# LiJiangnanBit/path_optimizer

Measured on AMD Instinct MI355X. Metric: QP paths/sec at N=200 pts, batch=4096; ADMM iters to 1e-4, higher is better.
Workload: dtype f64

## Files before the change

path_optimizer_amd/binding.py:

```python
from __future__ import annotations

import ctypes as C
import os
import sys

import numpy as np

from .abi import (INFO_BYTES, INFO_DTYPE, PO_ABI_VERSION, PO_ERR_HIP, PO_ERR_UNSUPPORTED, PO_OK, PoBatchIn, PoBatchOut, PoParams)

_HERE = os.path.dirname(os.path.abspath(__file__))
LIB_PATH = os.environ.get("PO_LIB") or os.path.join(_HERE, "libpo_hip.so")
_LIB = None

EXPORTS = ["po_default_params", "po_problem_dims", "po_keep_control_steps", "po_create", "po_destroy", "po_set_stream", "po_debug_set", "po_device_count",
           "po_solve_batch", "po_solve_batch_device", "po_assemble_batch", "po_scaling_batch", "po_last_kernel_ms", "po_last_phase_ms", "po_debug_get", "po_strerror",
           "po_last_hip_error", "po_version", "po_set_map", "po_postcheck_batch", "po_postcheck_batch_device", "po_bounds_batch",
           "po_bounds_batch_device", "po_map_sample", "po_smooth_dims", "po_smooth_batch", "po_smooth_batch_device",
           "po_resample_batch", "po_resample_batch_device", "po_limits_batch", "po_limits_batch_device", "po_dp_search_batch",
           "po_dp_search_batch_device", "po_bspline_batch_device", "po_segment_raw_batch_device", "po_post_project_batch_device",
           "po_segment_init_batch_device", "po_plan_batch", "po_plan_batch_device", "po_densify_batch", "po_densify_batch_device",
           "po_distance_map_batch", "po_distance_map_batch_device", "po_set_map_occupancy", "po_set_map_occupancy_device", "po_get_map",
           "po_set_map_stack", "po_set_map_stack_occupancy", "po_set_map_stack_occupancy_device", "po_set_map_assignment", "po_set_map_assignment_device",
           "po_get_map_layer", "po_map_sample_layer",
           "po_rasterize_batch", "po_rasterize_batch_device", "po_set_map_stack_obstacles", "po_set_map_stack_obstacles_device",
           "po_set_world_occupancy", "po_set_world_occupancy_device", "po_rasterize_scene_batch", "po_rasterize_scene_batch_device",
           "po_set_map_stack_scene", "po_set_map_stack_scene_device",
           "po_default_select_params", "po_select_batch", "po_select_batch_device",
           "po_default_speed_params", "po_speed_batch", "po_speed_batch_device",
           "po_default_dynamic_params", "po_dynamic_batch", "po_dynamic_batch_device",
           "po_default_stplan_params", "po_stplan_batch", "po_stplan_batch_device",
           "po_default_nudge_params", "po_nudge_batch", "po_nudge_batch_device",
           "po_default_trajectory_params", "po_trajectory_batch", "po_trajectory_batch_device",
           "po_default_agentsets_params", "po_agentsets_batch", "po_agentsets_batch_device"]


class PoError(RuntimeError):
    pass


_ENV_DEBUG = {"PO_IDENTITY_ORDER": "identity_order", "PO_DEBUG_CYCLES": "debug_cycles", "PO_SMOOTH_SEQ": "smooth_seq",
              "PO_SMOOTH_WAVES": "smooth_waves", "PO_SMOOTH_NOPAD": "smooth_nopad", "PO_SMOOTH_DEBUG": "smooth_debug", "PO_DP_ONE_WAVE": "dp_one_wave", "PO_NEWTON_SLICE": "newton_slice",
              "PO_FIXED_LENGTH": "fixed_length"}


def lib():
    global _LIB
    if _LIB is None:
        if not os.path.exists(LIB_PATH):
            raise PoError(f"{LIB_PATH} not built: run `python -c 'import __graft_entry__ as g; g.build()'` "
                          "(hipcc --offload-arch=gfx950). There is no CPU fallback.")
        try:
            import torch
        except Exception:
            pass
        L = C.CDLL(LIB_PATH)
        L.po_strerror.restype = C.c_char_p
        L.po_last_hip_error.restype = C.c_char_p
        L.po_version.restype = C.c_char_p
        ver = L.po_version().decode()
        parts = ver.split()
        if len(parts) < 2 or not parts[1].isdigit() or int(parts[1]) != PO_ABI_VERSION:
            raise PoError(f"{LIB_PATH} reports '{ver}' but this binding is written against PO_ABI_VERSION {PO_ABI_VERSION} (include/po_hip.h): rebuild the library")
        L.po_create.argtypes = [C.c_int, C.POINTER(PoParams), C.POINTER(C.c_void_p)]
        L.po_destroy.argtypes = [C.c_void_p]
        L.po_set_stream.argtypes = [C.c_void_p, C.c_void_p]
        L.po_solve_batch.argtypes = [C.c_void_p, C.POINTER(PoBatchIn), C.POINTER(PoBatchOut)]
        L.po_solve_batch_device.argtypes = [C.c_void_p, C.POINTER(PoBatchIn), C.POINTER(PoBatchOut)]
        L.po_assemble_batch.argtypes = [C.c_void_p, C.POINTER(PoBatchIn), C.c_void_p, C.c_void_p, C.c_void_p]
        L.po_scaling_batch.argtypes = [C.c_void_p, C.POINTER(PoBatchIn), C.c_void_p]
        L.po_last_kernel_ms.argtypes = [C.c_void_p, C.POINTER(C.c_float)]
        L.po_last_phase_ms.argtypes = [C.c_void_p, C.POINTER(C.c_float)]
        L.po_debug_get.argtypes = [C.c_void_p, C.c_char_p, C.POINTER(C.c_longlong)]
        L.po_distance_map_batch.argtypes = [C.c_void_p, C.c_int, C.c_void_p, C.c_void_p]
        L.po_distance_map_batch_device.argtypes = [C.c_void_p, C.c_int, C.c_void_p, C.c_void_p]
        L.po_set_map_occupancy.argtypes = [C.c_void_p, C.c_void_p]
        L.po_set_map_occupancy_device.argtypes = [C.c_void_p, C.c_void_p]
        L.po_get_map.argtypes = [C.c_void_p, C.c_void_p, C.c_void_p]
        L.po_set_map_stack.argtypes = [C.c_void_p, C.c_int, C.c_void_p, C.c_void_p]
        L.po_set_map_stack_occupancy.argtypes = [C.c_void_p, C.c_int, C.c_void_p, C.c_void_p]
        L.po_set_map_stack_occupancy_device.argtypes = [C.c_void_p, C.c_int, C.c_void_p, C.c_void_p]
        L.po_set_map_assignment.argtypes = [C.c_void_p, C.c_int, C.c_void_p]
        L.po_set_map_assignment_device.argtypes = [C.c_void_p, C.c_int, C.c_void_p]
        L.po_get_map_layer.argtypes = [C.c_void_p, C.c_int, C.c_void_p, C.c_void_p]
        L.po_map_sample_layer.argtypes = [C.c_void_p, C.c_int, C.c_int, C.c_void_p, C.c_void_p, C.c_void_p]
        L.po_rasterize_batch.argtypes = [C.c_void_p, C.c_int, C.c_void_p, C.c_void_p, C.c_void_p]
        L.po_rasterize_batch_device.argtypes = [C.c_void_p, C.c_int, C.c_void_p, C.c_void_p, C.c_void_p]
        L.po_set_map_stack_obstacles.argtypes = [C.c_void_p, C.c_int, C.c_void_p, C.c_void_p]
        L.po_set_map_stack_obstacles_device.argtypes = [C.c_void_p, C.c_int, C.c_void_p, C.c_void_p]
        L.po_set_world_occupancy.argtypes = [C.c_void_p, C.c_void_p, C.c_int]
        L.po_set_world_occupancy_device.argtypes = [C.c_void_p, C.c_void_p, C.c_int]
        L.po_rasterize_scene_batch.argtypes = [C.c_void_p, C.c_int, C.c_void_p, C.c_void_p, C.c_void_p]
        L.po_rasterize_scene_batch_device.argtypes = [C.c_void_p, C.c_int, C.c_void_p, C.c_void_p, C.c_void_p]
        L.po_set_map_stack_scene.argtypes = [C.c_void_p, C.c_int, C.c_void_p, C.c_void_p]
        L.po_set_map_stack_scene_device.argtypes = [C.c_void_p, C.c_int, C.c_void_p, C.c_void_p]
        L.po_default_select_params.argtypes = [C.c_void_p]
        L.po_default_select_params.restype = None
        L.po_select_batch.argtypes = [C.c_void_p, C.c_void_p, C.c_void_p, C.c_void_p]
        L.po_select_batch_device.argtypes = [C.c_void_p, C.c_void_p, C.c_void_p, C.c_void_p]
        L.po_default_speed_params.argtypes = [C.c_void_p]
        L.po_default_speed_params.restype = None
        L.po_speed_batch.argtypes = [C.c_void_p, C.c_void_p, C.c_void_p, C.c_void_p]
        L.po_speed_batch_device.argtypes = [C.c_void_p, C.c_void_p, C.c_void_p, C.c_void_p]
        L.po_default_dynamic_params.argtypes = [C.c_void_p]
        L.po_default_dynamic_params.restype = None
        L.po_dynamic_batch.argtypes = [C.c_void_p, C.c_void_p, C.c_void_p, C.c_void_p]
        L.po_dynamic_batch_device.argtypes = [C.c_void_p, C.c_void_p, C.c_void_p, C.c_void_p]
        L.po_default_stplan_params.argtypes = [C.c_void_p]
        L.po_default_stplan_params.restype = None
        L.po_stplan_batch.argtypes = [C.c_void_p, C.c_void_p, C.c_void_p, C.c_void_p]
        L.po_stplan_batch_device.argtypes = [C.c_void_p, C.c_void_p, C.c_void_p, C.c_void_p]
        L.po_default_nudge_params.argtypes = [C.c_void_p]
        L.po_default_nudge_params.restype = None
        L.po_nudge_batch.argtypes = [C.c_void_p, C.c_void_p, C.c_void_p, C.c_void_p]
        L.po_nudge_batch_device.argtypes = [C.c_void_p, C.c_void_p, C.c_void_p, C.c_void_p]
        L.po_default_trajectory_params.argtypes = [C.c_void_p]
        L.po_default_trajectory_params.restype = None
        L.po_trajectory_batch.argtypes = [C.c_void_p, C.c_void_p, C.c_void_p, C.c_void_p]
        L.po_trajectory_batch_device.argtypes = [C.c_void_p, C.c_void_p, C.c_void_p, C.c_void_p]
        L.po_default_agentsets_params.argtypes = [C.c_void_p]
        L.po_default_agentsets_params.restype = None
        L.po_agentsets_batch.argtypes = [C.c_void_p, C.c_void_p, C.c_void_p, C.c_void_p]
        L.po_agentsets_batch_device.argtypes = [C.c_void_p, C.c_void_p, C.c_void_p, C.c_void_p]
        _LIB = L
    return _LIB


def _check(rc: int):
    if rc != PO_OK:
        L = lib()
        msg = L.po_strerror(rc).decode()
        if rc == PO_ERR_HIP:
            msg += ": " + L.po_last_hip_error().decode()
        raise PoError(f"libpo_hip: {msg} (rc={rc})")


def default_params() -> PoParams:
    p = PoParams()
    lib().po_default_params(C.byref(p))
    return p


def default_select_params():
    from .abi import PoSelectParams

    p = PoSelectParams()
    lib().po_default_select_params(C.byref(p))
    return p


def default_speed_params():
    from .abi import PoSpeedParams

    p = PoSpeedParams()
    lib().po_default_speed_params(C.byref(p))
    return p


def default_dynamic_params():
    from .abi import PoDynamicParams

    p = PoDynamicParams()
    lib().po_default_dynamic_params(C.byref(p))
    return p


def default_stplan_params():
    from .abi import PoStplanParams

    p = PoStplanParams()
    lib().po_default_stplan_params(C.byref(p))
    return p


def default_nudge_params():
    from .abi import PoNudgeParams

    p = PoNudgeParams()
    lib().po_default_nudge_params(C.byref(p))
    return p


def default_trajectory_params():
    from .abi import PoTrajectoryParams

    p = PoTrajectoryParams()
    lib().po_default_trajectory_params(C.byref(p))
    return p


def covering_discs(params):
    rad = np.sqrt(np.float64(params.car_length / 8) * np.float64(params.car_length / 8) + np.float64(params.car_width / 2) * np.float64(params.car_width / 2))
    return [float(params.d[j]) for j in range(4)], float(rad + np.float64(params.safety_margin))


def default_agentsets_params():
    from .abi import PoAgentsetsParams

    p = PoAgentsetsParams()
    lib().po_default_agentsets_params(C.byref(p))
    return p


def footprint_reach(params, margin):
    width, back, front = params.car_width, params.car_length / 2.0 - params.rear_axle_to_center, params.car_length / 2.0 + params.rear_axle_to_center
    length, bx, shift = front + back, (front - back) / 2.0, width / 4.0
    small_r = float(np.sqrt(2 * (shift * shift)))
    large_r = float(np.sqrt(width * width + ((length - width) / 2.0) * ((length - width) / 2.0))) / 2
    cx = [-back + shift, -back + shift, front - shift, front - shift, bx + (length - width) / 4, bx - (length - width) / 4]
    cy = [-width / 2.0 + shift, width / 2.0 - shift, -width / 2.0 + shift, width / 2.0 - shift, 0.0, 0.0]
    cr = [small_r] * 4 + [large_r] * 2
    return max(float(np.hypot(cx[q], cy[q])) + cr[q] for q in range(6)) + float(margin) + 1e-6


def problem_dims(form: int, N: int, keep: int):
    n, m, c = C.c_int(), C.c_int(), C.c_int()
    _check(lib().po_problem_dims(form, N, keep, C.byref(n), C.byref(m), C.byref(c)))
    return n.value, m.value, c.value


def smooth_dims(kind: int, P: int):
    n, m = C.c_int(), C.c_int()
    _check(lib().po_smooth_dims(kind, P, C.byref(n), C.byref(m)))
    return n.value, m.value


def keep_control_steps(form: int, ref_s) -> int:
    ref_s = np.ascontiguousarray(ref_s, dtype=np.float64)
    k = lib().po_keep_control_steps(form, ref_s.ctypes.data_as(C.c_void_p), len(ref_s))
    if k < 0:
        _check(k)
    return k


def _np(a):
    return None if a is None else a.ctypes.data_as(C.c_void_p)


OBSTACLE_DTYPE = np.dtype([("kind", np.int32), ("n_verts", np.int32), ("v", np.float64, (16,))])


def obstacle_disc(x, y, r):
    from .abi import PO_OBS_DISC

    o = np.zeros((), dtype=OBSTACLE_DTYPE)
    o["kind"] = PO_OBS_DISC
    o["v"][:3] = (x, y, r)
    return o


def obstacle_polygon(xy):
    from .abi import PO_OBS_MAX_VERTS, PO_OBS_POLY

    xy = np.asarray(xy, dtype=np.float64)
    if xy.ndim != 2 or xy.shape[1] != 2 or not 3 <= len(xy) <= PO_OBS_MAX_VERTS:
        raise ValueError("a polygon has 3 .. 8 vertices (x, y)")
    o = np.zeros((), dtype=OBSTACLE_DTYPE)
    o["kind"] = PO_OBS_POLY
    o["n_verts"] = len(xy)
    o["v"][:2 * len(xy)] = xy.reshape(-1)
    return o


def obstacle_box(cx, cy, half_length, half_width, yaw):
    c, s = np.cos(yaw), np.sin(yaw)
    corners = [(cx + sl * half_length * c - sw * half_width * s, cy + sl * half_length * s + sw * half_width * c) for sl, sw in ((1, 1), (-1, 1), (-1, -1), (1, -1))]
    return obstacle_polygon(corners)


def pack_obstacles(layers):
    if isinstance(layers, tuple) and len(layers) == 2:
        return np.ascontiguousarray(layers[0], dtype=OBSTACLE_DTYPE).reshape(-1), np.ascontiguousarray(layers[1], dtype=np.int32).reshape(-1)
    first = np.zeros(len(layers) + 1, dtype=np.int32)
    first[1:] = np.cumsum([len(l) for l in layers])
    obs = np.zeros(int(first[-1]), dtype=OBSTACLE_DTYPE)
    n = 0
    for l in layers:
        for o in l:
            obs[n] = o
            n += 1
    return obs, first


AGENT_DTYPE = np.dtype([("n_pts", np.int32), ("flags", np.int32), ("radius", np.float64), ("t", np.float64, (8,)), ("x", np.float64, (8,)),
                        ("y", np.float64, (8,))])


def pack_agents(sets):
    if isinstance(sets, tuple) and len(sets) == 2:
        return np.ascontiguousarray(sets[0], dtype=AGENT_DTYPE).reshape(-1), np.ascontiguousarray(sets[1], dtype=np.int32).reshape(-1)
    first = np.zeros(len(sets) + 1, dtype=np.int32)
    first[1:] = np.cumsum([len(s) for s in sets])
    agents = np.zeros(int(first[-1]), dtype=AGENT_DTYPE)
    i = 0
    for s in sets:
        for radius, flags, pts in s:
            if len(pts) > 8:
                raise ValueError("an agent has at most 8 points (t, x, y)")
            agents[i]["n_pts"], agents[i]["flags"], agents[i]["radius"] = len(pts), int(flags), radius
            for j, (t, x, y) in enumerate(pts):
                agents[i]["t"][j], agents[i]["x"][j], agents[i]["y"][j] = t, x, y
            i += 1
    return agents, first


def _agent_lists(agents):
    from .abi import PoAgentLists

    ag, first = pack_agents(agents)
    return PoAgentLists(_np(ag) if len(ag) else None, _np(first), len(ag), len(first) - 1), ag, first


def _agent_lists_device(t):
    from .abi import PoAgentLists

    ag = t.get("agents")
    n_agents = 0 if ag is None else ag.numel() * ag.element_size() // AGENT_DTYPE.itemsize
    return PoAgentLists(C.c_void_p(ag.data_ptr()) if n_agents else None, C.c_void_p(t["first"].data_ptr()), n_agents, t["first"].shape[0] - 1)


def pack_rings(shared, layers=None):
    rings = list(shared) + ([] if layers is None else [r for l in layers for r in l])
    xy = [np.asarray(r[0], dtype=np.float64).reshape(-1, 2) for r in rings]
    start = np.zeros(len(rings) + 1, dtype=np.int32)
    start[1:] = np.cumsum([len(v) for v in xy])
    verts = np.concatenate(xy) if xy else np.zeros((0, 2))
    flags = np.array([int(r[1]) for r in rings], dtype=np.int32)
    first = None
    if layers is not None:
        first = np.full(len(layers) + 1, len(shared), dtype=np.int32)
        first[1:] += np.cumsum([len(l) for l in layers]).astype(np.int32)
    return np.ascontiguousarray(verts, dtype=np.float64), start, flags, len(shared), first


def _i32(a):
    return None if a is None else np.ascontiguousarray(a, dtype=np.int32)


class Engine:

    def __init__(self, device: int = 0, params: PoParams | None = None):
        self.params = params or default_params()
        self._h = C.c_void_p()
        _check(lib().po_create(device, C.byref(self.params), C.byref(self._h)))
        try:
            for env, key in _ENV_DEBUG.items():
# ... 766 lines not shown
```

path_optimizer_amd/csrc/po_capi.cpp:

```cpp
#include <hip/hip_runtime.h>

#include <cmath>
#include <cstdint>
#include <cstdio>
#include <algorithm>
#include <cstdlib>
#include <cstring>
#include <limits>
#include <mutex>
#include <new>
#include <string>
#include <vector>

#include "../../include/po_hip.h"
#include "po_handle.hpp"
#include "po_launch.hpp"
#include "po_map.hpp"
#include "po_smooth.hpp"

static thread_local std::string g_hip_err;

bool hip_ok(hipError_t e, const char *what) {
    if (e == hipSuccess) return true;
    g_hip_err = std::string(what) + ": " + hipGetErrorString(e);
    return false;
}

extern "C" {

void po_default_params(po_params *p) {
    if (!p) return;
    const double car_length = 4.9, rear_axle_to_center = 1.45;
    std::memset(p, 0, sizeof(*p));
    p->d[0] = -3.0 / 8.0 * car_length + rear_axle_to_center;
    p->d[1] = -1.0 / 8.0 * car_length + rear_axle_to_center;
    p->d[2] = 1.0 / 8.0 * car_length + rear_axle_to_center;
    p->d[3] = 3.0 / 8.0 * car_length + rear_axle_to_center;
    p->w_curv = 10; p->w_curv_rate = 200; p->w_dev = 0; p->w_slack = 3;
    p->k_w_curv = 50; p->k_w_curv_rate = 200; p->k_w_dev = 0;
    p->w_k_slack = 500; p->w_kp_slack = 25000;
    p->margin = 1.3;
    p->max_steer = 30.0 * M_PI / 180.0;
    p->wheel_base = 2.85;
    p->enable_collision_check = 1;
    p->car_width = 2.0; p->car_length = 4.9; p->rear_axle_to_center = 1.45; p->safety_margin = 0.0;
    p->constraint_end_heading = 1;
    p->scaling = 10;
    p->eps_abs = 1e-4; p->eps_rel = 1e-4; p->eps_prim_inf = 1e-4; p->eps_dual_inf = 1e-4;
    p->rho0 = 0.1; p->sigma = 1e-6; p->alpha = 1.6; p->adapt_tol = 5.0;
    p->max_iter = 4000; p->check_every = 25; p->adapt_every = 100;
    p->t2_w_dev = 0.005; p->t2_w_curv = 1; p->t2_w_curv_rate = 10;
    p->cart_w_curv = 1; p->cart_w_curv_rate = 50; p->cart_w_dev = 0.0;
    p->mu = 0.4; p->max_curvature_rate = 0.1; p->search_lateral_range = 10.0; p->search_long_spacing = 1.5; p->search_lat_spacing = 0.6;
    p->enable_dynamic_segmentation = 1;
    p->enable_raw_output = 1; p->output_spacing = 0.3;
    p->polish = 0; p->polish_delta = 1e-6; p->polish_refine_iter = 3;
    p->refine = 0; p->refine_eps = 1e-7; p->refine_rounds = 1; p->refine_chain = 2; p->refine_extra_rounds = 0;
    p->refine_newton_rho = 100.0; p->refine_newton_rho_eq = 1e4; p->refine_newton_rho_max = 1e5; p->refine_ls_tol = 0.6; p->refine_ls_max = 30; p->refine_newton_max = 300; p->refine_newton_final = 3; p->refine_newton_escalate = 12; p->refine_newton_rho_eq_max = 1e6;
}

int po_problem_dims(int form, int N, int keep, int *n, int *m, int *C) {
    if (N < 2) return PO_ERR_INVALID;
    int c, nn, mm;
    if (form == PO_KP) {
        if (keep < 1) return PO_ERR_INVALID;
        c = (N + keep - 2) / keep; nn = 5 * N + c; mm = 11 * N + c + 2;
    } else if (form == PO_KPC) {
        if (keep != 4) return PO_ERR_INVALID;
        c = (N + keep - 2) / keep; nn = 6 * N + c; mm = 12 * N + 3 * c + 2;
    } else if (form == PO_K) {
        c = N - 1; nn = 4 * N - 1; mm = 11 * N - 1;
    } else {
        return PO_ERR_INVALID;
    }
    if (n) *n = nn;
    if (m) *m = mm;
    if (C) *C = c;
    return PO_OK;
}

int po_keep_control_steps(int form, const double *ref_s, int N) {
    if (!ref_s || N < 2) return PO_ERR_INVALID;
    if (form == PO_KPC) return 4;
    if (form == PO_K) return 1;
    if (form != PO_KP) return PO_ERR_INVALID;
    double interval = 0;
    for (int i = 1; i < N && i < 10; ++i) interval = std::fmax(interval, ref_s[i] - ref_s[i - 1]);
    const double q = 1.2 / interval;
    const int k = (q >= 2147483647.0 || q != q) ? 1 : static_cast<int>(q);
    return k > 1 ? k : 1;
}

static void runtime_prepare() {
    static std::once_flag once;
    std::call_once(once, [] { setenv("GPU_MAX_HW_QUEUES", "16", 0); });
}

int po_device_count(void) {
    runtime_prepare();
    int n = 0;
    return hipGetDeviceCount(&n) == hipSuccess ? n : 0;
}

int po_create(int device, const po_params *params, po_handle *out) {
    if (!params || !out) return PO_ERR_INVALID;
    if (params->scaling < 0 || params->scaling > 100) return PO_ERR_INVALID;
    if (params->refine != 0 && params->refine != 2) return PO_ERR_INVALID;
    if (params->refine == 2 && (params->refine_rounds > 1 ? params->refine_rounds : 1) + (params->refine_extra_rounds > 0 ? params->refine_extra_rounds : 0) >= 32) return PO_ERR_INVALID;
    runtime_prepare();
    int ndev = 0;
    HIP_TRY(hipGetDeviceCount(&ndev));
    if (device < 0 || device >= ndev) return PO_ERR_INVALID;
    HIP_TRY(hipSetDevice(device));
    po_handle_s *h = new (std::nothrow) po_handle_s;
    if (!h) return PO_ERR_NOMEM;
    h->device = device;
    { int cus = 0; if (hipDeviceGetAttribute(&cus, hipDeviceAttributeMultiprocessorCount, device) == hipSuccess && cus > 0) h->wave_slots = 4 * cus; }
    h->params = *params;
    if (!hip_ok(hipStreamCreateWithFlags(&h->own_stream.s, hipStreamNonBlocking), "hipStreamCreate") ||
        !hip_ok(hipEventCreate(&h->ev0.e), "hipEventCreate") || !hip_ok(hipEventCreate(&h->ev1.e), "hipEventCreate")) {
        delete h;
        return PO_ERR_HIP;
    }
    for (Event &e : h->evh) if (!hip_ok(hipEventCreate(&e.e), "hipEventCreate")) { delete h; return PO_ERR_HIP; }
    for (Event &e : h->evp) if (!hip_ok(hipEventCreate(&e.e), "hipEventCreate")) { delete h; return PO_ERR_HIP; }
    {
        Lock g(h->mu);
        h->stream = h->own_stream.s;
    }
    *out = h;
    return PO_OK;
}

int po_destroy(po_handle h) {
    if (!h) return PO_ERR_INVALID;
    (void)hipSetDevice(h->device);
    {
        Lock g(h->mu);
        (void)hipStreamSynchronize(h->stream);
    }
    delete h;
    return PO_OK;
}

int po_debug_set(po_handle h, const char *key, int value) {
    if (!h || !key) return PO_ERR_INVALID;
    Lock g(h->mu);
    const std::string k(key);
    if (k == "identity_order") h->env_identity = value != 0;
    else if (k == "host_threads") h->host_threads = value < 0 ? 0 : value;
    else if (k == "debug_cycles") h->env_cycles = value != 0;
    else if (k == "newton_slice") { h->nw_slice = value > 0 ? (int)value : 0; h->nw_slice_forced = value > 0; }
    else if (k == "fixed_length") h->fixed_length = value != 0;
    else if (k == "smooth_seq") h->env_smooth_seq = value != 0;
    else if (k == "smooth_waves") h->env_smooth_waves = value;
    else if (k == "smooth_nopad") h->env_smooth_nopad = value != 0;
    else if (k == "smooth_debug") h->env_smooth_debug = value != 0;
    else if (k == "dp_one_wave") h->env_dp_one_wave = value != 0;
    else return PO_ERR_INVALID;
    return PO_OK;
}

int po_debug_get(po_handle h, const char *key, long long *value) {
    if (!h || !key || !value) return PO_ERR_INVALID;
    const std::string k(key);
    Lock g(h->mu);
    if (k == "map_ptr") {
        *value = (long long)reinterpret_cast<uintptr_t>(h->maps.d);
        return PO_OK;
    }
    if (k == "map_layers") {
        *value = h->maps.d ? h->maps.M : 0;
        return PO_OK;
    }
    if (k == "world_cells") {
        *value = h->world.cells ? (long long)h->world.size_x * (long long)h->world.size_y : 0;
        return PO_OK;
    }
    if (k == "fixed_length_used") {
        *value = h->fixed_used;
        return PO_OK;
    }
    if (k == "dp_waves_used") {
        *value = h->dp_waves_used;
        return PO_OK;
    }
    if (k == "smooth_variant_used") {
        *value = h->smooth_variant_used;
        return PO_OK;
    }
    if (k == "fallback_paths") {
        *value = 0;
        if (!h->fb_buf.p) return PO_OK;
        HIP_TRY(hipSetDevice(h->device));
        HIP_TRY(hipStreamSynchronize(h->stream));
        int c = 0;
        HIP_TRY(hipMemcpy(&c, h->fb_buf.p, sizeof(int), hipMemcpyDeviceToHost));
        *value = c;
        return PO_OK;
    }
    if (k == "newton_parked") {
        *value = -1;
        if (!h->nw_idx_buf.p || h->nw_last_B <= 0) return PO_OK;
        HIP_TRY(hipSetDevice(h->device));
        HIP_TRY(hipStreamSynchronize(h->stream));
        int c = 0;
        HIP_TRY(hipMemcpy(&c, static_cast<int *>(h->nw_idx_buf.p) + h->nw_last_B, sizeof(int), hipMemcpyDeviceToHost));
        *value = c;
        return PO_OK;
    }
    if (k == "newton_list_ok") {
        *value = -1;
        if (!h->nw_idx_buf.p || h->nw_last_B <= 0) return PO_OK;
        HIP_TRY(hipSetDevice(h->device));
        HIP_TRY(hipStreamSynchronize(h->stream));
        const int B = h->nw_last_B;
        std::vector<int> kl(2 * (size_t)B + 1);
        HIP_TRY(hipMemcpy(kl.data(), h->nw_idx_buf.p, sizeof(int) * kl.size(), hipMemcpyDeviceToHost));
        const int *keys = kl.data(), *list = kl.data() + B;
        const int n = list[0];
        int parked = 0;
        for (int b = 0; b < B; ++b) parked += keys[b] >= 0;
        bool ok = n == parked;
        std::vector<char> seen((size_t)B, 0);
        for (int i = 0; ok && i < n; ++i) {
            const int b = list[1 + i];
            ok = b >= 0 && b < B && keys[b] >= 0 && !seen[(size_t)b];
            if (ok) seen[(size_t)b] = 1;
            if (ok && i > 0) { const int a = list[i]; ok = keys[a] > keys[b] || (keys[a] == keys[b] && a < b); }
        }
        *value = ok ? 1 : 0;
        return PO_OK;
    }
    return PO_ERR_INVALID;
}

int po_set_stream(po_handle h, void *hip_stream) {
    if (!h) return PO_ERR_INVALID;
    Lock g(h->mu);
    h->stream = hip_stream ? static_cast<hipStream_t>(hip_stream) : h->own_stream.s;
    return PO_OK;
}

static po::DevCar make_car(const po_params &p) {
    po::DevCar c{};
    const double width = p.car_width, back = p.car_length / 2.0 - p.rear_axle_to_center, front = p.car_length / 2.0 + p.rear_axle_to_center;
    const double length = front + back;
    c.bx = (front - back) / 2.0;
    c.br = std::sqrt((length / 2) * (length / 2) + (width / 2) * (width / 2));
    const double shift = width / 4.0, small_r = std::sqrt(2 * (shift * shift));
    const double large_r = std::sqrt(width * width + ((length - width) / 2.0) * ((length - width) / 2.0)) / 2;
    const double px[4] = {-back + shift, -back + shift, front - shift, front - shift};
    const double py[4] = {-width / 2.0 + shift, width / 2.0 - shift, -width / 2.0 + shift, width / 2.0 - shift};
    for (int i = 0; i < 4; ++i) { c.cx[i] = px[i]; c.cy[i] = py[i]; c.cr[i] = small_r; }
    c.cx[4] = c.bx + (length - width) / 4; c.cy[4] = 0; c.cr[4] = large_r;
    c.cx[5] = c.bx - (length - width) / 4; c.cy[5] = 0; c.cr[5] = large_r;
    c.enable = p.enable_collision_check;
    return c;
}

static void publish_stack(po_handle h, int M, int sx, int sy, double res, double px, double py, bool layer_pos) PO_REQUIRES(h->mu) {
    const bool keep = h->maps.M == M && h->maps.layer_of;
    po::DevMaps s{};
    s.d = static_cast<const float *>(h->map_buf.p); s.sx = sx; s.sy = sy; s.res = res; s.px = px; s.py = py;
    s.M = M; s.stride = (size_t)sx * (size_t)sy;
    s.pos = layer_pos ? static_cast<const double *>(h->map_pos_buf.p) : nullptr;
    s.layer_of = keep ? static_cast<const int *>(h->map_assign_buf.p) : nullptr;
    s.n_assign = keep ? h->maps.n_assign : 0;
    h->maps = s;
}
static int install_layers(po_handle h, int M, const po_map *map, const double *pos_xy) PO_REQUIRES(h->mu) {
    HIP_TRY(hipSetDevice(h->device));
    const size_t bytes = sizeof(float) * (size_t)M * (size_t)map->size_x * (size_t)map->size_y;
    if (bytes > h->map_buf.cap) h->maps.d = nullptr;
    if (int rc = grow_after_sync(h, h->map_buf, bytes)) return rc;
    if (pos_xy) {
        if (int rc = grow_after_sync(h, h->map_pos_buf, sizeof(double) * 2 * (size_t)M)) return rc;
        HIP_TRY(hipMemcpyAsync(h->map_pos_buf.p, pos_xy, sizeof(double) * 2 * (size_t)M, hipMemcpyHostToDevice, h->stream));
    }
    HIP_TRY(hipMemcpyAsync(h->map_buf.p, map->distance, bytes, hipMemcpyHostToDevice, h->stream));
    HIP_TRY(hipStreamSynchronize(h->stream));
    publish_stack(h, M, map->size_x, map->size_y, map->resolution, map->pos_x, map->pos_y, pos_xy != nullptr);
    return PO_OK;
}

int po_set_map(po_handle h, const po_map *map) {
    if (!h || !map || !map->distance || map->size_x < 1 || map->size_y < 1 || !(map->resolution > 0)) return PO_ERR_INVALID;
    Lock g(h->mu);
    return install_layers(h, 1, map, nullptr);
}

int po_set_map_stack(po_handle h, int M, const po_map *layers, const double *pos_xy) {
    if (!h || M < 1 || !layers || !layers->distance || layers->size_x < 1 || layers->size_y < 1 || !(layers->resolution > 0)) return PO_ERR_INVALID;
    if (layers->size_x > po_edt_max_side() || layers->size_y > po_edt_max_side() || M > po_edt_max_images()) return PO_ERR_UNSUPPORTED;
    Lock call(h->call_mu);
    Lock g(h->mu);
    return install_layers(h, M, layers, pos_xy);
}

int po_set_map_assignment_device(po_handle h, int n, const int *layer_of) {
    if (!h || n < 0) return PO_ERR_INVALID;
    Lock g(h->mu);
    if (n == 0 || !layer_of) {
        h->maps.layer_of = nullptr; h->maps.n_assign = 0;
        return PO_OK;
    }
    if (!h->maps.d) return PO_ERR_INVALID;
    HIP_TRY(hipSetDevice(h->device));
    if (int rc = grow_after_sync(h, h->map_assign_buf, sizeof(int) * (size_t)n)) return rc;
    HIP_TRY(hipMemcpyAsync(h->map_assign_buf.p, layer_of, sizeof(int) * (size_t)n, hipMemcpyDeviceToDevice, h->stream));
    h->maps.layer_of = static_cast<const int *>(h->map_assign_buf.p); h->maps.n_assign = n;
    return PO_OK;
}

int po_set_map_assignment(po_handle h, int n, const int *layer_of) {
    if (!h || n < 0) return PO_ERR_INVALID;
    Lock call(h->call_mu);
    Lock g(h->mu);
    if (n == 0 || !layer_of) {
        h->maps.layer_of = nullptr; h->maps.n_assign = 0;
        return PO_OK;
    }
    if (!h->maps.d) return PO_ERR_INVALID;
    for (int b = 0; b < n; ++b)
        if (layer_of[b] < 0 || layer_of[b] >= h->maps.M) return PO_ERR_INVALID;
    HIP_TRY(hipSetDevice(h->device));
    if (int rc = grow_after_sync(h, h->map_assign_buf, sizeof(int) * (size_t)n)) {
        h->maps.layer_of = nullptr; h->maps.n_assign = 0;
        return rc;
    }
    HIP_TRY(hipMemcpyAsync(h->map_assign_buf.p, layer_of, sizeof(int) * (size_t)n, hipMemcpyHostToDevice, h->stream));
    HIP_TRY(hipStreamSynchronize(h->stream));
    h->maps.layer_of = static_cast<const int *>(h->map_assign_buf.p); h->maps.n_assign = n;
    return PO_OK;
}

static int check_occupancy(po_handle h, int M, const po_occupancy *occ) {
    if (!h || M < 1 || !occ || !occ->cells || occ->size_x < 1 || occ->size_y < 1 || !(occ->resolution > 0)) return PO_ERR_INVALID;
    if (occ->size_x > po_edt_max_side() || occ->size_y > po_edt_max_side() || M > po_edt_max_images()) return PO_ERR_UNSUPPORTED;
    return PO_OK;
}

int po_distance_map_batch_device(po_handle h, int M, const po_occupancy *occ, float *distance) {
    if (int rc = check_occupancy(h, M, occ)) return rc;
    if (!distance) return PO_ERR_INVALID;
    Lock g(h->mu);
    HIP_TRY(hipSetDevice(h->device));
    if (int rc = grow_after_sync(h, h->edt_buf, po_edt_scratch_bytes(M, occ->size_x, occ->size_y))) return rc;
    HIP_TRY(po_launch_edt(occ->cells, M, occ->size_x, occ->size_y, (float)occ->resolution, h->edt_buf.p, distance, h->stream));
    return PO_OK;
}

int po_distance_map_batch(po_handle h, int M, const po_occupancy *occ, float *distance) {
    if (int rc = check_occupancy(h, M, occ)) return rc;
    if (!distance) return PO_ERR_INVALID;
    const size_t cells = (size_t)M * (size_t)occ->size_x * (size_t)occ->size_y;
    Stage S;
    const Slot<float> d_dist = S.out(distance, cells);
    const Slot<unsigned char> d_cells = S.in(occ->cells, cells);
    return staged_call(h, S, &po_handle_s::edt_io, true, [&] {
        po_occupancy dev = *occ;
        dev.cells = d_cells;
        return po_distance_map_batch_device(h, M, &dev, d_dist);
    });
}

static int stack_from_images(po_handle h, int M, const unsigned char *cells, int sx, int sy, double res, double px, double py, const double *pos_xy)
    PO_REQUIRES(h->mu) {
    const size_t stack_bytes = sizeof(float) * (size_t)M * (size_t)sx * (size_t)sy;
    if (stack_bytes > h->map_buf.cap) h->maps.d = nullptr;
    if (int rc = grow_after_sync(h, h->map_buf, stack_bytes)) return rc;
    if (int rc = grow_after_sync(h, h->edt_buf, po_edt_scratch_bytes(M, sx, sy))) return rc;
    if (pos_xy) {
        if (int rc = grow_after_sync(h, h->map_pos_buf, sizeof(double) * 2 * (size_t)M)) return rc;
        HIP_TRY(hipMemcpyAsync(h->map_pos_buf.p, pos_xy, sizeof(double) * 2 * (size_t)M, hipMemcpyDeviceToDevice, h->stream));
    }
    HIP_TRY(po_launch_edt(cells, M, sx, sy, (float)res, h->edt_buf.p, static_cast<float *>(h->map_buf.p), h->stream));
    publish_stack(h, M, sx, sy, res, px, py, pos_xy != nullptr);
    return PO_OK;
}

int po_set_map_stack_occupancy_device(po_handle h, int M, const po_occupancy *occ, const double *pos_xy) {
    if (int rc = check_occupancy(h, M, occ)) return rc;
    Lock g(h->mu);
    HIP_TRY(hipSetDevice(h->device));
    return stack_from_images(h, M, occ->cells, occ->size_x, occ->size_y, occ->resolution, occ->pos_x, occ->pos_y, pos_xy);
}

int po_set_map_occupancy_device(po_handle h, const po_occupancy *occ) { return po_set_map_stack_occupancy_device(h, 1, occ, nullptr); }

int po_set_map_stack_occupancy(po_handle h, int M, const po_occupancy *occ, const double *pos_xy) {
    if (int rc = check_occupancy(h, M, occ)) return rc;
    Stage S;
    const Slot<unsigned char> d_cells = S.in(occ->cells, (size_t)M * (size_t)occ->size_x * (size_t)occ->size_y);
    const Slot<double> d_pos = S.in(pos_xy, 2 * (size_t)M);
    return staged_call(h, S, &po_handle_s::edt_io, true, [&] {
        po_occupancy dev = *occ;
        dev.cells = d_cells;
        return po_set_map_stack_occupancy_device(h, M, &dev, d_pos);
    });
}

int po_set_map_occupancy(po_handle h, const po_occupancy *occ) { return po_set_map_stack_occupancy(h, 1, occ, nullptr); }

static int check_lists(po_handle h, int M, const po_obstacle_lists *L) {
    if (!h || M < 1 || !L || !L->first || L->n_obs < 0 || (L->n_obs > 0 && !L->obs) || L->size_x < 1 || L->size_y < 1 || !(L->resolution > 0) ||
        !std::isfinite(L->resolution))
        return PO_ERR_INVALID;
    if (L->base_count != 0 && L->base_count != 1 && L->base_count != M) return PO_ERR_INVALID;
    if (L->base_count != 0 && !L->base) return PO_ERR_INVALID;
    if (L->size_x > po_edt_max_side() || L->size_y > po_edt_max_side() || M > po_edt_max_images()) return PO_ERR_UNSUPPORTED;
    return PO_OK;
}
static int check_list_contents(int M, const po_obstacle_lists *L) {
    if (L->first[0] != 0) return PO_ERR_INVALID;
    for (int k = 0; k < M; ++k)
        if (L->first[k + 1] < L->first[k]) return PO_ERR_INVALID;
    if (L->first[M] > L->n_obs) return PO_ERR_INVALID;
    for (int i = 0; i < L->n_obs; ++i) {
        const po_obstacle &o = L->obs[i];
        if (o.kind == PO_OBS_DISC) {
            if (!std::isfinite(o.v[0]) || !std::isfinite(o.v[1]) || !std::isfinite(o.v[2]) || o.v[2] < 0) return PO_ERR_INVALID;
        } else if (o.kind == PO_OBS_POLY) {
            if (o.n_verts < 3 || o.n_verts > PO_OBS_MAX_VERTS) return PO_ERR_INVALID;
            for (int e = 0; e < 2 * o.n_verts; ++e)
                if (!std::isfinite(o.v[e])) return PO_ERR_INVALID;
        } else {
            return PO_ERR_INVALID;
        }
    }
    return PO_OK;
}
struct StagedLists {
    Slot<po_obstacle> obs;
    Slot<int> first;
    Slot<unsigned char> base;
    Slot<double> pos;
    void declare(Stage &S, int M, const po_obstacle_lists *L, const double *pos_xy) {
        obs = S.in(L->n_obs > 0 ? L->obs : nullptr, (size_t)L->n_obs);
        first = S.in(L->first, (size_t)M + 1);
        base = S.in(L->base_count > 0 ? L->base : nullptr, (size_t)L->base_count * (size_t)L->size_x * (size_t)L->size_y);
        pos = S.in(pos_xy, 2 * (size_t)M);
    }
    po_obstacle_lists device(const po_obstacle_lists *L) const {
        po_obstacle_lists d = *L;
        d.obs = obs; d.first = first; d.base = base;
        return d;
    }
};

int po_rasterize_batch_device(po_handle h, int M, const po_obstacle_lists *lists, const double *pos_xy, unsigned char *cells_out) {
    if (int rc = check_lists(h, M, lists)) return rc;
    if (!cells_out) return PO_ERR_INVALID;
    Lock g(h->mu);
    HIP_TRY(hipSetDevice(h->device));
    HIP_TRY(po_launch_raster(lists, M, pos_xy, cells_out, h->stream));
    return PO_OK;
}

int po_rasterize_batch(po_handle h, int M, const po_obstacle_lists *lists, const double *pos_xy, unsigned char *cells_out) {
    if (int rc = check_lists(h, M, lists)) return rc;
    if (!cells_out) return PO_ERR_INVALID;
    if (int rc = check_list_contents(M, lists)) return rc;
    Stage S;
    StagedLists d;
    d.declare(S, M, lists, pos_xy);
    const Slot<unsigned char> d_cells = S.out(cells_out, (size_t)M * (size_t)lists->size_x * (size_t)lists->size_y);
    return staged_call(h, S, &po_handle_s::edt_io, true, [&] {
        const po_obstacle_lists dev = d.device(lists);
        return po_rasterize_batch_device(h, M, &dev, d.pos, d_cells);
    });
}

int po_set_map_stack_obstacles_device(po_handle h, int M, const po_obstacle_lists *lists, const double *pos_xy) {
    if (int rc = check_lists(h, M, lists)) return rc;
    Lock g(h->mu);
    HIP_TRY(hipSetDevice(h->device));
    if (int rc = grow_after_sync(h, h->raster_buf, (size_t)M * (size_t)lists->size_x * (size_t)lists->size_y)) return rc;
    unsigned char *cells = static_cast<unsigned char *>(h->raster_buf.p);
    HIP_TRY(po_launch_raster(lists, M, pos_xy, cells, h->stream));
    return stack_from_images(h, M, cells, lists->size_x, lists->size_y, lists->resolution, lists->pos_x, lists->pos_y, pos_xy);
}

int po_set_map_stack_obstacles(po_handle h, int M, const po_obstacle_lists *lists, const double *pos_xy) {
    if (int rc = check_lists(h, M, lists)) return rc;
    if (int rc = check_list_contents(M, lists)) return rc;
    Stage S;
    StagedLists d;
    d.declare(S, M, lists, pos_xy);
    return staged_call(h, S, &po_handle_s::edt_io, true, [&] {
        const po_obstacle_lists dev = d.device(lists);
        return po_set_map_stack_obstacles_device(h, M, &dev, d.pos);
    });
}

static int check_world(po_handle h, const po_occupancy *w, int outside_occupied) {
    if (!h || (outside_occupied != 0 && outside_occupied != 1)) return PO_ERR_INVALID;
    if (!w) return PO_OK;
    if (!w->cells || w->size_x < 1 || w->size_y < 1 || !(w->resolution > 0) || !std::isfinite(w->resolution) || !std::isfinite(w->pos_x) || !std::isfinite(w->pos_y))
        return PO_ERR_INVALID;
    if (w->size_x > PO_WORLD_MAX_SIDE || w->size_y > PO_WORLD_MAX_SIDE) return PO_ERR_UNSUPPORTED;
    return PO_OK;
}
static int install_world(po_handle h, const po_occupancy *w, int outside_occupied, hipMemcpyKind kind) PO_REQUIRES(h->mu) {
    if (!w) {
        h->world = po_occupancy{};
        return PO_OK;
    }
    HIP_TRY(hipSetDevice(h->device));
    const size_t bytes = (size_t)w->size_x * (size_t)w->size_y;
    if (bytes > h->world_buf.cap) h->world.cells = nullptr;
    if (int rc = grow_after_sync(h, h->world_buf, bytes)) return rc;
    HIP_TRY(hipMemcpyAsync(h->world_buf.p, w->cells, bytes, kind, h->stream));
    h->world = *w;
    h->world.cells = static_cast<const unsigned char *>(h->world_buf.p);
    h->world_outside = outside_occupied;
    return PO_OK;
}

int po_set_world_occupancy_device(po_handle h, const po_occupancy *world, int outside_occupied) {
    if (int rc = check_world(h, world, outside_occupied)) return rc;
    Lock g(h->mu);
    return install_world(h, world, outside_occupied, hipMemcpyDeviceToDevice);
}

int po_set_world_occupancy(po_handle h, const po_occupancy *world, int outside_occupied) {
    if (int rc = check_world(h, world, outside_occupied)) return rc;
    Lock call(h->call_mu);
    Lock g(h->mu);
    PO_TRY(install_world(h, world, outside_occupied, hipMemcpyHostToDevice));
    if (world) HIP_TRY(hipStreamSynchronize(h->stream));
    return PO_OK;
}
// ... 903 lines not shown
```

path_optimizer_amd/csrc/po_device.hpp:

```cpp
#pragma once
#include <hip/hip_runtime.h>

#include "../../include/po_hip.h"

namespace po {

constexpr double kInf = 1e30;
constexpr double kInfThresh = 1e26;
constexpr int kStatusDeferred = -100;
constexpr double kRhoMin = 1e-6, kRhoMax = 1e6, kRhoEqOverIneq = 1e3, kRhoTol = 1e-4;
constexpr double kPi = 3.14159265358979323846;
constexpr double kPi2 = 1.57079632679489661923;
constexpr int kNwKeys = 32;

enum { F_KP = 0, F_KPC = 1, F_K = 2 };
enum { M_EY = 1, M_EPHI = 2, M_C = 4, M_S1 = 8, M_S2 = 16 };

struct DevParams {
    double d1, d2, d3, d4;
    double w_dev, w_c, w_cr, w_s1, w_s2, w_u, w_su;
    double margin, kmax, max_steer, wheel_base;
    double sigma, alpha, rho0, eps_abs, eps_rel, eps_pinf, adapt_tol;
    int max_iter, check_every, adapt_every, end_heading;
    double pol_delta;
    int polish, pol_refine;
    int refine, ref_rounds, ref_extra;
    double ref_eps;
    double ref_nw_rho, ref_nw_rho_eq, ref_nw_rho_max, ref_nw_rho_eq_max, ref_ls_tol;
    int ref_ls_max, ref_nw_max, ref_nw_final, ref_nw_esc;
    int ref_nw_slice;
};

struct DevBatch {
    int B, N, keep, C;
    const double *ref_x, *ref_y, *ref_z, *ref_k, *ref_s;
    const double *bounds, *x0, *goal_z, *max_k, *max_kp;
    double *out_states;
    po_info *out_info;
    double *out_x;
    const int *n_points;
    const int *order;
    const double *scale;
    long long *dbg_cycles;
    int perm_bits;
    int only_deferred;
    int n, m;
    int round;
    double *pol_state;
    int pol_stride;
    int *fb_list;
    int nw_phase;
    double *nw_state;
    int nw_stride;
    int *nw_keys;
    int *nw_list;
    int nw_follows;
    int fixed_len;
};

template <int F> struct FormTraits;
template <> struct FormTraits<F_KP> {
    static constexpr int NLOC = 8, NEND = 2, NDYN = 3, NS = 1, HAS_U = 1, NCTL = 1, HAS_SU = 0;
};
template <> struct FormTraits<F_KPC> {
    static constexpr int NLOC = 9, NEND = 2, NDYN = 3, NS = 2, HAS_U = 1, NCTL = 3, HAS_SU = 1;
};
template <> struct FormTraits<F_K> {
    static constexpr int NLOC = 9, NEND = 0, NDYN = 2, NS = 1, HAS_U = 0, NCTL = 0, HAS_SU = 0;
};

__host__ __device__ __forceinline__ double clipd(double v, double l, double u) { return fmin(fmax(v, l), u); }
struct NegInfT { __host__ __device__ constexpr operator double() const { return -kInf; } };
struct PosInfT { __host__ __device__ constexpr operator double() const { return kInf; } };
__host__ __device__ __forceinline__ double clipd(double v, NegInfT, double u) { return fmin(v, u); }
__host__ __device__ __forceinline__ double clipd(double v, double l, PosInfT) { return fmax(v, l); }
__host__ __device__ __forceinline__ double clipd(double v, NegInfT, PosInfT) { return v; }

__device__ __forceinline__ double rho_of(double l, double u, double rho, double rho_eq) {
    if (l < -kInfThresh && u > kInfThresh) return kRhoMin;
    return (u - l < kRhoTol) ? rho_eq : rho;
}

__device__ __forceinline__ double wrap_angle(double a) {
    for (int it = 0; it < 64; ++it) {
        if (a > kPi) a -= 2 * kPi;
        else if (a < -kPi) a += 2 * kPi;
        else break;
    }
    return a;
}

struct StageIn {
    double lb[4], ub[4];
    double maxk;
    double elo, ehi;
    int j, N, last;
};

template <int F, class Fn> __device__ __forceinline__ void local_rows(const StageIn &s, const DevParams &P, Fn &fn) {
    if constexpr (F == F_KP) {
        fn.template row<M_C>(0, 0., 0., 1., 0., 0., -P.kmax, P.kmax);
        fn.template row<M_S1>(1, 0., 0., 0., 1., 0., 0.0, P.margin);
        fn.template row<M_EY | M_EPHI>(2, 1., P.d1, 0., 0., 0., s.lb[0], s.ub[0]);
        fn.template row<M_EY | M_EPHI>(3, 1., P.d3, 0., 0., 0., s.lb[2], s.ub[2]);
        fn.template row<M_EY | M_EPHI | M_S1>(4, 1., P.d4, 0., -1., 0., NegInfT{}, s.ub[3] - P.margin);
        fn.template row<M_EY | M_EPHI | M_S1>(5, 1., P.d4, 0., 1., 0., s.lb[3] + P.margin, PosInfT{});
        fn.template row<M_EY | M_EPHI | M_S1>(6, 1., P.d2, 0., -1., 0., NegInfT{}, s.ub[1] - P.margin);
        fn.template row<M_EY | M_EPHI | M_S1>(7, 1., P.d2, 0., 1., 0., s.lb[1] + P.margin, PosInfT{});
    } else if constexpr (F == F_KPC) {
        fn.template row<M_C | M_S2>(0, 0., 0., 1., 0., 1., -s.maxk, PosInfT{});
        fn.template row<M_C | M_S2>(1, 0., 0., 1., 0., -1., NegInfT{}, s.maxk);
        fn.template row<M_S1>(2, 0., 0., 0., 1., 0., 0.0, P.margin);
        fn.template row<M_S2>(3, 0., 0., 0., 0., 1., 0.0, fmax(P.kmax - s.maxk, 0.0));
        fn.template row<M_EY | M_EPHI>(4, 1., P.d1, 0., 0., 0., s.lb[0], s.ub[0]);
        fn.template row<M_EY | M_EPHI>(5, 1., P.d2, 0., 0., 0., s.lb[1], s.ub[1]);
        fn.template row<M_EY | M_EPHI>(6, 1., P.d4, 0., 0., 0., s.lb[3], s.ub[3]);
        fn.template row<M_EY | M_EPHI | M_S1>(7, 1., P.d3, 0., -1., 0., NegInfT{}, s.ub[2] - P.margin);
        fn.template row<M_EY | M_EPHI | M_S1>(8, 1., P.d3, 0., 1., 0., s.lb[2] + P.margin, PosInfT{});
    } else {
        const bool win = s.last && (s.elo > -kInf);
        fn.template row<M_EPHI>(0, 0., 1., 0., 0., 0., win ? s.elo : -kInf, win ? s.ehi : kInf);
        fn.template row<M_EY>(1, 1., 0., 0., 0., 0., NegInfT{}, PosInfT{});
        if (!s.last) fn.template row<M_C>(2, 0., 0., 1., 0., 0., -P.max_steer, P.max_steer);
        fn.template row<M_S1>(3, 0., 0., 0., 1., 0., 0.0, P.margin);
        fn.template row<M_EY | M_EPHI>(4, 1., P.d1, 0., 0., 0., s.lb[0], s.ub[0]);
        fn.template row<M_EY | M_EPHI>(5, 1., P.d3, 0., 0., 0., s.lb[2], s.ub[2]);
        fn.template row<M_EY | M_EPHI>(6, 1., P.d4, 0., 0., 0., s.lb[3], s.ub[3]);
        fn.template row<M_EY | M_EPHI | M_S1>(7, 1., P.d2, 0., -1., 0., NegInfT{}, s.ub[1] - P.margin);
        fn.template row<M_EY | M_EPHI | M_S1>(8, 1., P.d2, 0., 1., 0., s.lb[1] + P.margin, PosInfT{});
    }
}

template <int F, class Fn> __device__ __forceinline__ void end_rows(const StageIn &s, const DevParams &, Fn &fn) {
    if constexpr (F == F_KP) {
        fn.template row<M_EY>(0, 1., 0., 0., 0., 0., -1.0, 1.0);
        fn.template row<M_EPHI>(1, 0., 1., 0., 0., 0., s.elo, s.ehi);
    } else if constexpr (F == F_KPC) {
        fn.template row<M_EY>(0, 1., 0., 0., 0., 0., NegInfT{}, PosInfT{});
        fn.template row<M_EPHI>(1, 0., 1., 0., 0., 0., s.elo, s.ehi);
    }
}

template <int F> __device__ __forceinline__ int ref_row_local(int r, int j, int N, int C) {
    if constexpr (F == F_KP) {
        const int cb = 5 * N + C;
        switch (r) {
            case 0: return 3 * N + j;
            case 1: return 4 * N + C + j;
            case 2: return cb + 2 * j;
            case 3: return cb + 2 * j + 1;
            default: return cb + (r - 2) * N + j;
        }
    } else if constexpr (F == F_KPC) {
        const int sb = 5 * N + 2 * C, cb = 7 * N + 3 * C;
        switch (r) {
            case 0: return 3 * N + j;
            case 1: return 4 * N + j;
            case 2: return sb + j;
            case 3: return sb + N + j;
            case 4: case 5: case 6: return cb + 3 * j + (r - 4);
            case 7: return cb + 3 * N + j;
            default: return cb + 4 * N + j;
        }
    } else {
        switch (r) {
            case 0: return 2 * N + 2 * j;
            case 1: return 2 * N + 2 * j + 1;
            case 2: return 4 * N + j;
            case 3: return 5 * N - 1 + j;
            case 4: case 5: case 6: return 6 * N - 1 + 3 * j + (r - 4);
            case 7: return 9 * N - 1 + j;
            default: return 10 * N - 1 + j;
        }
    }
}
template <int F> __device__ __forceinline__ int ref_row_end(int r, int N, int C) {
    if constexpr (F == F_KP) return 11 * N + C + r;
    else if constexpr (F == F_KPC) return 12 * N + 3 * C + r;
    else return 0;
}
template <int F> __device__ __forceinline__ int ref_row_ctl(int r, int c, int N, int C) {
    if constexpr (F == F_KP) return 4 * N + c;
    else if constexpr (F == F_KPC) return r == 0 ? 5 * N + c : (r == 1 ? 5 * N + C + c : 5 * N + 2 * C + 2 * N + c);
    else return 0;
}

template <int F> struct Dyn {
    double f[FormTraits<F>::NDYN][3];
    double beta[FormTraits<F>::NDYN];
    double b[FormTraits<F>::NDYN];
};
template <int F> __device__ __forceinline__ constexpr int dyn_tau(int r) {
    if constexpr (F == F_K) return r == 0 ? 1 : 0;
    else return r;
}
template <int F> __device__ __forceinline__ Dyn<F> make_dyn(double k, double ds, const DevParams &P) {
    Dyn<F> d;
    if constexpr (F == F_K) {
        const double steer = atan(k * P.wheel_base);
        const double cs = cos(steer);
        const double c2 = __dmul_rn(cs, cs);
        d.f[0][0] = __dmul_rn(-ds, __dmul_rn(k, k));
        d.f[0][1] = 1.0;
        d.f[0][2] = ds / P.wheel_base / c2;
        d.beta[0] = 0;
        d.b[0] = __dmul_rn(ds, steer) / P.wheel_base / c2;
        d.f[1][0] = 1.0;
        d.f[1][1] = ds;
        d.f[1][2] = 0;
        d.beta[1] = 0;
        d.b[1] = 0;
    } else {
        d.f[0][0] = 1.0; d.f[0][1] = ds; d.f[0][2] = 0; d.beta[0] = 0; d.b[0] = 0;
        d.f[1][0] = __dmul_rn(-__dmul_rn(k, k), ds); d.f[1][1] = 1.0; d.f[1][2] = ds; d.beta[1] = 0;
        d.b[1] = __dmul_rn(ds, k);
        d.f[2][0] = 0; d.f[2][1] = 0; d.f[2][2] = 1.0; d.beta[2] = ds; d.b[2] = 0;
    }
    return d;
}

__device__ __forceinline__ void k_trig(double k, double ds, const DevParams &P, double tr[2]) {
    const double steer = atan(k * P.wheel_base);
    const double cs = cos(steer);
    const double c2 = __dmul_rn(cs, cs);
    tr[0] = ds / P.wheel_base / c2;
    tr[1] = __dmul_rn(ds, steer) / P.wheel_base / c2;
}
template <int F> __device__ __forceinline__ Dyn<F> make_dyn_tr(double k, double ds, const double tr[2], const DevParams &P) {
    if constexpr (F == F_K) {
        Dyn<F> d;
        d.f[0][0] = __dmul_rn(-ds, __dmul_rn(k, k)); d.f[0][1] = 1.0; d.f[0][2] = tr[0]; d.beta[0] = 0; d.b[0] = tr[1];
        d.f[1][0] = 1.0; d.f[1][1] = ds; d.f[1][2] = 0; d.beta[1] = 0; d.b[1] = 0;
        return d;
    } else {
        return make_dyn<F>(k, ds, P);
    }
}

template <int F> __device__ __forceinline__ double p_diag_node(int comp, int j, int N, const DevParams &P) {
    if (comp == 0) return P.w_dev;
    if (comp == 1) return 0.0;
    if constexpr (F == F_K) {
        if (j >= N - 1) return 0.0;
        return (j == 0 || j == N - 2) ? P.w_c + P.w_cr : P.w_cr * 2 + P.w_c;
    } else {
        return P.w_c;
    }
}

__device__ __forceinline__ int ctl_index(int i, int keep) { return keep == 4 ? (i >> 2) : (i / keep); }
__device__ __forceinline__ bool last_of_group(int i, int N, int keep) {
    return (i == N - 2) || (keep == 4 ? (((i + 1) & 3) == 0) : ((i + 1) % keep == 0));
}

__device__ __forceinline__ int perm_index(unsigned i, int bits, int B) {
    if (bits <= 0) return (int)i;
    const unsigned mask = (1u << bits) - 1u, h = bits > 1 ? (unsigned)bits >> 1 : 1u;
    do {
        i ^= i >> h; i = (i * 0x9E3779B1u) & mask;
        i ^= i >> h; i = (i * 0x85EBCA6Bu) & mask;
        i ^= i >> h;
    } while (i >= (unsigned)B);
    return (int)i;
}

#if defined(PO_REF) && PO_REF == 3 && !defined(PO_SHFL_REDUCE)
#define PO_DPP_REDUCE 1
#endif
#ifdef PO_DPP_REDUCE
template <int CTRL> __device__ __forceinline__ double dpp_shr_keep(double v) {
    const int lo = __builtin_amdgcn_update_dpp(__double2loint(v), __double2loint(v), CTRL, 0xf, 0xf, false);
    const int hi = __builtin_amdgcn_update_dpp(__double2hiint(v), __double2hiint(v), CTRL, 0xf, 0xf, false);
    return __hiloint2double(hi, lo);
}
template <int CTRL> __device__ __forceinline__ double dpp_shr_zero(double v) {
    const int lo = __builtin_amdgcn_mov_dpp(__double2loint(v), CTRL, 0xf, 0xf, true);
    const int hi = __builtin_amdgcn_mov_dpp(__double2hiint(v), CTRL, 0xf, 0xf, true);
    return __hiloint2double(hi, lo);
}
__device__ __forceinline__ double lane_of(double v, int k) {
    return __hiloint2double(__builtin_amdgcn_readlane(__double2hiint(v), k), __builtin_amdgcn_readlane(__double2loint(v), k));
}
__device__ __forceinline__ double wave_sum(double v) {
    v += dpp_shr_zero<0x111>(v); v += dpp_shr_zero<0x112>(v); v += dpp_shr_zero<0x114>(v); v += dpp_shr_zero<0x118>(v);
    return (lane_of(v, 15) + lane_of(v, 31)) + (lane_of(v, 47) + lane_of(v, 63));
}
#else
__device__ __forceinline__ double wave_sum(double v) {
#pragma unroll
    for (int o = 32; o > 0; o >>= 1) v += __shfl_xor(v, o);
    return v;
}
#endif
#ifndef PO_NO_UNI
__device__ __forceinline__ double uni(double v) {
    return __hiloint2double(__builtin_amdgcn_readfirstlane(__double2hiint(v)), __builtin_amdgcn_readfirstlane(__double2loint(v)));
}
__device__ __forceinline__ int uni(int v) { return __builtin_amdgcn_readfirstlane(v); }
#else
__device__ __forceinline__ double uni(double v) { return v; }
__device__ __forceinline__ int uni(int v) { return v; }
#endif
__device__ __forceinline__ int nonfinite_bits(double v) {
    int hi = __double2hiint(v);
    asm volatile("" : "+v"(hi));
    return (hi & 0x7ff00000) == 0x7ff00000;
}

__device__ __forceinline__ int nan_bits(double v) {
    int hi = __double2hiint(v), lo = __double2loint(v);
    asm volatile("" : "+v"(hi), "+v"(lo));
    return (hi & 0x7ff00000) == 0x7ff00000 && ((hi & 0x000fffff) | lo) != 0;
}

#ifdef PO_DPP_REDUCE
__device__ __forceinline__ double wave_max(double v) {
    v = fmax(v, dpp_shr_keep<0x111>(v)); v = fmax(v, dpp_shr_keep<0x112>(v)); v = fmax(v, dpp_shr_keep<0x114>(v)); v = fmax(v, dpp_shr_keep<0x118>(v));
    return fmax(fmax(lane_of(v, 15), lane_of(v, 31)), fmax(lane_of(v, 47), lane_of(v, 63)));
}
#else
__device__ __forceinline__ double wave_max(double v) {
#pragma unroll
    for (int o = 32; o > 0; o >>= 1) v = fmax(v, __shfl_xor(v, o));
    return v;
}
#endif

__device__ __forceinline__ double row_rho(double l, double u, double e, double w, double rho, double rho_eq) {
    return rho_of(l * e, u * e, rho, rho_eq) * w;
}
__device__ __forceinline__ unsigned row_class(double l, double u, double e) {
    const double ls = l * e, us = u * e;
    if (ls < -kInfThresh && us > kInfThresh) return 2u;
    return (us - ls < kRhoTol) ? 1u : 0u;
}
__device__ __forceinline__ double class_rho(unsigned cls, int r, double w, double rho, double rho_eq) {
    const unsigned c = (cls >> (2 * r)) & 3u;
    return w * (c == 0u ? rho : (c == 1u ? rho_eq : kRhoMin));
}
struct ClassFn {
    unsigned cls;
    const double *E;
    template <int MASK, class TL, class TU> __device__ __forceinline__ void row(int r, double, double, double, double, double, TL l, TU u) {
        cls |= row_class(l, u, E[r]) << (2 * r);
    }
};

struct HessFn {
    double H[15];
    double rho, rho_eq;
    const double *W, *E;
    unsigned cls;
    __device__ HessFn(double r, double re, const double *W_, const double *E_, unsigned cls_) : rho(r), rho_eq(re), W(W_), E(E_), cls(cls_) {
#pragma unroll
        for (int i = 0; i < 15; ++i) H[i] = 0;
    }
    static __device__ __forceinline__ constexpr int idx(int a, int b) { return a * 5 - a * (a - 1) / 2 + (b - a); }
    template <int MASK, class TL, class TU> __device__ __forceinline__ void row(int ri, double c0, double c1, double c2, double c3, double c4, TL l, TU u) {
        const double r = class_rho(cls, ri, W[ri], rho, rho_eq);
        const double c[5] = {c0, c1, c2, c3, c4};
#pragma unroll
// ... 260 lines not shown
```

path_optimizer_amd/csrc/po_fast.inc:

```

#ifndef PO_KERNEL_ATTR
#define PO_KERNEL_ATTR
#endif
#define PO_FRESH_LANE_ID(fx) asm volatile("" : "+v"((fx).tid))
#ifdef PO_MARKS
#define PO_MARK(name) asm volatile("; PO_MARK " name)
#else
#define PO_MARK(name)
#endif

template <int F, int SPL, int G = 1> struct LaneState {
    using T = FormTraits<F>;
    static_assert(G == 1 || (T::HAS_U && !T::HAS_SU && T::NCTL == 1), "several controls per lane: KP");
    double x[SPL][3 + T::NS];
    double vl[SPL][T::NLOC];
    double vd[SPL][T::NDYN];
    double vdo[T::NDYN];
    double vend[2];
    double lb[SPL][4], ub[SPL][4], maxk[SPL];
    double kin[SPL], dsin[SPL];
    double kout, dsout;
    double trin[F == F_K ? SPL : 1][2], trout[2];
    double hi[SPL][T::NS], hv[SPL][T::NS][3], gs[SPL][T::NS];
    double bin0[3];
// ... 3494 lines not shown
                for (int r = 0; r < T::NDYN; ++r) st.vdo[r] = d.b[r];
            }
        }
        st.su = 0;
#pragma unroll
        for (int g = 0; g < NG; ++g) st.u[g] = 0;
        if constexpr (T::HAS_U) {
#pragma unroll
            for (int g = 0; g < NG; ++g) if (has_ctl(g)) { PolResetFn fc{st.vc[g], st.pcc}; ctl_rows<F>(st.mkp, fc); }
        }
    }
    __device__ __forceinline__ PolRes pol_eval(const LS &st, const unsigned cls0[SPL], unsigned clse0, unsigned clsc0, double delta,
                                               unsigned pcn[SPL], unsigned &pcne, unsigned &pcnc) const {
        const double idelta = 1.0 / delta;
        const int nst = nst_own();
        double xl[4] = {0, 0, 0, st.u[NG - 1]}, pl[4], nf[3], xf[3] = {st.x[0][0], st.x[0][1], st.x[0][2]};
#pragma unroll
        for (int q = 0; q < SPL; ++q) if (q == nst - 1) { xl[0] = st.x[q][0]; xl[1] = st.x[q][1]; xl[2] = st.x[q][2]; }
        xchg<4>(xl, -1, pl, 0);
        xchg<3>(xf, +1, nf, 1);
        const double nf2 = nf[2];
        double rp = 0, rd = 0, ob = 0, ytku[NG];
#pragma unroll
        for (int g = 0; g < NG; ++g) ytku[g] = 0;
        int changes = 0, bad = 0;
        pcne = pcnc = 0;
#pragma unroll
        for (int q = 0; q < SPL; ++q) {
            pcn[q] = 0;
            const int j = stage(q);
            if (j >= N) continue;
            const StageIn si = stage_in(st, q);
            PolEvalFn fn;
            fn.v = st.vl[q]; fn.W = Wloc(j); fn.cls = cls0[q]; fn.pc_old = st.pc[q]; fn.pc_new = 0; fn.idelta = idelta; fn.rp = fn.nAx = fn.nz = 0; fn.changes = 0;
#pragma unroll
            for (int a = 0; a < 5; ++a) { fn.x[a] = a < 3 + T::NS ? st.x[q][a] : 0.0; fn.aty[a] = 0; }
            local_rows<F>(si, P, fn);
            pcn[q] = fn.pc_new;
            if (T::NEND && si.last) {
                const unsigned keep_new = fn.pc_new;
                fn.v = st.vend; fn.W = Wend(); fn.cls = clse0; fn.pc_old = st.pce; fn.pc_new = 0;
                end_rows<F>(si, P, fn);
                pcne = fn.pc_new; fn.pc_new = keep_new;
            }
            changes += fn.changes;
            double bin[3] = {0, 0, 0}, ax[3] = {0, 0, 0};
            if (j == 0) {
#pragma unroll
                for (int r = 0; r < T::NDYN; ++r) { bin[r] = st.bin0[r]; ax[r] = -fn.x[dyn_tau<F>(r)]; }
            } else {
                const Dyn<F> d = dyn_in(st, q);
                const double p0 = q > 0 ? st.x[q > 0 ? q - 1 : 0][0] : pl[0], p1 = q > 0 ? st.x[q > 0 ? q - 1 : 0][1] : pl[1], p2 = q > 0 ? st.x[q > 0 ? q - 1 : 0][2] : pl[2];
                const double uu = T::HAS_U ? (q > 0 ? st.u[gIn(q)] : pl[3]) : 0.0;
#pragma unroll
                for (int r = 0; r < T::NDYN; ++r) {
                    bin[r] = d.b[r];
                    ax[r] = d.f[r][0] * p0 + d.f[r][1] * p1 + d.f[r][2] * p2 + d.beta[r] * uu - fn.x[dyn_tau<F>(r)];
                    if (q > 0) ytku[gIn(q)] += Wdyn()[r] * ((ax[r] - d.b[r]) + (st.vd[q][r] - d.b[r]) * idelta) * d.beta[r];
                }
            }
#pragma unroll
            for (int r = 0; r < T::NDYN; ++r) {
                const double y = Wdyn()[r] * ((ax[r] - bin[r]) + (st.vd[q][r] - bin[r]) * idelta);
                fn.rp = fmax(fn.rp, fabs(ax[r] - bin[r]));
                fn.aty[dyn_tau<F>(r)] -= y;
            }
            if (j < N - 1) {
                const Dyn<F> d = dyn_out(st, q);
                const double n0 = q + 1 < SPL ? st.x[q + 1 < SPL ? q + 1 : q][0] : nf[0], n1 = q + 1 < SPL ? st.x[q + 1 < SPL ? q + 1 : q][1] : nf[1];
                const double n2 = q + 1 < SPL ? st.x[q + 1 < SPL ? q + 1 : q][2] : nf2;
                const double nx[3] = {n0, n1, n2};
                const double uu = T::HAS_U ? st.u[gOut(q)] : 0.0;
#pragma unroll
                for (int r = 0; r < T::NDYN; ++r) {
                    const double vv = q + 1 < SPL ? st.vd[q + 1 < SPL ? q + 1 : q][r] : st.vdo[r];
                    const double axo = d.f[r][0] * fn.x[0] + d.f[r][1] * fn.x[1] + d.f[r][2] * fn.x[2] + d.beta[r] * uu - nx[dyn_tau<F>(r)];
                    const double y = Wdyn()[r] * ((axo - d.b[r]) + (vv - d.b[r]) * idelta);
                    fn.aty[0] += y * d.f[r][0]; fn.aty[1] += y * d.f[r][1]; fn.aty[2] += y * d.f[r][2];
                    if (q == SPL - 1) ytku[NG - 1] += y * d.beta[r];
                }
            }
            double px[5];
            px[0] = p_diag_node<F>(0, j, N, P) * fn.x[0];
            px[1] = 0.0;
            px[2] = p_diag_node<F>(2, j, N, P) * fn.x[2];
            if constexpr (F == F_K) {
                if (j <= N - 2) {
                    if (j >= 1) px[2] -= P.w_cr * (q > 0 ? st.x[q > 0 ? q - 1 : 0][2] : pl[2]);
                    if (j + 1 <= N - 2) px[2] -= P.w_cr * (q + 1 < SPL ? st.x[q + 1 < SPL ? q + 1 : q][2] : nf2);
                }
            }
            px[3] = P.w_s1 * fn.x[3];
            px[4] = T::NS > 1 ? P.w_s2 * fn.x[4] : 0.0;
#pragma unroll
            for (int a = 0; a < 3 + T::NS; ++a) {
                ob += fn.x[a] * px[a];
                bad |= nonfinite_bits(fn.x[a]) | nonfinite_bits(px[a] + fn.aty[a]);
                rd = fmax(rd, fabs(px[a] + fn.aty[a]));
            }
            rp = fmax(rp, fn.rp);
        }
        if constexpr (T::HAS_U) {
#pragma unroll
            for (int g = 0; g < NG; ++g)
            if (has_ctl(g)) {
                PolEvalFn fn;
                fn.v = st.vc[g]; fn.W = Wctl(); fn.cls = clsc0; fn.pc_old = st.pcc; fn.pc_new = 0; fn.idelta = idelta; fn.rp = fn.nAx = fn.nz = 0; fn.changes = 0;
                fn.x[0] = fn.x[1] = fn.x[4] = 0; fn.x[2] = st.u[g]; fn.x[3] = T::HAS_SU ? st.su : 0.0;
#pragma unroll
                for (int a = 0; a < 5; ++a) fn.aty[a] = 0;
                ctl_rows<F>(st.mkp, fn);
                pcnc = fn.pc_new; changes += fn.changes;
                fn.aty[2] += ytku[g];
                const double pxv[2] = {P.w_u * fn.x[2], T::HAS_SU ? P.w_su * fn.x[3] : 0.0};
#pragma unroll
                for (int a = 0; a < 1 + T::HAS_SU; ++a) {
                    ob += fn.x[2 + a] * pxv[a];
                    bad |= nonfinite_bits(fn.x[2 + a]) | nonfinite_bits(pxv[a] + fn.aty[2 + a]);
                    rd = fmax(rd, fabs(pxv[a] + fn.aty[2 + a]));
                }
                rp = fmax(rp, fn.rp);
            }
        }
        rp = wave_max(rp); rd = wave_max(rd); ob = wave_sum(ob);
        double chs = wave_sum((double)changes);
        bad = __any(bad) ? 1 : 0;
        if constexpr (NT > 64) {
            __syncthreads();
            double *red = S + L.ex;
            const int w = tid >> 6;
            if ((tid & 63) == 0) { red[w * 5] = rp; red[w * 5 + 1] = rd; red[w * 5 + 2] = ob; red[w * 5 + 3] = chs; red[w * 5 + 4] = bad ? 1.0 : 0.0; }
            __syncthreads();
            ob = 0; chs = 0;
            for (int k = 0; k < NT / 64; ++k) { rp = fmax(rp, red[k * 5]); rd = fmax(rd, red[k * 5 + 1]); ob += red[k * 5 + 2]; chs += red[k * 5 + 3]; bad |= red[k * 5 + 4] != 0.0; }
            __syncthreads();
        }
        PolRes R = {rp, rd, 0.5 * ob, (int)chs, bad};
        return R;
    }

    __device__ __forceinline__ void output_pass(const LS &st) const {
        double *out = in.out_states + po * 5;
        double rz[SPL], rx[SPL], ry[SPL];
#pragma unroll
        for (int q = 0; q < SPL; ++q) {
            const int j = stage(q);
            const size_t at = po + (j < N ? j : 0);
            rz[q] = in.ref_z[at]; rx[q] = in.ref_x[at]; ry[q] = in.ref_y[at];
        }
        for (int i = 5 * N + tid; i < 5 * in.N; i += NT) out[i] = 0.0;
        double *pxy = S + L.bz;
#pragma unroll
        for (int q = 0; q < SPL; ++q) {
            const int j = stage(q);
            if (j >= N) continue;
            const double ey = st.x[q][0], ephi = st.x[q][1];
            const double ang = rz[q];
            const double na = wrap_angle(ang + kPi2);
            double sn, cn;
            sincos(na, &sn, &cn);
            const double tx = rx[q] + __dmul_rn(ey, cn);
            const double ty = ry[q] + __dmul_rn(ey, sn);
            pxy[2 * j] = tx; pxy[2 * j + 1] = ty;
            out[5 * j + 0] = tx; out[5 * j + 1] = ty; out[5 * j + 2] = ang + ephi;
            if constexpr (F != F_K) out[5 * j + 3] = st.x[q][2];
            else if (j < N - 1) out[5 * j + 3] = st.x[q][2];
            if constexpr (F == F_K) { if (j == N - 2) out[5 * (N - 1) + 3] = st.x[q][2]; }
        }
        __syncthreads();
        double *dsg = pxy + 2 * N;
#pragma unroll
        for (int q = 0; q < SPL; ++q) {
            const int j = stage(q);
            if (j < 1 || j >= N) continue;
            const double dx = pxy[2 * j] - pxy[2 * j - 2], dy = pxy[2 * j + 1] - pxy[2 * j - 1];
            dsg[j] = sqrt(__dadd_rn(__dmul_rn(dx, dx), __dmul_rn(dy, dy)));
        }
        __syncthreads();
        if (tid == 0) {
            double s = 0;
            out[4] = 0;
            for (int j = 1; j < N; ++j) {
                s += dsg[j];
                out[5 * j + 4] = s;
            }
        }
        if (in.out_x) {
            double *ox = in.out_x + (size_t)b * in.n;
            for (int i = tid; i < in.n; i += NT) ox[i] = 0.0;
            __syncthreads();
#pragma unroll
            for (int q = 0; q < SPL; ++q) {
                const int j = stage(q);
                if (j >= N) continue;
                if constexpr (F == F_K) {
                    ox[2 * j] = st.x[q][1]; ox[2 * j + 1] = st.x[q][0];
                    if (j < N - 1) ox[2 * N + j] = st.x[q][2];
                    ox[3 * N - 1 + j] = st.x[q][3];
                } else {
                    ox[3 * j] = st.x[q][0]; ox[3 * j + 1] = st.x[q][1]; ox[3 * j + 2] = st.x[q][2];
                    ox[3 * N + C + j] = st.x[q][3];
                    if constexpr (F == F_KPC) ox[3 * N + C + N + j] = st.x[q][4];
                }
            }
            if constexpr (T::HAS_U) {
#pragma unroll
                for (int g = 0; g < NG; ++g)
                    if (has_ctl(g)) { ox[3 * N + cidx(g)] = st.u[g]; if constexpr (T::HAS_SU) ox[3 * N + C + 2 * N + cidx(g)] = st.su; }
            }
        }
    }
};

struct LoopOut { int status, it, nref; double rho; Resid R; };
constexpr int kStatusSolvedOutOfIters = 2;
constexpr int kStatusRestoreEntry = 3;
template <bool UNI, bool RESUME, int F, int SPL, int NT, bool TWO, int NWX, int NFIX>
__device__ __forceinline__ LoopOut admm_loop(Fast<F, SPL, NT, TWO, NWX, NFIX> &fx, typename Fast<F, SPL, NT, TWO, NWX, NFIX>::LS &st, const DevBatch &in, const DevParams &P, long long tc[3], long long ph[8],
                                             double eps_mul = 1.0, bool resume = false, int it0 = 0, int nref0 = 0, double rho_prev = 0.0) {
    double rho = uni(fmin(fmax(P.rho0, kRhoMin), kRhoMax));
    if constexpr (RESUME) { if (resume) rho = uni(rho_prev); eps_mul = uni(eps_mul); }
    const long long tf0 = in.dbg_cycles != nullptr ? __builtin_readcyclecounter() : 0;
    if constexpr (TWO) { fx.template factor_blocks_two<UNI>(st, rho); }
    else { fx.factor_blocks(st, rho); }
    const long long tf1 = in.dbg_cycles != nullptr ? __builtin_readcyclecounter() : 0;
    if constexpr (TWO) { fx.factor_chain_two(st, rho); }
    else { fx.factor_chain(); }
    if (in.dbg_cycles != nullptr) { ph[6] = tf1 - tf0; ph[7] = (long long)__builtin_readcyclecounter() - tf1; }
    int status = PO_STATUS_UNSOLVED, it = 0, nref = 0;
    if constexpr (RESUME) { if (resume) { it = it0; nref = nref0 + 1; } }
    Resid R = {0, 0, 0, 0, 0, 0, 0, 0, 0, 0, 0, 0, 0, 0};
    const bool prof = in.dbg_cycles != nullptr;
    for (it = it + 1; it <= P.max_iter; ++it) {
        const bool first = (it == 1);
        PO_FRESH_LANE_ID(fx);
        long long t0 = prof ? __builtin_readcyclecounter() : 0;
        PO_MARK("rhs_begin");
        if constexpr (TWO) {
            if (first) fx.template rhs_pass_two<UNI, true>(st, rho);
            else { PO_MARK("rhs_hot"); fx.template rhs_pass_two<UNI, false>(st, rho); PO_MARK("rhs_hot_end"); }
        } else fx.rhs_pass(st, rho, first);
        long long t1 = prof ? __builtin_readcyclecounter() : 0;
        PO_MARK("solve_begin");
        PO_FRESH_LANE_ID(fx);
        if constexpr (NWX == 2 || NWX == 3) fx.solve_split(st, rho);
        else if constexpr (TWO) fx.solve_two(st, rho, prof ? ph : nullptr); else fx.chain_solve();
        PO_MARK("update_begin");
        PO_FRESH_LANE_ID(fx);
        long long t2 = prof ? __builtin_readcyclecounter() : 0;
        const bool can_check = P.check_every > 0 && (it % P.check_every == 0);
        typename Fast<F, SPL, NT, TWO, NWX, NFIX>::Cert cert = {0, 0, 0};
        if constexpr (TWO) {
            if (can_check) cert = fx.template update_pass_two<true, false, UNI>(st, rho, first);
            else if (first) (void)fx.template update_pass_two<false, true, UNI>(st, rho, true);
            else { PO_MARK("upd_hot"); (void)fx.template update_pass_two<false, false, UNI>(st, rho, false); PO_MARK("upd_hot_end"); }
        }
        else { if (can_check) cert = fx.template update_pass<true>(st, first, rho); else (void)fx.template update_pass<false>(st, first, rho); }
        long long t3 = prof ? __builtin_readcyclecounter() : 0;
        tc[0] += t1 - t0; tc[1] += t2 - t1; tc[2] += t3 - t2;
        PO_MARK("update_end");
        const bool can_adapt = P.adapt_every > 0 && (it % P.adapt_every == 0);
        if (can_check || can_adapt || it == P.max_iter) {
            if constexpr (TWO) R = fx.template residual_pass_two<UNI>(st, rho); else R = fx.residual_pass(st, rho);
            if (R.bad) { status = PO_STATUS_NON_FINITE; break; }
            if (can_check || it == P.max_iter) {
                double eps_p = P.eps_abs + P.eps_rel * fmax(R.nAx, R.nz);
                double eps_d = P.eps_abs + P.eps_rel * fmax(R.nPx, R.nAty);
                if constexpr (RESUME) { eps_p *= eps_mul; eps_d *= eps_mul; }
                if (R.rp < eps_p && R.rd < eps_d) { status = PO_STATUS_SOLVED; break; }
                if (can_check && !(R.rp < eps_p) && fx.sc[kScC] * cert.ndy > P.eps_pinf && cert.sup < -P.eps_pinf * cert.ndy &&
                    cert.natdy < P.eps_pinf * cert.ndy) { status = PO_STATUS_PRIMAL_INFEASIBLE; break; }
            }
            if (can_adapt) {
                const double pr = R.rps / (fmax(R.nAxs, R.nzs) + 1e-10);
                const double dr = R.rds / (fmax(R.nPxs, R.nAtys) + 1e-10);
                double rn = rho * sqrt(pr / (dr + 1e-10));
                rn = fmin(fmax(rn, kRhoMin), kRhoMax);
                if (rn > rho * P.adapt_tol || rn < rho / P.adapt_tol) {
                    fx.template rescale_pass<UNI>(st, rho / rn);
                    rho = uni(rn);
                    if constexpr (TWO) { fx.template factor_blocks_two<UNI>(st, rho); fx.factor_chain_two(st, rho); }
                    else { fx.factor_blocks(st, rho); fx.factor_chain(); }
                    ++nref;
                }
            }
        }
    }
    if (it > P.max_iter) {
        it = P.max_iter;
        if (status == PO_STATUS_UNSOLVED) {
            status = PO_STATUS_MAX_ITER;
            if constexpr (RESUME) {
                if (eps_mul < 1.0) status = (R.rp < P.eps_abs + P.eps_rel * fmax(R.nAx, R.nz) && R.rd < P.eps_abs + P.eps_rel * fmax(R.nPx, R.nAty)) ? kStatusSolvedOutOfIters : kStatusRestoreEntry;
            }
        }
    }
    LoopOut o = {status, it, nref, rho, R};
    return o;
}

struct RefineOut { bool take, stop; int it, nfac; Resid R; bool parked; };
constexpr int kNwParkScalars = 12;
constexpr int kNwStagnation = 8;
template <int F, int SPL, int NT, int NWX, int PH = 0, int NFIX = 0>
__device__ __forceinline__ RefineOut refine_phase_newton(Fast<F, SPL, NT, true, NWX, NFIX> &fx, typename Fast<F, SPL, NT, true, NWX, NFIX>::LS &st, const DevParams &P, double rho_solve, double rp0, double rd0,
                                                         int slice = 0, double *park = nullptr, int *park_key = nullptr) {
    constexpr bool resume = PH == 2;
    if constexpr (PH != 1) slice = 0;
#pragma unroll
    for (int q = 0; q < SPL; ++q) {
#pragma unroll
        for (int s = 0; s < FormTraits<F>::NS; ++s) { st.hi[q][s] = 0; st.gs[q][s] = 0; st.hv[q][s][0] = st.hv[q][s][1] = st.hv[q][s][2] = 0; }
    }
    st.hiu = st.hus = st.gsu = 0;
    fx.bound_classes(st);
    unsigned cls0[SPL];
#pragma unroll
    for (int q = 0; q < SPL; ++q) cls0[q] = st.cls[q];
    const unsigned clse0 = st.clse, clsc0 = st.clsc;
    double rb = uni(fmin(fmax(P.ref_nw_rho, kRhoMin), kRhoMax)), pri_outer = -1.0;
    rho_solve = uni(rho_solve); rp0 = uni(rp0); rd0 = uni(rd0);
    fx.nw_req = uni(P.ref_nw_rho_eq);
    int nfac = 0, it2 = 0, nouter = 0, nfinal = 0, nsmall = 0, nstag = 0;
    bool stop = false, dirty = true, certified = false, parked = false, refac_uncounted = false, quiet = false;
    double rd_prev = -1.0;
    bool first_pass = true;
    unsigned clsf[SPL], clsef = 0, clscf = 0;
#pragma unroll
    for (int q = 0; q < SPL; ++q) clsf[q] = 0;
    if constexpr (resume) {
        rb = uni(park[0]); fx.nw_req = uni(park[1]); pri_outer = uni(park[2]); nouter = uni((int)park[3]); it2 = uni((int)park[4]); nfinal = uni((int)park[5]); nfac = uni((int)park[6]);
        certified = uni((int)(park[7] != 0.0)) != 0;
        nstag = uni((int)park[8]); quiet = uni((int)(park[9] != 0.0)) != 0; rd_prev = uni(park[10]);
#pragma unroll
        for (int q = 0; q < SPL; ++q) clsf[q] = st.pc[q];
        clsef = st.pce; clscf = st.pcc;
        dirty = false; refac_uncounted = true;
    }
    Resid R = {0, 0, 0, 0, 0, 0, 0, 0, 0, 0, 0, 0, 0, 0};
#ifdef PO_NW_TRACE
    long long tcy[8] = {0, 0, 0, 0, 0, 0, 0, 0}, tlast = __builtin_readcyclecounter();
    int nev = 0;
#define PO_NW_TICK(i) { const long long n_ = __builtin_readcyclecounter(); tcy[i] += n_ - tlast; tlast = n_; }
#else
#define PO_NW_TICK(i)
#endif
    PO_FRESH_LANE_ID(fx);
    if constexpr (!resume) fx.nw_reexpress_pass(st, rho_solve / rb, kRhoEqOverIneq * rho_solve / fx.nw_req, cls0, clse0, clsc0);
    for (;;) {
        PO_FRESH_LANE_ID(fx);
        PO_MARK("nw_reclass");
        (void)fx.reclass_pass(st, cls0, clse0, clsc0, rb, rb, 3);
        PO_NW_TICK(0)
        PO_MARK("nw_residual");
        R = fx.template residual_pass_two<false>(st, rb);
        R.rp = uni(R.rp); R.rd = uni(R.rd); R.obj = uni(R.obj);
        PO_NW_TICK(1)
        PO_MARK("nw_test");
        if (R.bad) break;
        const double tol_d = P.ref_eps + P.ref_eps * fmax(R.nPx, R.nAty);
        const bool dual_ok = R.rd < tol_d;
        stop = dual_ok && R.rp < P.ref_eps + P.ref_eps * fmax(R.nAx, R.nz);
        if (!(resume && first_pass)) {
            if (quiet && rd_prev >= 0.0 && R.rd > 0.5 * rd_prev) ++nstag; else nstag = 0;
            rd_prev = R.rd;
        }
        first_pass = false;
        if (stop) {
            if (P.ref_nw_final <= 0 || R.rd < 1e-3 * tol_d || nfinal >= P.ref_nw_final) break;
            certified = true;
        } else {
            certified = false;
            if (it2 >= P.ref_nw_max) break;
            if (nstag >= kNwStagnation) break;
            if constexpr (PH == 1) { if (it2 >= slice) { parked = true; break; } }
        }
        if (!certified && dual_ok) {
            if (++nouter > 50) break;
            double ratio = 1.0, ratio_eq = 1.0;
            if (pri_outer >= 0.0 && R.rp > 0.25 * pri_outer) {
                const double esc = P.ref_nw_esc > 0 && nouter >= P.ref_nw_esc ? (nouter >= 2 * P.ref_nw_esc ? 100.0 : 10.0) : 1.0;
                if (rb * 10.0 <= fmin(P.ref_nw_rho_max * esc, kRhoMax)) { ratio = 0.1; rb = uni(rb * 10.0); dirty = true; }
                else if (fx.nw_req * 10.0 <= fmin(P.ref_nw_rho_eq_max * esc, 1e8)) { ratio_eq = 0.1; fx.nw_req = uni(fx.nw_req * 10.0); dirty = true; }
            }
            pri_outer = R.rp;
            PO_FRESH_LANE_ID(fx);
            fx.nw_reexpress_pass(st, ratio, ratio_eq, cls0, clse0, clsc0);
            quiet = false;
            continue;
        }
        PO_MARK("nw_factor");
        {
            bool diff = st.clse != clsef || (fx.has_ctl() && st.clsc != clscf);
#pragma unroll
            for (int q = 0; q < SPL; ++q) diff = diff || st.cls[q] != clsf[q];
            if (fx.block_any(diff)) dirty = true;
        }
        quiet = !dirty;
        if (dirty || (resume && refac_uncounted)) {
            fx.template factor_blocks_two<false>(st, rb); fx.factor_chain_two(st, rb);
            if (!resume || dirty) ++nfac;
            dirty = false; refac_uncounted = false;
#pragma unroll
            for (int q = 0; q < SPL; ++q) clsf[q] = st.cls[q];
            clsef = st.clse; clscf = st.clsc;
        }
        PO_NW_TICK(2)
#if defined(PO_NW_TRACE) && !defined(PO_NW_TRACE_QUIET)
        if (fx.b == 0 && fx.tid == 0) printf("  dev step %d outer %d nfac %d certified %d  r_prim %.3e r_dual %.3e (tol %.3e)\n", it2, nouter, nfac, (int)certified, R.rp, R.rd, tol_d);
#endif
        PO_FRESH_LANE_ID(fx);
        PO_MARK("nw_rhs");
        fx.template rhs_pass_two<false, false, false, true>(st, rb);
        PO_NW_TICK(3)
        PO_FRESH_LANE_ID(fx);
        PO_MARK("nw_solve");
        if constexpr (NWX == 2 || NWX == 3) fx.solve_split(st, rb); else fx.solve_two(st, rb, nullptr);
        PO_NW_TICK(4)
        PO_FRESH_LANE_ID(fx);
        PO_MARK("nw_dir0");
        double c0 = 0, c1 = 0, f0i = 0, dum_ = 0;
        fx.template nw_dir_pass<0>(st, rb, 0.0, cls0, clse0, clsc0, c0, c1, f0i);
        fx.block_sum2(c0, c1);
        c0 = uni(c0); c1 = uni(c1);
        PO_NW_TICK(5)
        double t = 1.0, lo = 0.0, hi = -1.0, f0 = 0.0, f = 0.0, fp = 0.0;
        PO_MARK("nw_ls_begin");
        fx.nw_ls_eval01(st, rb, cls0, clse0, clsc0, f0, f, fp);
#ifdef PO_NW_TRACE
        nev += 2;
#endif
        f0 = uni(f0 + c0); f = uni(f + (c0 + c1)); fp = uni(fp + c1);
        const bool fail = !(f0 < 0.0);
        if (!fail) {
            const double ls_tol = certified ? fmin(P.ref_ls_tol, 1e-4) : P.ref_ls_tol;
            for (int ev = 0;;) {
                if (fabs(f) <= ls_tol * fabs(f0)) break;
                if (f < 0) lo = t; else hi = t;
                double tn = fp > 0 ? t - f / fp : -1.0;
                if (!(tn > lo && (hi < 0 || tn < hi))) tn = hi < 0 ? 2.0 * t : 0.5 * (lo + hi);
                t = uni(tn);
                if (++ev >= P.ref_ls_max) break;
                fx.nw_ls_eval(st, rb, t, cls0, clse0, clsc0, f, fp);
#ifdef PO_NW_TRACE
                ++nev;
#endif
                f = uni(f + (c0 + c1 * t)); fp = uni(fp + c1);
            }
        }
        PO_MARK("nw_ls_end");
        PO_NW_TICK(6)
        if (fail) { stop = certified; break; }
        double d0 = 0, d1 = 0;
        PO_MARK("nw_dir1");
        fx.template nw_dir_pass<1>(st, rb, t, cls0, clse0, clsc0, d0, d1, dum_);
        PO_MARK("nw_step_end");
        PO_NW_TICK(7)
        ++it2;
        if (certified) ++nfinal;
        quiet = quiet && t == 1.0;
        if constexpr (PH == 1) { if (t < 0.5) ++nsmall; }
    }
    if constexpr (PH == 1) if (parked) {
        if (fx.tid == 0) {
            park[0] = rb; park[1] = fx.nw_req; park[2] = pri_outer; park[3] = nouter; park[4] = it2; park[5] = nfinal; park[6] = nfac; park[7] = certified ? 1.0 : 0.0;
            park[8] = nstag; park[9] = quiet ? 1.0 : 0.0; park[10] = rd_prev;
            const float kf = (nouter == 0 ? (float)nsmall : 0.0f) + 2.0f * __log10f((float)fmax(R.rp, 1e-30)) + 14.0f;
            const int ki = (int)floorf(1.5f * kf);
            *park_key = ki < 0 ? 0 : (ki > kNwKeys - 1 ? kNwKeys - 1 : ki);
        }
#pragma unroll
        for (int q = 0; q < SPL; ++q) st.pc[q] = clsf[q];
        st.pce = clsef; st.pcc = clscf;
        fx.nw_req = 0.0;
        RefineOut o = {false, false, it2, nfac, R, true};
        return o;
    }
#ifdef PO_NW_TRACE
    if (fx.b == 0 && fx.tid == 0)
        printf("  dev newton: %d steps %d fac %d outer %d ls evals; cycles: reclass %lld residual %lld factor %lld (pivots %lld phi %lld tables %lld) rhs %lld solve %lld dir0 %lld ls %lld dir1 %lld\n", it2, nfac, nouter, nev,
               tcy[0], tcy[1], tcy[2], fx.dbgc[0], fx.dbgc[1], fx.dbgc[2], tcy[3], tcy[4], tcy[5], tcy[6], tcy[7]);
#endif
#undef PO_NW_TICK
    (void)fx.reclass_pass(st, cls0, clse0, clsc0, rb, rho_solve, 2, fx.nw_req, kRhoEqOverIneq * rho_solve);
    fx.nw_req = 0.0;
    RefineOut o = {!R.bad && (stop || (R.rp <= rp0 && R.rd <= rd0)), stop && !R.bad, it2, nfac, R, false};
    return o;
}

__device__ __forceinline__ void zero_outputs(const DevBatch &in, int b, int nt) {
    double *os = in.out_states + (size_t)b * in.N * 5;
    for (int i = threadIdx.x; i < in.N * 5; i += nt) os[i] = 0.0;
    if (in.out_x != nullptr) {
        double *ox = in.out_x + (size_t)b * in.n;
        for (int i = threadIdx.x; i < in.n; i += nt) ox[i] = 0.0;
    }
}

template <int F, int SPL, int NT, bool TWO, bool UNI, int NWX, int REF = 0, int NFIX = 0> __device__ __forceinline__ void solve_body(const DevBatch &in, const DevParams &P, int b_given = -1) {
    static_assert(TWO || !UNI, "the single-level mapping has no uniform variant");
    static_assert(REF == 0 || (REF == 2 && TWO && !UNI), "the later rounds run on the general variant of the two-level mapping");
    static_assert(NFIX == 0 || (REF == 0 && UNI), "fixed length: the uniform warm start only");
    extern __shared__ double smem[];
    int b;
    const int round = in.round;
    if (b_given >= 0) b = b_given;
    else b = in.order ? in.order[blockIdx.x] : perm_index(blockIdx.x, in.perm_bits, in.B);
    if ((unsigned)b >= (unsigned)in.B) return;
    if constexpr (REF) { if (round > 0 && in.out_info[b].status != kStatusDeferred - round) return; }
    if constexpr (TWO && !UNI) {
        if (in.only_deferred && round == 0 && in.out_info[b].status != kStatusDeferred) return;
    }
    Fast<F, SPL, NT, TWO, NWX, NFIX> fx(P, in, smem, b);
    typename Fast<F, SPL, NT, TWO, NWX, NFIX>::LS st;
    fx.load(st);
    if (fx.inputs_have_nan()) {
        zero_outputs(in, b, NT);
        if (fx.tid == 0) { po_info o = {PO_STATUS_NON_FINITE, 0, 0, 0, 0.0, 0.0, 0.0, 0.0, 0, 0}; in.out_info[b] = o; }
        return;
    }
    if constexpr (UNI) {
        if (!fx.classify(st)) {
            if (fx.tid == 0 && round == 0) in.out_info[b].status = kStatusDeferred;
            return;
        }
    }
    for (int i = fx.tid; i < fx.L.total; i += NT) smem[i] = 0.0;
    __syncthreads();
    fx.scale_to_lds();
    long long tc[3] = {0, 0, 0}, ph[8] = {0, 0, 0, 0, 0, 0, 0, 0};
    LoopOut lo;
    int sref = 0;
    if constexpr (!REF) {
        lo = admm_loop<UNI, false>(fx, st, in, P, tc, ph);
        if constexpr (TWO) {
            if (in.pol_state != nullptr) fx.template state_io<true>(st, in.pol_state + (size_t)b * in.pol_stride);
        }
    } else {
        double *state = in.pol_state + (size_t)b * in.pol_stride;
        const int rounds = P.ref_rounds > 1 ? P.ref_rounds : 1;
        const int rounds_total = rounds + P.ref_extra;
        double eps_mul = 1.0;
        for (int r = round + 1; r < rounds; ++r) eps_mul *= 10.0;
        for (int r = rounds; r <= round; ++r) eps_mul *= 0.1;
        const po_info *oi0 = in.out_info + b;
        const int it0 = oi0->status_polish, nref0 = oi0->n_refactor;
        int ref_it = oi0->iters - oi0->status_polish;
        const double rho_prev = oi0->rho;
        sref = oi0->status_refine;
        fx.template state_io<false>(st, state);
        lo = admm_loop<UNI, true>(fx, st, in, P, tc, ph, eps_mul, true, it0, nref0, rho_prev);
        if (lo.status == kStatusRestoreEntry) {
            fx.template state_io<false>(st, state);
            const po_info *oi = in.out_info + b;
            lo.R.rp = oi->r_prim; lo.R.rd = oi->r_dual; lo.R.obj = oi->obj; lo.rho = oi->rho;
            lo.status = kStatusSolvedOutOfIters;
        } else fx.template state_io<true>(st, state);
        bool hand_back = false;
        if (P.refine && lo.status == PO_STATUS_SOLVED) {
            const bool last = round + 1 >= rounds_total;
            __syncthreads();
            typename Fast<F, SPL, NT, TWO, NWX, NFIX>::LS st2;
            fx.load(st2);
            fx.template state_io<false>(st2, state);
            const RefineOut ro = refine_phase_newton<F, SPL, NT, NWX, 0, NFIX>(fx, st2, P, lo.rho, lo.R.rp, lo.R.rd);
            __syncthreads();
            if (ro.take) fx.template state_io<true>(st2, state);
            ref_it += ro.it; lo.nref += ro.nfac;
            if (ro.take) lo.R = ro.R;
            sref = ro.stop ? 1 : -1;
            hand_back = !ro.stop && !last;
            __syncthreads();
            fx.template state_io<false>(st, state);
        }
        if (hand_back) {
            if (fx.tid == 0) {
                po_info *oi = in.out_info + b;
                oi->status = kStatusDeferred - (round + 1); oi->iters = lo.it + ref_it; oi->status_polish = lo.it; oi->n_refactor = lo.nref;
                oi->r_prim = lo.R.rp; oi->r_dual = lo.R.rd; oi->rho = lo.rho; oi->obj = lo.R.obj; oi->status_refine = sref;
            }
            return;
        }
        if (lo.status == kStatusSolvedOutOfIters) lo.status = PO_STATUS_SOLVED;
        lo.it += ref_it;
    }
    bool outputs_later = false;
    if constexpr (!REF) outputs_later = in.nw_follows != 0 && lo.status == PO_STATUS_SOLVED;
    if (!outputs_later) fx.output_pass(st);
    if (fx.tid == 0) {
        po_info o;
        o.status = lo.status; o.iters = lo.it; o.n_refactor = lo.nref; o.status_polish = 0;
        o.r_prim = lo.R.rp; o.r_dual = lo.R.rd; o.rho = lo.rho; o.obj = lo.R.obj;
        o.status_refine = sref; o.reserved = 0;
        in.out_info[b] = o;
        if (in.dbg_cycles != nullptr) { long long *d = in.dbg_cycles + (size_t)b * 16; d[0] = tc[0]; d[1] = tc[1]; d[2] = tc[2]; d[3] = lo.it; for (int i = 0; i < 8; ++i) d[4 + i] = ph[i]; d[12] = UNI ? 1 : 0; }
    }
}
template <int F, int SPL, int NT, bool TWO, bool UNI, int NWX = 1, int NFIX = 0> __global__ PO_KERNEL_ATTR __launch_bounds__(NT) void solve_kernel_fast(DevBatch in, DevParams P) {
    solve_body<F, SPL, NT, TWO, UNI, NWX, 0, NFIX>(in, P);
}

template <int F, int SPL, int NT, int NWX = 1> __global__ PO_KERNEL_ATTR __launch_bounds__(NT) void polish_kernel(DevBatch in, DevParams P0) {
    static_assert(NWX == 1 || NWX == 4 || NWX == 5, "polish: one lane per chunk (one or several groups per lane)");
    using FX = Fast<F, SPL, NT, true, NWX>;
    extern __shared__ double smem[];
    const int b = in.order ? in.order[blockIdx.x] : perm_index(blockIdx.x, in.perm_bits, in.B);
    if ((unsigned)b >= (unsigned)in.B) return;
    if (in.out_info[b].status != PO_STATUS_SOLVED) return;
    DevParams P = P0;
    P.alpha = 1.0;
    FX fx(P, in, smem, b);
    typename FX::LS st;
    fx.load(st);
    for (int i = fx.tid; i < fx.L.total; i += NT) smem[i] = 0.0;
    __syncthreads();
    fx.scale_to_lds();
    if (fx.tid < kNVC) smem[fx.L.cst + kScSig + fx.tid] *= P.pol_delta / P.sigma;
    __syncthreads();
    fx.template state_io<false>(st, in.pol_state + (size_t)b * in.pol_stride);
    unsigned cls0[SPL];
#pragma unroll
    for (int q = 0; q < SPL; ++q) cls0[q] = st.cls[q];
    const unsigned clse0 = st.clse, clsc0 = st.clsc;
    fx.pol_init(st);
#pragma unroll
    for (int q = 0; q < SPL; ++q) st.cls[q] = kPolAllEq;
    st.clse = st.clsc = kPolAllEq;
    const double rho = 1.0 / (P.pol_delta * kRhoEqOverIneq);
    PolRes R = {0, 0, 0, 1, 0};
    {
        fx.pol_reset(st);
        fx.template factor_blocks_two<false, true>(st, rho);
        fx.factor_chain_two(st, rho);
        for (int it = 0; it <= P.pol_refine; ++it) {
            PO_FRESH_LANE_ID(fx);
            fx.template rhs_pass_two<false, false, true>(st, rho);
            PO_FRESH_LANE_ID(fx);
            fx.solve_two(st, rho, nullptr);
            PO_FRESH_LANE_ID(fx);
            (void)fx.template update_pass_two<false, false, false, true>(st, rho, false);
        }
        unsigned pcn[SPL], pcne, pcnc;
        R = fx.pol_eval(st, cls0, clse0, clsc0, P.pol_delta, pcn, pcne, pcnc);
    }
    po_info *oi = in.out_info + b;
    const double rp0 = oi->r_prim, rd0 = oi->r_dual;
    const bool ok = !R.bad && ((R.rp < rp0 && R.rd < rd0) || (R.rp < rp0 && rd0 < 1e-10) || (R.rd < rd0 && rp0 < 1e-10));
    if (ok) fx.output_pass(st);
    if (fx.tid == 0) {
        oi->status_polish = ok ? 1 : -1;
        if (ok) { oi->r_prim = R.rp; oi->r_dual = R.rd; oi->obj = R.obj; }
    }
}

constexpr int kFallbackGrid = 256;
template <int F, int SPL, int NT, int NWX = 1> __global__ PO_KERNEL_ATTR __launch_bounds__(NT) void newton_fallback_kernel(DevBatch in, DevParams P) {
    const int count = in.fb_list[0];
    const int rounds = P.ref_rounds > 1 ? P.ref_rounds : 1, rounds_total = rounds + P.ref_extra;
    DevBatch rb = in;
    rb.only_deferred = 0;
    for (int i = blockIdx.x; i < count; i += gridDim.x) {
        const int b = in.fb_list[1 + i];
        for (int r = 1; r < rounds_total; ++r) {
            __threadfence();
            __syncthreads();
            rb.round = r;
            solve_body<F, SPL, NT, true, false, NWX, 2>(rb, P, b);
        }
        __syncthreads();
    }
}

template <int F, int SPL, int NT, int NWX = 1, int PH = 1, int NFIX = 0> __global__ PO_KERNEL_ATTR __launch_bounds__(NT) void newton_kernel(DevBatch in, DevParams P) {
    using FX = Fast<F, SPL, NT, true, NWX, NFIX>;
    extern __shared__ double smem[];
#ifdef PO_NW_TRACE
    const long long tk0_ = __builtin_readcyclecounter();
#endif
    int b;
    if constexpr (PH == 2) {
        if ((int)blockIdx.x >= in.nw_list[0]) return;
        b = in.nw_list[1 + blockIdx.x];
    } else b = in.order ? in.order[blockIdx.x] : perm_index(blockIdx.x, in.perm_bits, in.B);
    if ((unsigned)b >= (unsigned)in.B) return;
    po_info *oi = in.out_info + b;
    const bool slicing = PH == 2 || P.ref_nw_slice > 0;
    if (oi->status != PO_STATUS_SOLVED) return;
    FX fx(P, in, smem, b);
    typename FX::LS st;
    fx.load(st);
    double *state = in.pol_state + (size_t)b * in.pol_stride;
    double *pstate = slicing ? in.nw_state + (size_t)b * in.nw_stride : nullptr, *pscal = slicing ? pstate + (size_t)FX::kParkDoubles * NT : nullptr;
    if constexpr (PH == 2) fx.template park_io<false>(st, pstate); else fx.template state_io<false>(st, state);
    for (int i = fx.tid; i < fx.L.total; i += NT) smem[i] = 0.0;
    __syncthreads();
    fx.scale_to_lds();
    const int lo_it = uni(oi->iters), lo_nref = uni(oi->n_refactor);
    const double lo_rho = uni(oi->rho), rp0 = uni(oi->r_prim), rd0 = uni(oi->r_dual);
    const int rounds = P.ref_rounds > 1 ? P.ref_rounds : 1, rounds_total = rounds + P.ref_extra;
    const bool last = 1 >= rounds_total;
#ifdef PO_NW_TRACE
    const long long tk1_ = __builtin_readcyclecounter();
#endif
    const RefineOut ro = refine_phase_newton<F, SPL, NT, NWX, PH, NFIX>(fx, st, P, lo_rho, rp0, rd0, slicing ? P.ref_nw_slice : 1 << 30, pscal, slicing ? in.nw_keys + b : nullptr);
    __syncthreads();
#ifdef PO_NW_TRACE
    const long long tk2_ = __builtin_readcyclecounter();
    if (fx.b == 0 && fx.tid == 0) printf("  dev kernel PH %d: entry %lld cycles (load, LDS set-up, state block), phase %lld (%d steps)\n", PH, tk1_ - tk0_, tk2_ - tk1_, ro.it);
#endif
    if constexpr (PH == 1) if (ro.parked) { fx.template park_io<true>(st, pstate); return; }
    const bool hand_back = !ro.stop && !last;
    if (ro.take) { if (hand_back || P.polish) fx.template state_io<true>(st, state); }
    else if (!hand_back) fx.template state_io<false>(st, state);
    if (hand_back) {
        if (fx.tid == 0) {
            oi->status = kStatusDeferred - 1; oi->iters = lo_it + ro.it; oi->status_polish = lo_it; oi->n_refactor = lo_nref + ro.nfac;
            if (ro.take) { oi->r_prim = ro.R.rp; oi->r_dual = ro.R.rd; oi->obj = ro.R.obj; }
            oi->status_refine = -1;
            in.fb_list[1 + atomicAdd(in.fb_list, 1)] = b;
        }
        return;
    }
    fx.output_pass(st);
    if (fx.tid == 0) {
        oi->iters = lo_it + ro.it; oi->n_refactor = lo_nref + ro.nfac;
        if (ro.take) { oi->r_prim = ro.R.rp; oi->r_dual = ro.R.rd; oi->obj = ro.R.obj; }
        oi->status_refine = ro.stop ? 1 : -1;
    }
}

template <int F> size_t lds_bytes_fast(int N, int C, int spl, bool two, int nt, int nwx = 1) { return sizeof(double) * (size_t)LayoutF<F>(N, C, spl, two, nt, (nwx == 2 || nwx == 3) ? 2 : 1, (nwx == 2 || nwx == 3) ? 2 * spl - (nwx == 3 ? 1 : 0) : 0, nwx == 4 ? spl : (nwx == 5 ? spl / 2 : 1)).total; }
```

path_optimizer_amd/csrc/po_handle.hpp:

```cpp
#pragma once
#include <hip/hip_runtime.h>

#include <mutex>
#include <vector>

#include "../../include/po_hip.h"
#include "po_launch.hpp"
#include "po_map.hpp"

#pragma GCC visibility push(hidden)

bool hip_ok(hipError_t e, const char *what);
#define HIP_TRY(x)                                   \
    do {                                             \
        if (!hip_ok((x), #x)) return PO_ERR_HIP;     \
    } while (0)
#define PO_TRY(x)                     \
    do {                              \
        const int rc_ = (x);          \
        if (rc_ != PO_OK) return rc_; \
    } while (0)

struct NoCopy {
    NoCopy() = default;
    NoCopy(const NoCopy &) = delete;
    NoCopy &operator=(const NoCopy &) = delete;
};
struct Stream : NoCopy {
    hipStream_t s = nullptr;
    ~Stream() { if (s) (void)hipStreamDestroy(s); }
};
struct Event : NoCopy {
    hipEvent_t e = nullptr;
    ~Event() { if (e) (void)hipEventDestroy(e); }
    operator hipEvent_t() const { return e; }
};
struct DevBuf : NoCopy {
    void *p = nullptr;
    size_t cap = 0;
    int ensure(size_t bytes) {
        if (bytes <= cap) return PO_OK;
        release();
        if (!hip_ok(hipMalloc(&p, bytes), "hipMalloc")) return PO_ERR_NOMEM;
        cap = bytes;
        return PO_OK;
    }
    void release() {
        if (p) (void)hipFree(p);
        p = nullptr;
        cap = 0;
    }
    ~DevBuf() { release(); }
};
struct HostBuf : NoCopy {
    void *p = nullptr;
    size_t cap = 0;
    int ensure(size_t bytes) {
        if (bytes <= cap) return PO_OK;
        release();
        if (!hip_ok(hipHostMalloc(&p, bytes, hipHostMallocDefault), "hipHostMalloc")) return PO_ERR_NOMEM;
        cap = bytes;
        return PO_OK;
    }
    void release() {
        if (p) (void)hipHostFree(p);
        p = nullptr;
        cap = 0;
    }
    ~HostBuf() { release(); }
};

#define PO_GUARDED_BY(m) __attribute__((guarded_by(m)))
#define PO_REQUIRES(m) __attribute__((requires_capability(m)))
#define PO_ACQUIRED_AFTER(m) __attribute__((acquired_after(m)))
class __attribute__((capability("mutex"))) Mutex : NoCopy {
    std::mutex m_;

public:
    void lock() __attribute__((acquire_capability())) { m_.lock(); }
    void unlock() __attribute__((release_capability())) { m_.unlock(); }
};
class __attribute__((scoped_lockable)) Lock : NoCopy {
    Mutex &m_;

public:
    explicit Lock(Mutex &m) __attribute__((acquire_capability(m))) : m_(m) { m_.lock(); }
    ~Lock() __attribute__((release_capability())) { m_.unlock(); }
};

struct po_handle_s {
    Mutex call_mu;
    Mutex mu PO_ACQUIRED_AFTER(call_mu);
    int device = 0;
    po_params params{};
    Stream own_stream;
    PO_GUARDED_BY(mu) hipStream_t stream = nullptr;
    Event ev0, ev1;
    Event evh[4];
    Event evp[2];
    PO_GUARDED_BY(mu) bool timed = false, timed_host = false, timed_phases = false;
    PO_GUARDED_BY(mu) double host_pack_ms = 0.0, host_unpack_ms = 0.0;
    PO_GUARDED_BY(call_mu) HostBuf pin_in, pin_out;
    PO_GUARDED_BY(mu) int host_threads = 0;
    PO_GUARDED_BY(mu) DevBuf pol_buf;
    PO_GUARDED_BY(mu) DevBuf fb_buf;
    PO_GUARDED_BY(mu) DevBuf nw_state_buf, nw_idx_buf;
    PO_GUARDED_BY(mu) bool nw_slice_forced = false;
    PO_GUARDED_BY(mu) int nw_last_B = 0;
    int wave_slots = 1024;
    PO_GUARDED_BY(mu) bool fixed_length = true;
    PO_GUARDED_BY(mu) int fixed_used = 0;
    PO_GUARDED_BY(mu) int dp_waves_used = 0;
    PO_GUARDED_BY(mu) int smooth_variant_used = 0;
    PO_GUARDED_BY(mu) int nw_slice = 8;
    PO_GUARDED_BY(mu) HostBuf fb_host;
    PO_GUARDED_BY(mu) bool env_identity = false, env_cycles = false, env_smooth_seq = false, env_smooth_nopad = false, env_smooth_debug = false, env_dp_one_wave = false;
    PO_GUARDED_BY(mu) int env_smooth_waves = 0;
    PO_GUARDED_BY(call_mu) DevBuf in_buf, out_buf, asm_buf, post_buf, bnd_buf, smooth_io, plan_io, plan_arena, plan_host, edt_io;
    PO_GUARDED_BY(mu) DevBuf scale_buf, dbg_buf, map_buf, coef_buf, smooth_buf, edt_buf;
    PO_GUARDED_BY(mu) DevBuf raster_buf;
    PO_GUARDED_BY(mu) DevBuf map_pos_buf, map_assign_buf;
    PO_GUARDED_BY(mu) po::DevMaps maps{};
    PO_GUARDED_BY(mu) DevBuf world_buf;
    PO_GUARDED_BY(mu) po_occupancy world{};
    PO_GUARDED_BY(mu) int world_outside = 0;
    PO_GUARDED_BY(mu) DevBuf select_buf;
};

inline int grow_after_sync(po_handle h, DevBuf &buf, size_t bytes) PO_REQUIRES(h->mu) {
    if (bytes <= buf.cap) return PO_OK;
    HIP_TRY(hipStreamSynchronize(h->stream));
    return buf.ensure(bytes);
}

inline bool assignment_covers(const po_handle_s *h, int B) PO_REQUIRES(h->mu) { return !h->maps.layer_of || B <= h->maps.n_assign; }

class Stage;
template <typename T> struct Slot {
    const Stage *stage = nullptr;
    size_t item = 0;
    T *ptr() const;
    operator T *() const { return ptr(); }
};
class Stage : NoCopy {
    struct Item { size_t off, bytes; const void *src; void *dst; };
    std::vector<Item> items_;
    size_t bytes_ = 0;
    char *base_ = nullptr;
    template <typename T> friend struct Slot;
    template <typename T> Slot<T> add(size_t n, const void *src, void *dst) {
        bytes_ = (bytes_ + 15) & ~(size_t)15;
        items_.push_back({bytes_, sizeof(T) * n, src, dst});
        bytes_ += sizeof(T) * n;
        return {this, items_.size() - 1};
    }

public:
    template <typename T> Slot<T> in(const T *host, size_t n) { return host ? add<T>(n, host, nullptr) : Slot<T>{}; }
    template <typename T> Slot<T> out(T *host, size_t n) { return add<T>(n, nullptr, host); }
    template <typename T> Slot<T> out_opt(T *host, size_t n) { return host ? out(host, n) : Slot<T>{}; }
    template <typename T> Slot<T> inout(T *host, size_t n) { return host ? add<T>(n, host, host) : Slot<T>{}; }
    template <typename T> Slot<T> scratch(size_t n) { return add<T>(n, nullptr, nullptr); }
    size_t bytes() const { return bytes_; }
    template <typename F> void each(F f) const {
        for (const Item &it : items_) f(it.off, it.bytes, it.src, it.dst);
    }
    int reserve(po_handle h, DevBuf &buf, bool after_sync = false) PO_REQUIRES(h->mu) {
        PO_TRY(after_sync ? grow_after_sync(h, buf, bytes_) : buf.ensure(bytes_));
        base_ = static_cast<char *>(buf.p);
        return PO_OK;
    }
    int copy_in(po_handle h) const PO_REQUIRES(h->mu) {
        for (const Item &it : items_)
            if (it.src) HIP_TRY(hipMemcpyAsync(base_ + it.off, it.src, it.bytes, hipMemcpyHostToDevice, h->stream));
        return PO_OK;
    }
    int upload(po_handle h, DevBuf &buf, bool after_sync = false) PO_REQUIRES(h->mu) {
        PO_TRY(reserve(h, buf, after_sync));
        return copy_in(h);
    }
    int copy_out(po_handle h) const PO_REQUIRES(h->mu) {
        for (const Item &it : items_)
            if (it.dst) HIP_TRY(hipMemcpyAsync(it.dst, base_ + it.off, it.bytes, hipMemcpyDeviceToHost, h->stream));
        HIP_TRY(hipStreamSynchronize(h->stream));
        return PO_OK;
    }
};
template <typename T> T *Slot<T>::ptr() const { return stage ? reinterpret_cast<T *>(stage->base_ + stage->items_[item].off) : nullptr; }

struct NoPrecheck {
    int operator()(po_handle) const { return PO_OK; }
};
template <typename Twin, typename Precheck = NoPrecheck>
int staged_call(po_handle h, Stage &S, DevBuf po_handle_s::*block, bool after_sync, Twin twin, Precheck precheck = Precheck{}) {
    Lock call(h->call_mu);
    {
        Lock g(h->mu);
        PO_TRY(precheck(h));
        HIP_TRY(hipSetDevice(h->device));
        PO_TRY(S.upload(h, h->*block, after_sync));
    }
    PO_TRY(twin());
    Lock g(h->mu);
    return S.copy_out(h);
}

inline bool spline_args_ok(const po_spline_in *in, bool need_length = true) {
    return in && in->B >= 0 && in->K >= 3 && (in->B == 0 || (in->knot_s && in->knot_x && in->knot_y && (in->length || !need_length)));
}
inline po::DevSpline make_dev_spline(const po_spline_in *in) {
    return po::DevSpline{in->B, in->K, in->knot_s, in->knot_x, in->knot_y, in->n_knots, in->length, nullptr};
}

#pragma GCC visibility pop
```

path_optimizer_amd/csrc/po_kernels.hip:

```cpp
#include "po_solve_common.hpp"

namespace po {

template <int F> __global__ __launch_bounds__(64) void assemble_kernel(DevBatch in, DevParams P, double *l, double *u, double *dyn) {
    using T = FormTraits<F>;
    extern __shared__ double smem[];
    const int b = blockIdx.x;
    Ctx<F> cx(P, in, smem, b);
    const int N = cx.N, C = cx.C;
    double *lb = l + (size_t)b * in.m, *ub = u + (size_t)b * in.m;
    for (int j = cx.lane; j < N; j += 64) {
        const StageIn si = cx.stage_in(j);
        AsmFn<F> fn{lb, ub, j, N, C, 0};
        local_rows<F>(si, P, fn);
        if (T::NEND && si.last) { fn.kind = 1; end_rows<F>(si, P, fn); }
        double bin[3];
        if (j == 0) cx.init_bounds(bin);
        else {
            const Dyn<F> d = cx.dyn(j - 1);
#pragma unroll
            for (int r = 0; r < T::NDYN; ++r) bin[r] = d.b[r];
            double *dd = dyn + ((size_t)b * (N - 1) + (j - 1)) * 3;
            if constexpr (F == F_K) { dd[0] = d.f[0][0]; dd[1] = d.f[1][1]; dd[2] = d.f[0][2]; }
            else { dd[0] = d.f[0][1]; dd[1] = d.f[1][0]; dd[2] = d.beta[2]; }
        }
#pragma unroll
        for (int r = 0; r < T::NDYN; ++r) { lb[T::NDYN * j + r] = bin[r]; ub[T::NDYN * j + r] = bin[r]; }
        if constexpr (F == F_K) {
            if (si.last) {  }
        }
    }
    if constexpr (T::HAS_U)
        for (int c = cx.lane; c < C; c += 64) {
            AsmFn<F> fn{lb, ub, c, N, C, 2};
            const double mkp = (F == F_KPC) ? in.max_kp[cx.po + c] : 0.0;
            ctl_rows<F>(mkp, fn);
        }
}

}

namespace po {
__global__ void finalize_status_kernel(po_info *info, int B) {
    const int b = blockIdx.x * blockDim.x + threadIdx.x;
    if (b < B && info[b].status <= kStatusDeferred) { info[b].status = PO_STATUS_UNSOLVED; info[b].status_polish = 0; }
}
__global__ void mark_unavailable_kernel(po_info *info, int B, int refine, int polish) {
    const int b = blockIdx.x * blockDim.x + threadIdx.x;
    if (b < B) {
        if (refine) info[b].status_refine = PO_NOT_AVAILABLE;
        if (polish) info[b].status_polish = PO_NOT_AVAILABLE;
    }
}
}
extern "C" hipError_t po_launch_mark_unavailable(po_info *info, int B, int refine, int polish, hipStream_t st) {
    hipLaunchKernelGGL(po::mark_unavailable_kernel, dim3((B + 255) / 256), dim3(256), 0, st, info, B, refine, polish);
    return hipGetLastError();
}
namespace po {
namespace {
using Entry = hipError_t(int, const Shape &, size_t, const DevBatch *, const DevParams *, hipStream_t);
struct Object { Entry *entry; int form, kind, groups; };
#define PO_X(name, form, kind, groups) {&name, form, kind, groups},
const Object kObjects[] = {PO_SOLVE_OBJECTS(PO_X)};
#undef PO_X
template <int F, bool TWO, int SPL, int NT, int NWX> struct RowSizes { static constexpr int state = 0, park = 0; };
template <int F, int SPL, int NT, int NWX> struct RowSizes<F, true, SPL, NT, NWX> {
    static constexpr int state = Fast<F, SPL, NT, true, NWX>::kStateDoubles * NT, park = Fast<F, SPL, NT, true, NWX>::kParkDoubles * NT + kNwParkScalars;
};
hipError_t call(int form, int kind, int launch, const SolveShape &r, const DevBatch *in, const DevParams *P, hipStream_t st) {
    if (!r.nt || r.lds > kLdsLimit) return hipErrorInvalidValue;
    const Shape s{.nt = r.nt, .spl = r.spl, .two = r.two != 0, .nwx = r.nwx};
    for (const Object &o : kObjects)
        if (o.form == form && o.kind == kind && (o.groups & r.group) && o.entry) return o.entry(launch, s, r.lds, in, P, st);
    return hipErrorNotSupported;
}
bool fixed(const SolveShape &r, const DevBatch *in) { return r.fixed && in->fixed_len && in->n_points == nullptr; }
}
}
extern "C" hipError_t po_launch_solve(int form, const po::SolveShape *s, const po::DevBatch *in, const po::DevParams *P, hipStream_t st) {
    using namespace po;
    hipError_t e;
    DevBatch copy = *in;
    copy.only_deferred = 0;
    if (s->uni && (e = call(form, fixed(*s, in) ? kObjFixUni : kObjUni, kLaunchSolve, *s, &copy, P, st)) != hipSuccess) return e;
    copy.only_deferred = s->uni ? 1 : 0;
    return call(form, kObjGen, kLaunchSolve, *s, &copy, P, st);
}
extern "C" hipError_t po_launch_finalize_status(po_info *info, int B, hipStream_t st) {
    hipLaunchKernelGGL(po::finalize_status_kernel, dim3((B + 255) / 256), dim3(256), 0, st, info, B);
    return hipGetLastError();
}

static hipError_t launch_two_level(int form, int launch, const po::SolveShape *s, const po::DevBatch *in, const po::DevParams *P, hipStream_t st) {
    using namespace po;
    if (!s->two) return hipErrorInvalidValue;
    if (launch == kLaunchPolish && !s->polish) return hipSuccess;
    const int kind = (launch == kLaunchNewton && fixed(*s, in)) ? (in->nw_phase == 2 ? kObjFixNewton2 : kObjFixNewton1) : (launch == kLaunchPolish ? kObjGen : kObjNewton);
    return call(form, kind, launch, *s, in, P, st);
}
extern "C" hipError_t po_launch_newton(int form, const po::SolveShape *s, const po::DevBatch *in, const po::DevParams *P, hipStream_t st) { return launch_two_level(form, po::kLaunchNewton, s, in, P, st); }
extern "C" hipError_t po_launch_newton_fallback(int form, const po::SolveShape *s, const po::DevBatch *in, const po::DevParams *P, hipStream_t st) { return launch_two_level(form, po::kLaunchFallback, s, in, P, st); }
extern "C" hipError_t po_launch_polish(int form, const po::SolveShape *s, const po::DevBatch *in, const po::DevParams *P, hipStream_t st) { return launch_two_level(form, po::kLaunchPolish, s, in, P, st); }
namespace po {
constexpr int kNwSortThreads = 256;
__global__ __launch_bounds__(kNwSortThreads) void nw_sort_kernel(const int *keys, int B, int *list) {
    __shared__ int cnt[kNwKeys][kNwSortThreads + 1];
    __shared__ int rowbase[kNwKeys];
    const int t = threadIdx.x, per = (B + kNwSortThreads - 1) / kNwSortThreads, lo = t * per, hi = min(B, lo + per);
    constexpr int kCache = 16;
    int kc[kCache];
#pragma unroll
    for (int i = 0; i < kCache; ++i) kc[i] = (lo + i < hi) ? keys[lo + i] : -1;
#pragma unroll
    for (int k = 0; k < kNwKeys; ++k) cnt[k][t] = 0;
#pragma unroll
    for (int i = 0; i < kCache; ++i)
        if (kc[i] >= 0) cnt[kc[i] < kNwKeys ? kc[i] : kNwKeys - 1][t] += 1;
    for (int b = lo + kCache; b < hi; ++b) {
        const int k = keys[b];
        if (k >= 0) cnt[k < kNwKeys ? k : kNwKeys - 1][t] += 1;
    }
    __syncthreads();
    {
        constexpr int kPerLane = kNwSortThreads / 64, kWaves = kNwSortThreads / 64;
        const int lane = t & 63, wv = t >> 6;
        for (int k = wv; k < kNwKeys; k += kWaves) {
            int v[kPerLane], sum = 0;
#pragma unroll
            for (int i = 0; i < kPerLane; ++i) { v[i] = cnt[k][lane * kPerLane + i]; sum += v[i]; }
            int incl = sum;
#pragma unroll
            for (int d = 1; d < 64; d <<= 1) { const int o = __shfl_up(incl, d, 64); if (lane >= d) incl += o; }
            int run = incl - sum;
#pragma unroll
            for (int i = 0; i < kPerLane; ++i) { cnt[k][lane * kPerLane + i] = run; run += v[i]; }
            if (lane == 63) cnt[k][kNwSortThreads] = incl;
        }
    }
    __syncthreads();
    if (t < kNwKeys) {
        int run = 0;
        for (int j = kNwKeys - 1; j > t; --j) run += cnt[j][kNwSortThreads];
        rowbase[t] = run;
        if (t == 0) list[0] = run + cnt[0][kNwSortThreads];
    }
    __syncthreads();
    auto place = [&](int b, int k) {
        const int kk = k < kNwKeys ? k : kNwKeys - 1;
        const int pos = rowbase[kk] + cnt[kk][t];
        cnt[kk][t] += 1;
        list[1 + pos] = b;
    };
#pragma unroll
    for (int i = 0; i < kCache; ++i)
        if (kc[i] >= 0) place(lo + i, kc[i]);
    for (int b = lo + kCache; b < hi; ++b) {
        const int k = keys[b];
        if (k >= 0) place(b, k);
    }
}

}
extern "C" hipError_t po_launch_nw_sort(const int *keys, int B, int *list, hipStream_t st) {
    hipLaunchKernelGGL(po::nw_sort_kernel, dim3(1), dim3(po::kNwSortThreads), 0, st, keys, B, list);
    return hipGetLastError();
}
extern "C" int po_resolve_solve(int form, int N, int C, int keep, po::SolveShape *r) {
    using namespace po;
    *r = SolveShape{};
    r->lds = (size_t)1 << 30;
    Shape s;
    if (!resolve_shape(form, N, form == F_K ? 0 : C, keep, &s)) return 0;
    r->nt = s.nt; r->spl = s.spl; r->two = s.two; r->nwx = s.nwx;
    r->lds = lds_of(form, N, C, s);
    r->group = group_of(form, s);
#ifdef PO_DEV_HEADLINE
    if (form == F_KP && r->group) r->group = ~0;
#endif
    r->uni = form == F_K ? has_uni_variant<F_K>(s) : has_uni_variant<F_KP>(s);
    r->polish = has_polish_kernel(s);
    bool listed = false;
#define PO_X(N_) listed = listed || N == N_;
    PO_FIXED_LIST(PO_X)
#undef PO_X
    r->fixed = listed && is_fixed_shape(form, N, C, keep, s) && r->lds <= kLdsLimit;
#define PO_X(F_, TWO_, SPL_, NT_, NWX_, G_) if (form == F_ && is_shape(s, TWO_, SPL_, NT_, NWX_)) { r->state_doubles = RowSizes<F_, TWO_, SPL_, NT_, NWX_>::state; r->park_doubles = RowSizes<F_, TWO_, SPL_, NT_, NWX_>::park; }
    PO_SHAPE_ROWS(PO_X)
#undef PO_X
    return 1;
}
static po::SolveShape resolved(int form, int N, int C, int keep) { po::SolveShape r; po_resolve_solve(form, N, C, keep, &r); return r; }
extern "C" size_t po_lds_bytes(int form, int N, int C, int keep) { return resolved(form, N, C, keep).lds; }
extern "C" int po_shape_threads(int form, int N, int C, int keep) { return resolved(form, N, C, keep).nt; }
extern "C" int po_polish_state_doubles(int form, int N, int C, int keep) { return resolved(form, N, C, keep).state_doubles; }
extern "C" int po_newton_park_doubles(int form, int N, int C, int keep) { return resolved(form, N, C, keep).park_doubles; }
extern "C" int po_has_polish_kernel(int form, int N, int C, int keep) { return resolved(form, N, C, keep).polish; }
extern "C" int po_has_fixed_length(int form, int N, int C, int keep) { return resolved(form, N, C, keep).fixed; }

extern "C" hipError_t po_launch_scale(int form, const po::DevBatch *in, const po::DevParams *P, int passes, double *sc, int *nw_keys, int *fb_count, hipStream_t st) {
    using namespace po;
    const int bs = 64, gs = (in->B + bs - 1) / bs;
    if (form == F_KP) hipLaunchKernelGGL(scale_kernel<F_KP>, dim3(gs), dim3(bs), 0, st, *in, *P, passes, sc, nw_keys, fb_count);
    else if (form == F_KPC) hipLaunchKernelGGL(scale_kernel<F_KPC>, dim3(gs), dim3(bs), 0, st, *in, *P, passes, sc, nw_keys, fb_count);
    else hipLaunchKernelGGL(scale_kernel<F_K>, dim3(gs), dim3(bs), 0, st, *in, *P, passes, sc, nw_keys, fb_count);
    return hipGetLastError();
}

extern "C" hipError_t po_launch_assemble(int form, const po::DevBatch *in, const po::DevParams *P, double *l, double *u, double *dyn, hipStream_t st) {
    using namespace po;
    if (form == F_KP) hipLaunchKernelGGL(assemble_kernel<F_KP>, dim3(in->B), dim3(64), 0, st, *in, *P, l, u, dyn);
    else if (form == F_KPC) hipLaunchKernelGGL(assemble_kernel<F_KPC>, dim3(in->B), dim3(64), 0, st, *in, *P, l, u, dyn);
    else hipLaunchKernelGGL(assemble_kernel<F_K>, dim3(in->B), dim3(64), 0, st, *in, *P, l, u, dyn);
    return hipGetLastError();
}
```

path_optimizer_amd/csrc/po_launch.hpp:

```cpp
#pragma once
#include <hip/hip_runtime.h>

#include "../../include/po_hip.h"

namespace po {
struct DevBatch; struct DevParams;
struct Shape;
enum { kObjUni, kObjGen, kObjNewton, kObjFixUni, kObjFixNewton1, kObjFixNewton2 };
enum { kLaunchSolve, kLaunchNewton, kLaunchFallback, kLaunchPolish };
enum { kGrpLane = 1, kGrpSplit = 2, kGrpMulti = 4, kGrpW56 = 8, kGrpW7 = 16, kGrpW8 = 32, kGrpOne = 64 };
struct SolveShape {
    int nt, spl, two, nwx;
    size_t lds;
    int group;
    int uni, polish, fixed;
    int state_doubles, park_doubles;
};
constexpr size_t kLdsLimit = 160 * 1024;
struct DevMap; struct DevMaps; struct DevCar; struct DevBounds; struct DevSpline; struct DevSearch;
struct DevResample; struct PlanGate; struct PlanRows; struct DevSelect; struct DevSpeed; struct DevDynamic; struct DevStplan; struct DevNudge;
struct DevTrajectory; struct DevAgentSets;
struct DevSmooth;
}

extern "C" {
int po_resolve_solve(int form, int N, int C, int keep, po::SolveShape *s);
hipError_t po_launch_solve(int form, const po::SolveShape *s, const po::DevBatch *in, const po::DevParams *P, hipStream_t st);
hipError_t po_launch_newton(int form, const po::SolveShape *s, const po::DevBatch *in, const po::DevParams *P, hipStream_t st);
hipError_t po_launch_newton_fallback(int form, const po::SolveShape *s, const po::DevBatch *in, const po::DevParams *P, hipStream_t st);
hipError_t po_launch_polish(int form, const po::SolveShape *s, const po::DevBatch *in, const po::DevParams *P, hipStream_t st);
hipError_t po_launch_finalize_status(po_info *info, int B, hipStream_t st);
hipError_t po_launch_mark_unavailable(po_info *info, int B, int refine, int polish, hipStream_t st);
hipError_t po_launch_nw_sort(const int *keys, int B, int *list, hipStream_t st);
hipError_t po_launch_scale(int form, const po::DevBatch *in, const po::DevParams *P, int passes, double *sc, int *nw_keys, int *fb_count, hipStream_t st);
hipError_t po_launch_assemble(int form, const po::DevBatch *in, const po::DevParams *P, double *l, double *u, double *dyn, hipStream_t st);
size_t po_lds_bytes(int form, int N, int C, int keep);
int po_shape_threads(int form, int N, int C, int keep);
int po_polish_state_doubles(int form, int N, int C, int keep);
int po_newton_park_doubles(int form, int N, int C, int keep);
int po_has_polish_kernel(int form, int N, int C, int keep);
int po_has_fixed_length(int form, int N, int C, int keep);

int po_plan_solve(int form, int N, int keep, int B, int ragged, int refine, int refine_rounds, int refine_extra_rounds, int refine_chain, int polish, int nw_slice,
                  int slice_forced, int fixed_on, int wave_slots, int *out);

#define PO_SOLVE_OBJECTS(X)                                                     \
    X(po_solve_kp_uni, F_KP, kObjUni, kGrpLane | kGrpSplit | kGrpMulti)         \
    X(po_solve_kp, F_KP, kObjGen, kGrpLane | kGrpSplit | kGrpMulti | kGrpOne)   \
    X(po_solve_kp_w_uni, F_KP, kObjUni, kGrpW56 | kGrpW7 | kGrpW8)              \
    X(po_solve_kp_w, F_KP, kObjGen, kGrpW56 | kGrpW7 | kGrpW8)                  \
    X(po_solve_kpc_uni, F_KPC, kObjUni, kGrpLane)                               \
    X(po_solve_kpc, F_KPC, kObjGen, kGrpLane | kGrpOne)                         \
    X(po_solve_k_uni, F_K, kObjUni, kGrpLane)                                   \
    X(po_solve_k, F_K, kObjGen, kGrpLane | kGrpOne)                             \
    X(po_newton_kp, F_KP, kObjNewton, kGrpLane)                                 \
    X(po_newton_kp_b, F_KP, kObjNewton, kGrpSplit)                              \
    X(po_newton_kp_c, F_KP, kObjNewton, kGrpMulti)                              \
    X(po_newton_kp_w1, F_KP, kObjNewton, kGrpW56)                               \
    X(po_newton_kp_w2, F_KP, kObjNewton, kGrpW7)                                \
    X(po_newton_kp_w3, F_KP, kObjNewton, kGrpW8)                                \
    X(po_newton_kpc, F_KPC, kObjNewton, kGrpLane)                               \
    X(po_newton_k, F_K, kObjNewton, kGrpLane)                                   \
    X(po_solve_kp_fix_uni, F_KP, kObjFixUni, kGrpLane)                          \
    X(po_newton_kp_fix1, F_KP, kObjFixNewton1, kGrpLane)                        \
    X(po_newton_kp_fix2, F_KP, kObjFixNewton2, kGrpLane)
#if defined(PO_DEV_HEADLINE) && !defined(PO_ENTRY)
#define PO_OBJECT_ATTR __attribute__((weak))
#else
#define PO_OBJECT_ATTR
#endif
#define PO_X(name, form, kind, groups) \
    PO_OBJECT_ATTR hipError_t name(int launch, const po::Shape &s, size_t lds, const po::DevBatch *in, const po::DevParams *P, hipStream_t st);
PO_SOLVE_OBJECTS(PO_X)
#undef PO_X

hipError_t po_launch_postcheck(const po::DevMaps *m, const po::DevCar *c, int B, int N, const int *n_points, const double *states, const po_info *info, int *n_valid,
                               int *ok, hipStream_t st);
hipError_t po_launch_densify(const po::DevMaps *m, const po::DevCar *c, int B, int N, const int *n_points, const double *states, const po_info *info, double spacing,
                             int M, double *out, int *n_out, int *ok, hipStream_t st);
hipError_t po_launch_map_sample(const po::DevMaps *m, int layer, int n, const double *xy, double *dist, int *inside, hipStream_t st);
hipError_t po_launch_bounds(const po::DevMaps *m, const po::DevBounds *in, double *bounds, int *n_valid, hipStream_t st);
hipError_t po_launch_resample(const po::DevSpline *in, const po::DevResample *r, hipStream_t st);
hipError_t po_launch_limits(int B, int N, const int *n_points, const double *v, const double *a, double *max_k, double *max_kp, double mu, double rate, hipStream_t st);
hipError_t po_launch_dp_search(const po::DevMaps *m, const po::DevSpline *in, const po::DevSearch *q, int one_wave, int *waves_used, hipStream_t st);
size_t po_dp_lds_bytes(int K, int L);
size_t po_spline_lds_bytes(int K);
hipError_t po_launch_bspline(int B, int W, const int *n_way, const double *wx, const double *wy, int M, double *x, double *y, double *s, int *n_samples, hipStream_t st);
hipError_t po_launch_segment_raw(const po::DevSpline *in, int P, double *x, double *y, double *s, double *angle, double *k, int *n_points, hipStream_t st);
hipError_t po_launch_post_project(const po::DevSpline *in, int L, const int *n_layers, const double *layer_s, const double *off, double *x, double *y, double *s,
                                  double *length_out, hipStream_t st);
hipError_t po_launch_segment_init(const po::DevSpline *in, const double *start, int start_stride, const double *goal, int goal_stride, int exact, double *init, int *ok,
                                  hipStream_t st);
hipError_t po_launch_plan_gate(const po::PlanGate *g, hipStream_t st);
hipError_t po_launch_plan_gather(const po::PlanRows *r, hipStream_t st);
hipError_t po_launch_plan_scatter(const po::PlanRows *r, hipStream_t st);
hipError_t po_launch_plan_clear(int B, int N, const int *stage, double *states, po_info *info, hipStream_t st);

hipError_t po_launch_smooth(const po::DevSmooth *a, int *variant_used, hipStream_t st);
size_t po_smooth_lds_bytes(int kind, int P);
size_t po_smooth_scratch_doubles(int kind, int P);
int po_smooth_blocked(int kind, int P);

hipError_t po_launch_edt(const unsigned char *cells, int M, int sx, int sy, float res, void *scratch, float *out, hipStream_t st);
size_t po_edt_scratch_bytes(int M, int sx, int sy);
int po_edt_max_side(void);
int po_edt_max_images(void);

hipError_t po_launch_raster(const po_obstacle_lists *lists, int M, const double *pos_xy, unsigned char *out, hipStream_t st);

hipError_t po_launch_scene(const po_scene *scene, int M, const double *pos_xy, const po_occupancy *world, int outside_occupied, unsigned char *img, hipStream_t st);

hipError_t po_launch_select(const po::DevMaps *m, const po::DevCar *c, const po::DevSelect *a, hipStream_t st);

hipError_t po_launch_speed(const po::DevMaps *m, const po::DevCar *c, const po::DevSpeed *a, hipStream_t st);

hipError_t po_launch_dynamic(const po::DevCar *c, const po::DevDynamic *a, hipStream_t st);

hipError_t po_launch_stplan(const po::DevCar *c, const po::DevStplan *a, hipStream_t st);

hipError_t po_launch_nudge(const po::DevNudge *a, hipStream_t st);

hipError_t po_launch_trajectory(const po::DevTrajectory *a, hipStream_t st);

hipError_t po_launch_agentsets(const po::DevAgentSets *a, hipStream_t st);
}
```

path_optimizer_amd/csrc/po_scale.hpp:

```cpp
#pragma once
#include "po_device.hpp"

namespace po {

constexpr int kNVC = 8;
constexpr int kNRC = 24;
constexpr int kScStride = 64;
constexpr int kScW = 0, kScE = 24, kScSig = 48, kScCD = 56, kScC = 63;
constexpr int kKEndRow = 11, kKEndVar = 6, kScAlt = 12;
constexpr double kMinScaling = 1e-4, kMaxScaling = 1e4;

struct ClassModel {
    int nr;
    double Pmax[kNVC], cnt[kNVC];
    double a[kNRC][kNVC];
    int tgt[kNRC];
};

struct PatFn {
    ClassModel *M;
    int base;
    template <int MASK, class TL, class TU> __host__ __device__ void row(int r, double c0, double c1, double c2, double c3, double c4, TL, TU) {
        double *a = M->a[base + r];
        a[0] = c0; a[1] = c1; a[2] = c2; a[3] = c3; a[4] = c4;
    }
};
struct PatCtlFn {
    ClassModel *M;
    int base;
    template <int MASK, class TL, class TU> __host__ __device__ void row(int r, double, double, double c2, double c3, double, TL, TU) {
        double *a = M->a[base + r];
        a[5] = c2; a[6] = c3;
    }
};

__device__ inline double limit_scaling(double v) {
    v = v < kMinScaling ? 1.0 : v;
    return v > kMaxScaling ? kMaxScaling : v;
}

template <int F> __device__ void class_scaling(const DevParams &P, int N, int keep, int C, double ds_nom, int passes, double *out ) {
#pragma clang fp contract(off)
    using T = FormTraits<F>;
    ClassModel M;
    M.nr = T::NLOC + T::NDYN + T::NCTL + T::NEND;
    for (int r = 0; r < kNRC; ++r) { M.tgt[r] = -1; for (int v = 0; v < kNVC; ++v) M.a[r][v] = 0; }
    StageIn s;
    for (int c = 0; c < 4; ++c) { s.lb[c] = -1; s.ub[c] = 1; }
    s.maxk = 0; s.elo = -kInf; s.ehi = kInf; s.j = 0; s.N = N; s.last = 0;
    PatFn pf{&M, 0};
    local_rows<F>(s, P, pf);
    const Dyn<F> d = make_dyn<F>(0.0, ds_nom, P);
    for (int r = 0; r < T::NDYN; ++r) {
        double *a = M.a[T::NLOC + r];
        a[0] = d.f[r][0]; a[1] = d.f[r][1]; a[2] = d.f[r][2]; a[5] = d.beta[r];
        M.tgt[T::NLOC + r] = dyn_tau<F>(r);
    }
    if constexpr (T::NCTL > 0) { PatCtlFn cf{&M, T::NLOC + T::NDYN}; ctl_rows<F>(0.0, cf); }
    if constexpr (T::NEND > 0) { PatFn ef{&M, T::NLOC + T::NDYN + T::NCTL}; end_rows<F>(s, P, ef); }
    if constexpr (F == F_K) {
        static_assert(T::NLOC + T::NDYN == kKEndRow && kScAlt + T::NLOC <= 24, "K end classes");
        M.a[kKEndRow][kKEndVar] = M.a[2][2];
        M.a[T::NLOC + 0][kKEndVar] = M.a[T::NLOC + 0][2];
        M.nr = kKEndRow + 1;
    }
    for (int v = 0; v < kNVC; ++v) { M.Pmax[v] = 0; M.cnt[v] = 0; }
    M.Pmax[0] = P.w_dev; M.Pmax[2] = (F == F_K) ? P.w_c + 2 * P.w_cr : P.w_c; M.Pmax[3] = P.w_s1;
    M.cnt[0] = N; M.cnt[1] = N; M.cnt[2] = N; M.cnt[3] = N;
    if constexpr (F == F_K) { M.Pmax[kKEndVar] = P.w_c + P.w_cr; M.cnt[kKEndVar] = N - 1 < 2 ? N - 1 : 2; M.cnt[2] = N - 1 - M.cnt[kKEndVar]; }
    if constexpr (F == F_KP) { M.Pmax[5] = P.w_u; M.cnt[5] = C; M.Pmax[7] = P.w_s1; M.cnt[7] = N; }
    if constexpr (F == F_KPC) { M.Pmax[4] = P.w_s2; M.cnt[4] = N; M.Pmax[5] = P.w_u; M.cnt[5] = C; M.Pmax[6] = P.w_su; M.cnt[6] = C; M.cnt[7] = N - C; }
    double Dv[kNVC], Er[kNRC], c = 1.0, ntot = 0;
    for (int v = 0; v < kNVC; ++v) { Dv[v] = 1.0; ntot += M.cnt[v]; }
    for (int r = 0; r < kNRC; ++r) Er[r] = 1.0;
    for (int pass = 0; pass < passes; ++pass) {
        double cn[kNVC], rn[kNRC];
        for (int v = 0; v < kNVC; ++v) cn[v] = fabs(c * M.Pmax[v] * Dv[v] * Dv[v]);
        for (int r = 0; r < M.nr; ++r) {
            double rmax = 0;
            for (int v = 0; v < kNVC; ++v) {
                const double a = fabs(Er[r] * M.a[r][v] * Dv[v]);
                if (a > rmax) rmax = a;
                if (a > cn[v]) cn[v] = a;
            }
            if (M.tgt[r] >= 0) {
                const double a = fabs(Er[r] * Dv[M.tgt[r]]);
                if (a > rmax) rmax = a;
                if (a > cn[M.tgt[r]]) cn[M.tgt[r]] = a;
            }
            rn[r] = rmax;
        }
        for (int v = 0; v < kNVC; ++v) Dv[v] *= 1.0 / sqrt(limit_scaling(cn[v]));
        for (int r = 0; r < M.nr; ++r) Er[r] *= 1.0 / sqrt(limit_scaling(rn[r]));
        double mean = 0;
        for (int v = 0; v < kNVC; ++v) mean += M.cnt[v] * fabs(c * M.Pmax[v] * Dv[v] * Dv[v]);
        mean /= ntot;
        double ct = mean > 1.0 ? mean : 1.0;
        ct = 1.0 / limit_scaling(ct);
        c *= ct;
    }
    for (int i = 0; i < kScStride; ++i) out[i] = 0;
    for (int r = 0; r < kNRC; ++r) { out[kScW + r] = Er[r] * Er[r] / c; out[kScE + r] = Er[r]; }
    for (int v = 0; v < 7; ++v) { out[kScSig + v] = P.sigma / (c * Dv[v] * Dv[v]); out[kScCD + v] = c * Dv[v]; }
    if constexpr (F == F_K) {
        for (int r = 0; r < T::NLOC; ++r) { out[kScW + kScAlt + r] = out[kScW + (r == 2 ? kKEndRow : r)]; out[kScE + kScAlt + r] = out[kScE + (r == 2 ? kKEndRow : r)]; }
    }
    out[kScC] = c;
}

template <int F> __global__ void scale_kernel(DevBatch in, DevParams P, int passes, double *sc, int *nw_keys, int *fb_count) {
    const int b = blockIdx.x * blockDim.x + threadIdx.x;
    if (b >= in.B) return;
    if (nw_keys) nw_keys[b] = -1;
    if (fb_count && b == 0) *fb_count = 0;
    const double *s = in.ref_s + (size_t)b * in.N;
    int N = in.N, C = in.C;
    if (in.n_points) { N = in.n_points[b]; N = N < 2 ? 2 : (N > in.N ? in.N : N); C = (F == F_K) ? N - 1 : (N + in.keep - 2) / in.keep; }
    double ds_nom = 0;
    for (int i = 1; i < N && i < 10; ++i) ds_nom = fmax(ds_nom, __dsub_rn(s[i], s[i - 1]));
    class_scaling<F>(P, N, in.keep, C, ds_nom, passes, sc + (size_t)b * kScStride);
}

}
```

path_optimizer_amd/csrc/po_solve.cpp:

```cpp
#include <hip/hip_runtime.h>

#include <algorithm>
#include <chrono>
#include <cmath>
#include <cstdio>
#include <cstring>
#include <thread>
#include <vector>

#include "../../include/po_hip.h"
#include "po_device.hpp"
#include "po_handle.hpp"
#include "po_launch.hpp"

namespace {
struct CopySeg { char *dst; const char *src; size_t bytes; };
void parallel_copy(const std::vector<CopySeg> &segs, int nthr) {
    std::vector<CopySeg> pieces;
    const size_t kPiece = (size_t)2 << 20;
    for (const CopySeg &sg : segs)
        for (size_t o = 0; o < sg.bytes; o += kPiece) pieces.push_back({sg.dst + o, sg.src + o, std::min(kPiece, sg.bytes - o)});
    if (nthr <= 1 || pieces.size() <= 1) {
        for (const CopySeg &pc : pieces) std::memcpy(pc.dst, pc.src, pc.bytes);
        return;
    }
    nthr = (int)std::min<size_t>((size_t)nthr, pieces.size());
    std::vector<std::thread> th;
    for (int t = 1; t < nthr; ++t)
        th.emplace_back([&pieces, t, nthr] { for (size_t i = (size_t)t; i < pieces.size(); i += (size_t)nthr) std::memcpy(pieces[i].dst, pieces[i].src, pieces[i].bytes); });
    for (size_t i = 0; i < pieces.size(); i += (size_t)nthr) std::memcpy(pieces[i].dst, pieces[i].src, pieces[i].bytes);
    for (std::thread &t : th) t.join();
}

po::DevParams make_dev_params(const po_params &p, int form, int keep) {
    po::DevParams D;
    D.d1 = p.d[0]; D.d2 = p.d[1]; D.d3 = p.d[2]; D.d4 = p.d[3];
    if (form == PO_K) {
        D.w_dev = p.k_w_dev; D.w_c = p.k_w_curv; D.w_cr = p.k_w_curv_rate; D.w_s1 = p.w_slack; D.w_s2 = 0; D.w_u = 0; D.w_su = 0;
    } else {
        D.w_dev = p.w_dev; D.w_c = p.w_curv; D.w_cr = p.w_curv_rate; D.w_s1 = p.w_slack;
        D.w_s2 = (form == PO_KPC) ? p.w_k_slack : 0.0;
        D.w_u = keep * p.w_curv_rate;
        D.w_su = (form == PO_KPC) ? p.w_kp_slack * keep : 0.0;
    }
    D.margin = p.margin;
    D.kmax = std::tan(p.max_steer) / p.wheel_base;
    D.max_steer = p.max_steer;
    D.wheel_base = p.wheel_base;
    D.sigma = p.sigma; D.alpha = p.alpha; D.rho0 = p.rho0; D.eps_abs = p.eps_abs; D.eps_rel = p.eps_rel;
    D.eps_pinf = p.eps_prim_inf; D.adapt_tol = p.adapt_tol;
    D.max_iter = p.max_iter; D.check_every = p.check_every; D.adapt_every = p.adapt_every;
    D.end_heading = p.constraint_end_heading;
    D.polish = p.polish; D.pol_delta = p.polish_delta > 0 ? p.polish_delta : 1e-6; D.pol_refine = p.polish_refine_iter < 0 ? 0 : p.polish_refine_iter;
    D.refine = p.refine; D.ref_eps = p.refine_eps; D.ref_rounds = p.refine_rounds;
    D.ref_extra = (p.refine && p.refine_extra_rounds > 0) ? p.refine_extra_rounds : 0;
    D.ref_nw_rho = p.refine_newton_rho > 0 ? std::min(p.refine_newton_rho, po::kRhoMax) : 100.0;
    D.ref_nw_rho_eq = p.refine_newton_rho_eq > 0 ? std::min(p.refine_newton_rho_eq, 1e8) : 1e4;
    D.ref_nw_rho_max = p.refine_newton_rho_max > 0 ? std::min(p.refine_newton_rho_max, po::kRhoMax) : 1e5;
    D.ref_nw_rho_eq_max = p.refine_newton_rho_eq_max > 0 ? std::min(p.refine_newton_rho_eq_max, 1e8) : (p.refine_newton_rho_eq_max < 0 ? 1e6 : 0.0);
    D.ref_ls_tol = p.refine_ls_tol > 0 ? p.refine_ls_tol : 1e-4;
    D.ref_nw_final = p.refine_newton_final; D.ref_nw_esc = p.refine_newton_escalate; D.ref_nw_slice = 0; D.ref_ls_max = p.refine_ls_max > 0 ? p.refine_ls_max : 30; D.ref_nw_max = p.refine_newton_max > 0 ? p.refine_newton_max : 300;
    return D;
}

struct Dims { int n, m, C; po::SolveShape shape; };
int validate(const po_batch_in *in, Dims *d) {
    if (!in || in->B < 0) return PO_ERR_INVALID;
    PO_TRY(po_problem_dims(in->formulation, in->N, in->keep, &d->n, &d->m, &d->C));
    if (!in->ref_x || !in->ref_y || !in->ref_z || !in->ref_k || !in->ref_s || !in->bounds || !in->x0 || !in->goal_z) return PO_ERR_INVALID;
    if (in->formulation == PO_KPC && (!in->max_k || !in->max_kp)) return PO_ERR_INVALID;
    po_resolve_solve(in->formulation, in->N, d->C, in->keep, &d->shape);
    return d->shape.lds > po::kLdsLimit ? PO_ERR_UNSUPPORTED : PO_OK;
}

po::DevBatch fill_dev_batch(const po_handle_s *h, const po_batch_in *in, const po_batch_out *out, const Dims &d) PO_REQUIRES(h->mu) {
    po::DevBatch D{};
    D.B = in->B; D.N = in->N; D.keep = in->keep; D.C = d.C;
    D.ref_x = in->ref_x; D.ref_y = in->ref_y; D.ref_z = in->ref_z; D.ref_k = in->ref_k; D.ref_s = in->ref_s;
    D.bounds = in->bounds; D.x0 = in->x0; D.goal_z = in->goal_z; D.max_k = in->max_k; D.max_kp = in->max_kp;
    D.n_points = in->n_points;
    D.order = in->order;
    D.out_states = out ? out->states : nullptr;
    D.out_info = out ? out->info : nullptr;
    D.out_x = out ? out->x : nullptr;
    if (!h->env_identity && in->B > 8)
        while ((1 << D.perm_bits) < in->B) ++D.perm_bits;
    D.n = d.n; D.m = d.m;
    return D;
}

struct SolveSchedule {
    bool state;
    bool split, sliced;
    bool polish, fixed;
    bool no_refine, no_polish;
    bool read_back;
    int warm_decades;
};
SolveSchedule plan_solve(const po_params &p, const po::SolveShape &s, int B, bool ragged, int nw_slice, bool slice_forced, bool fixed_on, int wave_slots) {
    SolveSchedule q{};
    const int rounds = p.refine_rounds > 1 ? p.refine_rounds : 1;
    const int rounds_total = rounds + ((p.refine && p.refine_extra_rounds > 0) ? p.refine_extra_rounds : 0);
    q.state = (p.polish || p.refine) && s.state_doubles > 0;
    q.polish = p.polish && q.state && s.polish;
    q.split = p.refine == 2 && q.state && rounds_total < 32;
    q.sliced = q.split && nw_slice > 0 && (slice_forced || (B >= 2 * wave_slots && s.nt == 64));
    q.fixed = fixed_on && !ragged && s.fixed;
    q.no_refine = p.refine == 2 && !q.split;
    q.no_polish = p.polish && !q.polish;
    q.read_back = p.refine_chain != 3;
    q.warm_decades = rounds - 1;
    return q;
}

int provision(po_handle h, const po::SolveShape &s, size_t B, SolveSchedule *q) PO_REQUIRES(h->mu) {
    if (h->env_cycles) PO_TRY(h->dbg_buf.ensure(sizeof(long long) * 16 * B));
    PO_TRY(h->scale_buf.ensure(sizeof(double) * 64 * B));
    if (q->state) PO_TRY(h->pol_buf.ensure(sizeof(double) * (size_t)s.state_doubles * B));
    if (!q->split) return PO_OK;
    PO_TRY(h->fb_buf.ensure(sizeof(int) * (B + 1)));
    PO_TRY(h->fb_host.ensure(64));
    if (q->sliced && (h->nw_state_buf.ensure(sizeof(double) * (size_t)s.park_doubles * B) || h->nw_idx_buf.ensure(sizeof(int) * (2 * B + 1)))) {
        (void)hipGetLastError();
        h->nw_state_buf.release();
        q->sliced = false;
    }
    h->nw_last_B = q->sliced ? (int)B : 0;
    return PO_OK;
}

int enqueue(po_handle h, int form, const po::SolveShape &s, const SolveSchedule &q, po::DevBatch &D, po::DevParams &P) PO_REQUIRES(h->mu) {
    const int B = D.B;
    if (h->env_cycles) {
        D.dbg_cycles = static_cast<long long *>(h->dbg_buf.p);
        HIP_TRY(hipMemsetAsync(D.dbg_cycles, 0, sizeof(long long) * 16 * (size_t)B, h->stream));
    }
    D.scale = static_cast<double *>(h->scale_buf.p);
    if (q.state) { D.pol_state = static_cast<double *>(h->pol_buf.p); D.pol_stride = s.state_doubles; }
    HIP_TRY(hipEventRecord(h->ev0, h->stream));
    h->timed_phases = false;
    HIP_TRY(po_launch_scale(form, &D, &P, h->params.scaling, static_cast<double *>(h->scale_buf.p), q.sliced ? static_cast<int *>(h->nw_idx_buf.p) : nullptr,
                            q.split ? static_cast<int *>(h->fb_buf.p) : nullptr, h->stream));
    if (q.split) {
        po::DevParams P1 = P;
        for (int r = 0; r < q.warm_decades; ++r) { P1.eps_abs *= 10.0; P1.eps_rel *= 10.0; }
        D.nw_follows = 1;
        HIP_TRY(po_launch_solve(form, &s, &D, &P1, h->stream));
        D.nw_follows = 0;
        HIP_TRY(hipEventRecord(h->evp[0], h->stream));
        D.fb_list = static_cast<int *>(h->fb_buf.p);
        if (q.sliced) {
            D.nw_state = static_cast<double *>(h->nw_state_buf.p); D.nw_stride = s.park_doubles;
            D.nw_keys = static_cast<int *>(h->nw_idx_buf.p); D.nw_list = D.nw_keys + B;
            P.ref_nw_slice = h->nw_slice;
            D.nw_phase = 1;
            HIP_TRY(po_launch_newton(form, &s, &D, &P, h->stream));
            HIP_TRY(po_launch_nw_sort(D.nw_keys, B, D.nw_list, h->stream));
            D.nw_phase = 2;
            HIP_TRY(po_launch_newton(form, &s, &D, &P, h->stream));
            D.nw_phase = 0;
        } else {
            HIP_TRY(po_launch_newton(form, &s, &D, &P, h->stream));
        }
        HIP_TRY(hipEventRecord(h->evp[1], h->stream));
        h->timed_phases = true;
        bool need_fb = true;
        hipStreamCaptureStatus cap_st = hipStreamCaptureStatusNone;
        const bool capturing = hipStreamIsCapturing(h->stream, &cap_st) == hipSuccess && cap_st != hipStreamCaptureStatusNone;
        if (q.read_back && !capturing) {
            volatile int *cnt = static_cast<volatile int *>(h->fb_host.p);
            *cnt = -1;
            HIP_TRY(hipMemcpyAsync(const_cast<int *>(cnt), D.fb_list, sizeof(int), hipMemcpyDeviceToHost, h->stream));
            const auto ts0 = std::chrono::steady_clock::now();
            unsigned spins = 0;
            while (*cnt == -1) {
                if ((++spins & 1023u) == 0 && std::chrono::steady_clock::now() - ts0 > std::chrono::milliseconds(20)) { HIP_TRY(hipStreamSynchronize(h->stream)); break; }
#if defined(__x86_64__) || defined(__i386__)
                __builtin_ia32_pause();
#else
                std::this_thread::yield();
#endif
            }
            need_fb = *cnt != 0;
        }
        if (need_fb) HIP_TRY(po_launch_newton_fallback(form, &s, &D, &P, h->stream));
        HIP_TRY(po_launch_finalize_status(D.out_info, B, h->stream));
    } else {
        HIP_TRY(po_launch_solve(form, &s, &D, &P, h->stream));
    }
    if (q.polish) HIP_TRY(po_launch_polish(form, &s, &D, &P, h->stream));
    if (q.no_refine || q.no_polish) HIP_TRY(po_launch_mark_unavailable(D.out_info, B, q.no_refine, q.no_polish, h->stream));
    HIP_TRY(hipEventRecord(h->ev1, h->stream));
    h->timed = true;
    return PO_OK;
}

int dump_cycles(po_handle h, const po::DevBatch &D, int form) PO_REQUIRES(h->mu) {
    long long c4[16];
    HIP_TRY(hipStreamSynchronize(h->stream));
    HIP_TRY(hipMemcpy(c4, D.dbg_cycles, sizeof(c4), hipMemcpyDeviceToHost));
    std::vector<long long> all(16 * (size_t)D.B);
    HIP_TRY(hipMemcpy(all.data(), D.dbg_cycles, sizeof(long long) * all.size(), hipMemcpyDeviceToHost));
    long long nf = 0, nb = 0;
    double worst = 0;
    for (int b = 0; b < D.B; ++b) {
        nf += all[16 * (size_t)b + 13]; nb += all[16 * (size_t)b + 14];
        double w; std::memcpy(&w, &all[16 * (size_t)b + 15], sizeof(w)); worst = std::fmax(worst, w);
    }
    std::fprintf(stderr, "[po] batch of %d (form %d, N %d, keep %d): %lld scan factorisations, %lld fell back to the sequential chain; worst relative disagreement scan vs recursion %.3e\n", D.B, form, D.N, D.keep, nf, nb, worst);
    std::fprintf(stderr, "[po] path0 cycles: rhs %lld solve %lld update %lld over %lld iterations | solve phases F1 %lld F2 %lld F3B1 %lld B2 %lld B3 %lld | first factorisation: blocks %lld chain %lld | uniform row classes %lld | scan factorisations %lld, fell back to the sequential chain %lld\n",
                 c4[0], c4[1], c4[2], c4[3], c4[4], c4[5], c4[6], c4[7], c4[8], c4[10], c4[11], c4[12], c4[13], c4[14]);
    return PO_OK;
}
}

extern "C" {

int po_plan_solve(int form, int N, int keep, int B, int ragged, int refine, int refine_rounds, int refine_extra_rounds, int refine_chain, int polish, int nw_slice,
                  int slice_forced, int fixed_on, int wave_slots, int *out) {
    if (!out) return PO_ERR_INVALID;
    int C;
    PO_TRY(po_problem_dims(form, N, keep, nullptr, nullptr, &C));
    po::SolveShape s;
    po_resolve_solve(form, N, C, keep, &s);
    if (s.lds > po::kLdsLimit) return PO_ERR_UNSUPPORTED;
    po_params p{};
    p.refine = refine; p.refine_rounds = refine_rounds; p.refine_extra_rounds = refine_extra_rounds; p.refine_chain = refine_chain; p.polish = polish;
    const SolveSchedule q = plan_solve(p, s, B, ragged != 0, nw_slice, slice_forced != 0, fixed_on != 0, wave_slots);
    for (int v : {(int)q.split, (int)q.state, (int)q.polish, (int)q.sliced, (int)q.fixed, (int)q.no_refine, (int)q.no_polish, (int)q.read_back, q.warm_decades}) *out++ = v;
    return PO_OK;
}

int po_solve_batch_device(po_handle h, const po_batch_in *in, const po_batch_out *out) {
    if (!h || !out || !out->states || !out->info) return PO_ERR_INVALID;
    Dims d;
    PO_TRY(validate(in, &d));
    if (in->B == 0) return PO_OK;
    Lock g(h->mu);
    HIP_TRY(hipSetDevice(h->device));
    h->timed_host = false;
    po::DevParams P = make_dev_params(h->params, in->formulation, in->keep);
    po::DevBatch D = fill_dev_batch(h, in, out, d);
    const po::SolveShape &s = d.shape;
    SolveSchedule q = plan_solve(h->params, s, in->B, in->n_points != nullptr, h->nw_slice, h->nw_slice_forced, h->fixed_length, h->wave_slots);
    h->fixed_used = D.fixed_len = q.fixed;
    PO_TRY(provision(h, s, (size_t)in->B, &q));
    PO_TRY(enqueue(h, in->formulation, s, q, D, P));
    return h->env_cycles ? dump_cycles(h, D, in->formulation) : PO_OK;
}

int po_solve_batch(po_handle h, const po_batch_in *in, const po_batch_out *out) {
    if (!h || !out || !out->states || !out->info) return PO_ERR_INVALID;
    Dims d;
    PO_TRY(validate(in, &d));
    if (in->B == 0) return PO_OK;
    HIP_TRY(hipSetDevice(h->device));
    const size_t B = in->B, N = in->N;
    const bool kpc = in->formulation == PO_KPC;
    if (in->n_points)
        for (size_t b = 0; b < B; ++b)
            if (in->n_points[b] < 2 || in->n_points[b] > in->N) return PO_ERR_INVALID;
    if (in->order) {
        std::vector<char> seen(B, 0);
        for (size_t b = 0; b < B; ++b) {
            const int v = in->order[b];
            if (v < 0 || (size_t)v >= B || seen[(size_t)v]) return PO_ERR_INVALID;
            seen[(size_t)v] = 1;
        }
    }
    Stage I, O;
    const Slot<double> rx = I.in(in->ref_x, B * N), ry = I.in(in->ref_y, B * N), rz = I.in(in->ref_z, B * N), rk = I.in(in->ref_k, B * N), rs = I.in(in->ref_s, B * N);
    const Slot<double> bd = I.in(in->bounds, B * N * 8), x0 = I.in(in->x0, B * 3), gz = I.in(in->goal_z, B);
    const Slot<double> mk = I.in(kpc ? in->max_k : nullptr, B * N), mkp = I.in(kpc ? in->max_kp : nullptr, B * N);
    const Slot<int> np = I.in(in->n_points, B), ord = I.in(in->order, B);
    const Slot<double> os = O.out(out->states, B * N * 5), ox = O.out_opt(out->x, B * (size_t)d.n);
    const Slot<po_info> oi = O.out(out->info, B);
    Lock call(h->call_mu);
    hipStream_t st;
    int nthr;
    {
        Lock g(h->mu);
        int rc;
        if ((rc = I.reserve(h, h->in_buf)) || (rc = O.reserve(h, h->out_buf)) || (rc = h->pin_in.ensure(I.bytes())) || (rc = h->pin_out.ensure(O.bytes()))) return rc;
        st = h->stream;
        nthr = h->host_threads > 0 ? h->host_threads : (int)std::min(8u, std::max(1u, std::thread::hardware_concurrency()));
    }
    char *dev = static_cast<char *>(h->in_buf.p), *pin = static_cast<char *>(h->pin_in.p);
    std::vector<CopySeg> segs;
    I.each([&](size_t off, size_t bytes, const void *src, void *) { segs.push_back({pin + off, static_cast<const char *>(src), bytes}); });
    double pack_ms, unpack_ms;
    HIP_TRY(hipEventRecord(h->evh[0], st));
    {
        const auto t0 = std::chrono::steady_clock::now();
        const size_t kSlice = (size_t)32 << 20;
        for (size_t lo = 0; lo < I.bytes(); lo += kSlice) {
            const size_t hi = std::min(I.bytes(), lo + kSlice);
            std::vector<CopySeg> cur;
            for (const CopySeg &sg : segs) {
                const size_t s0 = (size_t)(sg.dst - pin), s1 = s0 + sg.bytes;
                const size_t a0 = std::max(s0, lo), a1 = std::min(s1, hi);
                if (a0 < a1) cur.push_back({pin + a0, sg.src + (a0 - s0), a1 - a0});
            }
            parallel_copy(cur, nthr);
            HIP_TRY(hipMemcpyAsync(dev + lo, pin + lo, hi - lo, hipMemcpyHostToDevice, st));
        }
        pack_ms = std::chrono::duration<double, std::milli>(std::chrono::steady_clock::now() - t0).count();
    }
    HIP_TRY(hipEventRecord(h->evh[1], st));
    po_batch_in din = *in;
    din.ref_x = rx; din.ref_y = ry; din.ref_z = rz; din.ref_k = rk; din.ref_s = rs; din.bounds = bd; din.x0 = x0; din.goal_z = gz; din.n_points = np; din.order = ord;
    if (kpc) { din.max_k = mk; din.max_kp = mkp; }
    const po_batch_out dout{os, oi, ox};
    PO_TRY(po_solve_batch_device(h, &din, &dout));
    char *pout = static_cast<char *>(h->pin_out.p);
    HIP_TRY(hipMemcpyAsync(pout, h->out_buf.p, O.bytes(), hipMemcpyDeviceToHost, st));
    HIP_TRY(hipEventRecord(h->evh[2], st));
    HIP_TRY(hipStreamSynchronize(st));
    {
        const auto t0 = std::chrono::steady_clock::now();
        std::vector<CopySeg> us;
        O.each([&](size_t off, size_t bytes, const void *, void *dst) { us.push_back({static_cast<char *>(dst), pout + off, bytes}); });
        parallel_copy(us, nthr);
        unpack_ms = std::chrono::duration<double, std::milli>(std::chrono::steady_clock::now() - t0).count();
    }
    Lock g(h->mu);
    h->host_pack_ms = pack_ms; h->host_unpack_ms = unpack_ms;
    h->timed_host = true;
    return PO_OK;
}

int po_last_phase_ms(po_handle h, float *ms8) {
    if (!h || !ms8) return PO_ERR_INVALID;
    Lock g(h->mu);
    if (!h->timed) return PO_ERR_INVALID;
    for (int i = 0; i < 8; ++i) ms8[i] = 0.0f;
    HIP_TRY(hipEventSynchronize(h->ev1));
    HIP_TRY(hipEventElapsedTime(&ms8[1], h->ev0, h->ev1));
    if (h->timed_host) {
        HIP_TRY(hipEventSynchronize(h->evh[2]));
        HIP_TRY(hipEventElapsedTime(&ms8[0], h->evh[0], h->evh[1]));
        HIP_TRY(hipEventElapsedTime(&ms8[2], h->ev1, h->evh[2]));
        ms8[3] = (float)h->host_pack_ms; ms8[4] = (float)h->host_unpack_ms;
    }
    if (h->timed_phases) {
        HIP_TRY(hipEventElapsedTime(&ms8[5], h->ev0, h->evp[0]));
        HIP_TRY(hipEventElapsedTime(&ms8[6], h->evp[0], h->evp[1]));
        HIP_TRY(hipEventElapsedTime(&ms8[7], h->evp[1], h->ev1));
    }
    return PO_OK;
}

int po_last_kernel_ms(po_handle h, float *ms) {
    if (!h || !ms) return PO_ERR_INVALID;
    Lock g(h->mu);
    if (!h->timed) return PO_ERR_INVALID;
    HIP_TRY(hipEventSynchronize(h->ev1));
    HIP_TRY(hipEventElapsedTime(ms, h->ev0, h->ev1));
    return PO_OK;
}

int po_assemble_batch(po_handle h, const po_batch_in *in, double *l, double *u, double *dyn) {
    if (!h || !l || !u || !dyn) return PO_ERR_INVALID;
    if (in && in->n_points) return PO_ERR_INVALID;
    Dims d;
    PO_TRY(validate(in, &d));
    if (in->B == 0) return PO_OK;
    const size_t B = in->B, N = in->N;
    const bool kpc = in->formulation == PO_KPC;
    Stage S;
    const Slot<double> rx = S.in(in->ref_x, B * N), ry = S.in(in->ref_y, B * N), rz = S.in(in->ref_z, B * N), rk = S.in(in->ref_k, B * N), rs = S.in(in->ref_s, B * N);
    const Slot<double> bd = S.in(in->bounds, B * N * 8), x0 = S.in(in->x0, B * 3), gz = S.in(in->goal_z, B);
    const Slot<double> mk = S.in(kpc ? in->max_k : nullptr, B * N), mkp = S.in(kpc ? in->max_kp : nullptr, B * N);
    const size_t out_from = (S.bytes() + 15) & ~(size_t)15;
    const Slot<double> dl = S.out(l, B * (size_t)d.m), du = S.out(u, B * (size_t)d.m), dd = S.out(dyn, B * (N - 1) * 3);
    return staged_call(h, S, &po_handle_s::asm_buf, false, [&]() -> int {
        Lock g(h->mu);
        po_batch_in din = *in;
        din.ref_x = rx; din.ref_y = ry; din.ref_z = rz; din.ref_k = rk; din.ref_s = rs; din.bounds = bd; din.x0 = x0; din.goal_z = gz;
        if (kpc) { din.max_k = mk; din.max_kp = mkp; }
        HIP_TRY(hipMemsetAsync(dl, 0, S.bytes() - out_from, h->stream));
        const po::DevParams P = make_dev_params(h->params, in->formulation, in->keep);
        const po::DevBatch D = fill_dev_batch(h, &din, nullptr, d);
        HIP_TRY(po_launch_assemble(in->formulation, &D, &P, dl, du, dd, h->stream));
        return PO_OK;
    });
}

int po_scaling_batch(po_handle h, const po_batch_in *in, double *out) {
    if (!h || !out) return PO_ERR_INVALID;
    if (in && in->n_points) return PO_ERR_INVALID;
    Dims d;
    PO_TRY(validate(in, &d));
    if (in->B == 0) return PO_OK;
    const size_t B = in->B, N = in->N;
    Stage S;
    const Slot<double> rs = S.in(in->ref_s, B * N), sc = S.out(out, 64 * B);
    return staged_call(h, S, &po_handle_s::asm_buf, false, [&]() -> int {
        Lock g(h->mu);
        po_batch_in din = *in;
        din.ref_s = rs;
        const po::DevParams P = make_dev_params(h->params, in->formulation, in->keep);
        const po::DevBatch D = fill_dev_batch(h, &din, nullptr, d);
        HIP_TRY(po_launch_scale(in->formulation, &D, &P, h->params.scaling, sc, nullptr, nullptr, h->stream));
        return PO_OK;
    });
}

}
```

path_optimizer_amd/csrc/po_solve_form.hip:

```cpp
#include "po_solve_common.hpp"

#ifndef PO_ENTRY
#error "compile with -DPO_ENTRY=<an object of PO_SOLVE_OBJECTS (po_launch.hpp)>"
#endif
#define PO_STR2(x) #x
#define PO_STR(x) PO_STR2(x)

namespace {
using namespace po;
struct Object { int form, kind, groups; };
constexpr bool same(const char *a, const char *b) { return *a == *b && (!*a || same(a + 1, b + 1)); }
constexpr Object me() {
#define PO_X(name, form, kind, groups) if (same(#name, PO_STR(PO_ENTRY))) return {form, kind, groups};
    PO_SOLVE_OBJECTS(PO_X)
#undef PO_X
    return {-1, -1, 0};
}
static_assert(me().form >= 0, "PO_ENTRY names no object of PO_SOLVE_OBJECTS");
#ifdef PO_REF
static_assert(me().kind == kObjNewton || me().kind == kObjFixNewton1 || me().kind == kObjFixNewton2, "-DPO_REF=3 is for the Newton objects");
#else
static_assert(me().kind != kObjNewton && me().kind != kObjFixNewton1 && me().kind != kObjFixNewton2, "the Newton objects build with -DPO_REF=3");
#endif
[[maybe_unused]] constexpr bool holds(int G, bool two, int spl, int nt, int nwx, int g) {
#ifdef PO_DEV_HEADLINE
#ifndef PO_DEV_SPL
#define PO_DEV_SPL 4
#endif
#ifndef PO_DEV_NWX
#define PO_DEV_NWX 1
#endif
#ifndef PO_DEV_NT
#define PO_DEV_NT 64
#endif
    return two && spl == PO_DEV_SPL && nt == PO_DEV_NT && nwx == PO_DEV_NWX;
#else
    return (G & g) != 0;
#endif
}
template <int F, int G, bool UNI> hipError_t launch_rows(int launch, const Shape &s, size_t lds, const DevBatch *in, const DevParams *P, hipStream_t st) {
#define PO_X(F_, TWO_, SPL_, NT_, NWX_, G_)                                                                                                     \
    if constexpr (F == F_ && holds(G, TWO_, SPL_, NT_, NWX_, G_) && (TWO_ || !UNI)) {                                                           \
        if (is_shape(s, TWO_, SPL_, NT_, NWX_)) return launch1(&solve_kernel_fast<F, SPL_, NT_, TWO_, TWO_ && UNI, NWX_>, in, P, NT_, lds, st); \
    }
    if (launch == kLaunchSolve) { PO_SHAPE_ROWS(PO_X) }
#undef PO_X
#define PO_X(F_, TWO_, SPL_, NT_, NWX_, G_)                                                                                                     \
    if constexpr (!UNI && F == F_ && TWO_ && holds(G, TWO_, SPL_, NT_, NWX_, G_) && has_polish_kernel(Shape{NT_, SPL_, TWO_, NWX_})) {          \
        if (is_shape(s, TWO_, SPL_, NT_, NWX_)) return launch1(&polish_kernel<F, SPL_, NT_, NWX_>, in, P, NT_, lds, st);                         \
    }
    if (launch == kLaunchPolish) { PO_SHAPE_ROWS(PO_X) }
#undef PO_X
    return hipErrorNotSupported;
}
template <int F, int G, bool FB> hipError_t launch_newton(const Shape &s, size_t lds, const DevBatch *in, const DevParams *P, hipStream_t st) {
#define PO_X(F_, TWO_, SPL_, NT_, NWX_, G_)                                                                                                     \
    if constexpr (F == F_ && TWO_ && holds(G, TWO_, SPL_, NT_, NWX_, G_)) {                                                                     \
        if (is_shape(s, TWO_, SPL_, NT_, NWX_)) {                                                                                               \
            if constexpr (FB) return launch_grid(&newton_fallback_kernel<F, SPL_, NT_, NWX_>, in, P, kFallbackGrid, NT_, lds, st);              \
            else if (in->nw_phase == 2) return launch1(&newton_kernel<F, SPL_, NT_, NWX_, 2>, in, P, NT_, lds, st);                             \
            else return launch1(&newton_kernel<F, SPL_, NT_, NWX_, 1>, in, P, NT_, lds, st);                                                    \
        }                                                                                                                                       \
    }
    PO_SHAPE_ROWS(PO_X)
#undef PO_X
    return hipErrorNotSupported;
}
template <int F, int KIND> hipError_t launch_fixed(const DevBatch *in, const DevParams *P, size_t lds, hipStream_t st) {
#define PO_X(N_)                                                                                                                                \
    if (in->N == N_) {                                                                                                                          \
        if constexpr (KIND == kObjFixUni) return launch1(&solve_kernel_fast<F, kFixSpl, kFixNt, true, true, 1, N_>, in, P, kFixNt, lds, st);    \
        else return launch1(&newton_kernel<F, kFixSpl, kFixNt, 1, KIND == kObjFixNewton2 ? 2 : 1, N_>, in, P, kFixNt, lds, st);                 \
    }
    PO_FIXED_LIST(PO_X)
#undef PO_X
    return hipErrorNotSupported;
}
template <int F, int KIND, int G> hipError_t entry(int launch, const Shape &s, size_t lds, const DevBatch *in, const DevParams *P, hipStream_t st) {
    if constexpr (KIND == kObjUni || KIND == kObjGen) return launch_rows<F, G, KIND == kObjUni>(launch, s, lds, in, P, st);
    else if constexpr (KIND == kObjNewton) {
        if (launch == kLaunchNewton) return launch_newton<F, G, false>(s, lds, in, P, st);
        if (launch == kLaunchFallback) return launch_newton<F, G, true>(s, lds, in, P, st);
        return hipErrorNotSupported;
    } else return launch_fixed<F, KIND>(in, P, lds, st);
}
}
extern "C" hipError_t PO_ENTRY(int launch, const po::Shape &s, size_t lds, const po::DevBatch *in, const po::DevParams *P, hipStream_t st) {
    return entry<me().form, me().kind, me().groups>(launch, s, lds, in, P, st);
}
```

Before: 1.207 million.

## Split Newton refine into constant-row-class kernel for standard paths

Adds a select kernel that flags paths whose bound row classes are all the standard location/control classes. Those paths run a specialized Newton kernel with compile-time constant classes, and the rest run the general one. The sort is extended to build separate parked lists for the second phase. This is meant to cut per-row class branching and register pressure for the common case, at the cost of an extra select launch, an extra kernel launch per phase, and more index bookkeeping.

```diff
diff --git a/path_optimizer_amd/binding.py b/path_optimizer_amd/binding.py
--- a/path_optimizer_amd/binding.py
+++ b/path_optimizer_amd/binding.py
@@ -40,7 +40,7 @@
 
 _ENV_DEBUG = {"PO_IDENTITY_ORDER": "identity_order", "PO_DEBUG_CYCLES": "debug_cycles", "PO_SMOOTH_SEQ": "smooth_seq",
               "PO_SMOOTH_WAVES": "smooth_waves", "PO_SMOOTH_NOPAD": "smooth_nopad", "PO_SMOOTH_DEBUG": "smooth_debug", "PO_DP_ONE_WAVE": "dp_one_wave", "PO_NEWTON_SLICE": "newton_slice",
-              "PO_FIXED_LENGTH": "fixed_length"}
+              "PO_FIXED_LENGTH": "fixed_length", "PO_FIXED_CLASSES": "fixed_classes"}
 
 
 def lib():
diff --git a/path_optimizer_amd/csrc/po_capi.cpp b/path_optimizer_amd/csrc/po_capi.cpp
--- a/path_optimizer_amd/csrc/po_capi.cpp
+++ b/path_optimizer_amd/csrc/po_capi.cpp
@@ -152,6 +152,7 @@
     else if (k == "debug_cycles") h->env_cycles = value != 0;
     else if (k == "newton_slice") { h->nw_slice = value > 0 ? (int)value : 0; h->nw_slice_forced = value > 0; }
     else if (k == "fixed_length") h->fixed_length = value != 0;
+    else if (k == "fixed_classes") h->fixed_classes = value != 0;
     else if (k == "smooth_seq") h->env_smooth_seq = value != 0;
     else if (k == "smooth_waves") h->env_smooth_waves = value;
     else if (k == "smooth_nopad") h->env_smooth_nopad = value != 0;
@@ -199,6 +200,16 @@
         *value = c;
         return PO_OK;
     }
+    if (k == "fixed_classes_used") {
+        *value = 0;
+        if (!h->nw_idx_buf.p || h->std_flag_at < 0 || h->std_B <= 0) return PO_OK;
+        HIP_TRY(hipSetDevice(h->device));
+        HIP_TRY(hipStreamSynchronize(h->stream));
+        std::vector<int> flag((size_t)h->std_B);
+        HIP_TRY(hipMemcpy(flag.data(), static_cast<int *>(h->nw_idx_buf.p) + h->std_flag_at, sizeof(int) * flag.size(), hipMemcpyDeviceToHost));
+        for (int f : flag) *value += f != 0;
+        return PO_OK;
+    }
     if (k == "newton_parked") {
         *value = -1;
         if (!h->nw_idx_buf.p || h->nw_last_B <= 0) return PO_OK;
@@ -207,6 +218,10 @@
         int c = 0;
         HIP_TRY(hipMemcpy(&c, static_cast<int *>(h->nw_idx_buf.p) + h->nw_last_B, sizeof(int), hipMemcpyDeviceToHost));
         *value = c;
+        if (h->std_left2_at >= 0) {
+            HIP_TRY(hipMemcpy(&c, static_cast<int *>(h->nw_idx_buf.p) + h->std_left2_at, sizeof(int), hipMemcpyDeviceToHost));
+            *value += c;
+        }
         return PO_OK;
     }
     if (k == "newton_list_ok") {
@@ -215,20 +230,27 @@
         HIP_TRY(hipSetDevice(h->device));
         HIP_TRY(hipStreamSynchronize(h->stream));
         const int B = h->nw_last_B;
-        std::vector<int> kl(2 * (size_t)B + 1);
+        const bool two_lists = h->std_left2_at >= 0;
+        std::vector<int> kl(two_lists ? (size_t)h->std_left2_at + (size_t)B + 1 : 2 * (size_t)B + 1);
         HIP_TRY(hipMemcpy(kl.data(), h->nw_idx_buf.p, sizeof(int) * kl.size(), hipMemcpyDeviceToHost));
-        const int *keys = kl.data(), *list = kl.data() + B;
-        const int n = list[0];
-        int parked = 0;
+        const int *keys = kl.data();
+        int parked = 0, listed = 0;
         for (int b = 0; b < B; ++b) parked += keys[b] >= 0;
-        bool ok = n == parked;
+        bool ok = true;
         std::vector<char> seen((size_t)B, 0);
-        for (int i = 0; ok && i < n; ++i) {
-            const int b = list[1 + i];
-            ok = b >= 0 && b < B && keys[b] >= 0 && !seen[(size_t)b];
-            if (ok) seen[(size_t)b] = 1;
-            if (ok && i > 0) { const int a = list[i]; ok = keys[a] > keys[b] || (keys[a] == keys[b] && a < b); }
+        for (const int *list : {kl.data() + B, two_lists ? kl.data() + h->std_left2_at : nullptr}) {
+            if (!list) continue;
+            const int n = list[0];
+            ok = ok && n >= 0 && n <= B;
+            for (int i = 0; ok && i < n; ++i) {
+                const int b = list[1 + i];
+                ok = b >= 0 && b < B && keys[b] >= 0 && !seen[(size_t)b];
+                if (ok) seen[(size_t)b] = 1;
+                if (ok && i > 0) { const int a = list[i]; ok = keys[a] > keys[b] || (keys[a] == keys[b] && a < b); }
+            }
+            listed += n;
         }
+        ok = ok && listed == parked;
         *value = ok ? 1 : 0;
         return PO_OK;
     }
diff --git a/path_optimizer_amd/csrc/po_device.hpp b/path_optimizer_amd/csrc/po_device.hpp
--- a/path_optimizer_amd/csrc/po_device.hpp
+++ b/path_optimizer_amd/csrc/po_device.hpp
@@ -57,6 +57,19 @@
     int nw_follows;
     int fixed_len;
 };
+constexpr unsigned kStdClsLoc = 0u, kStdClsCtl = 2u;
+struct StdLists {
+    int *left1;
+    int *left2;
+    int *order;
+    int *flag;
+};
+constexpr size_t std_left2_index(size_t B) { return 3 * B + 1; }
+constexpr size_t std_flag_index(size_t B) { return 5 * B + 2; }
+constexpr size_t std_lists_ints(size_t B) { return std_flag_index(B) + B; }
+__host__ __device__ inline StdLists std_lists(int *nw_keys, int B) {
+    return {nw_keys + 2 * B + 1, nw_keys + std_left2_index(B), nw_keys + 4 * B + 2, nw_keys + std_flag_index(B)};
+}
 
 template <int F> struct FormTraits;
 template <> struct FormTraits<F_KP> {
diff --git a/path_optimizer_amd/csrc/po_fast.inc b/path_optimizer_amd/csrc/po_fast.inc
--- a/path_optimizer_amd/csrc/po_fast.inc
+++ b/path_optimizer_amd/csrc/po_fast.inc
@@ -3820,7 +3820,7 @@
 struct RefineOut { bool take, stop; int it, nfac; Resid R; bool parked; };
 constexpr int kNwParkScalars = 12;
 constexpr int kNwStagnation = 8;
-template <int F, int SPL, int NT, int NWX, int PH = 0, int NFIX = 0>
+template <int F, int SPL, int NT, int NWX, int PH = 0, int NFIX = 0, bool CK = false>
 __device__ __forceinline__ RefineOut refine_phase_newton(Fast<F, SPL, NT, true, NWX, NFIX> &fx, typename Fast<F, SPL, NT, true, NWX, NFIX>::LS &st, const DevParams &P, double rho_solve, double rp0, double rd0,
                                                          int slice = 0, double *park = nullptr, int *park_key = nullptr) {
     constexpr bool resume = PH == 2;
@@ -3831,11 +3831,17 @@
         for (int s = 0; s < FormTraits<F>::NS; ++s) { st.hi[q][s] = 0; st.gs[q][s] = 0; st.hv[q][s][0] = st.hv[q][s][1] = st.hv[q][s][2] = 0; }
     }
     st.hiu = st.hus = st.gsu = 0;
+    static_assert(!CK || (NFIX > 0 && F == F_KP), "constant row classes: the fixed-length KP kernels only");
     fx.bound_classes(st);
     unsigned cls0[SPL];
 #pragma unroll
     for (int q = 0; q < SPL; ++q) cls0[q] = st.cls[q];
     const unsigned clse0 = st.clse, clsc0 = st.clsc;
+    unsigned cls_std[SPL];
+#pragma unroll
+    for (int q = 0; q < SPL; ++q) cls_std[q] = kStdClsLoc;
+    const unsigned *const cls_k = CK ? cls_std : cls0;
+    const unsigned clsc_k = CK ? kStdClsCtl : clsc0;
     double rb = uni(fmin(fmax(P.ref_nw_rho, kRhoMin), kRhoMax)), pri_outer = -1.0;
     rho_solve = uni(rho_solve); rp0 = uni(rp0); rd0 = uni(rd0);
     fx.nw_req = uni(P.ref_nw_rho_eq);
@@ -3864,11 +3870,11 @@
 #define PO_NW_TICK(i)
 #endif
     PO_FRESH_LANE_ID(fx);
-    if constexpr (!resume) fx.nw_reexpress_pass(st, rho_solve / rb, kRhoEqOverIneq * rho_solve / fx.nw_req, cls0, clse0, clsc0);
+    if constexpr (!resume) fx.nw_reexpress_pass(st, rho_solve / rb, kRhoEqOverIneq * rho_solve / fx.nw_req, cls_k, clse0, clsc_k);
     for (;;) {
         PO_FRESH_LANE_ID(fx);
         PO_MARK("nw_reclass");
-        (void)fx.reclass_pass(st, cls0, clse0, clsc0, rb, rb, 3);
+        (void)fx.reclass_pass(st, cls_k, clse0, clsc_k, rb, rb, 3);
         PO_NW_TICK(0)
         PO_MARK("nw_residual");
         R = fx.template residual_pass_two<false>(st, rb);
@@ -3903,7 +3909,7 @@
             }
             pri_outer = R.rp;
             PO_FRESH_LANE_ID(fx);
-            fx.nw_reexpress_pass(st, ratio, ratio_eq, cls0, clse0, clsc0);
+            fx.nw_reexpress_pass(st, ratio, ratio_eq, cls_k, clse0, clsc_k);
             quiet = false;
             continue;
         }
@@ -4000,7 +4006,7 @@
                tcy[0], tcy[1], tcy[2], fx.dbgc[0], fx.dbgc[1], fx.dbgc[2], tcy[3], tcy[4], tcy[5], tcy[6], tcy[7]);
 #endif
 #undef PO_NW_TICK
-    (void)fx.reclass_pass(st, cls0, clse0, clsc0, rb, rho_solve, 2, fx.nw_req, kRhoEqOverIneq * rho_solve);
+    (void)fx.reclass_pass(st, cls_k, clse0, clsc_k, rb, rho_solve, 2, fx.nw_req, kRhoEqOverIneq * rho_solve);
     fx.nw_req = 0.0;
     RefineOut o = {!R.bad && (stop || (R.rp <= rp0 && R.rd <= rd0)), stop && !R.bad, it2, nfac, R, false};
     return o;
@@ -4189,61 +4195,33 @@
     }
 }
 
-template <int F, int SPL, int NT, int NWX = 1, int PH = 1, int NFIX = 0> __global__ PO_KERNEL_ATTR __launch_bounds__(NT) void newton_kernel(DevBatch in, DevParams P) {
-    using FX = Fast<F, SPL, NT, true, NWX, NFIX>;
+#define PO_NW_KERNEL newton_kernel
+#define PO_NW_CK false
+#include "po_newton_kernel.inc"
+#undef PO_NW_KERNEL
+#undef PO_NW_CK
+#define PO_NW_KERNEL newton_kernel_std
+#define PO_NW_CK true
+#include "po_newton_kernel.inc"
+#undef PO_NW_KERNEL
+#undef PO_NW_CK
+template <int F, int SPL, int NT, int NFIX> __global__ PO_KERNEL_ATTR __launch_bounds__(NT) void newton_std_select_kernel(DevBatch in, DevParams P) {
+    static_assert(NT == 64, "constant row classes: one wave per path");
+    using FX = Fast<F, SPL, NT, true, 1, NFIX>;
     extern __shared__ double smem[];
-#ifdef PO_NW_TRACE
-    const long long tk0_ = __builtin_readcyclecounter();
-#endif
-    int b;
-    if constexpr (PH == 2) {
-        if ((int)blockIdx.x >= in.nw_list[0]) return;
-        b = in.nw_list[1 + blockIdx.x];
-    } else b = in.order ? in.order[blockIdx.x] : perm_index(blockIdx.x, in.perm_bits, in.B);
+    const int b = in.order ? in.order[blockIdx.x] : perm_index(blockIdx.x, in.perm_bits, in.B);
     if ((unsigned)b >= (unsigned)in.B) return;
-    po_info *oi = in.out_info + b;
-    const bool slicing = PH == 2 || P.ref_nw_slice > 0;
-    if (oi->status != PO_STATUS_SOLVED) return;
     FX fx(P, in, smem, b);
     typename FX::LS st;
     fx.load(st);
-    double *state = in.pol_state + (size_t)b * in.pol_stride;
-    double *pstate = slicing ? in.nw_state + (size_t)b * in.nw_stride : nullptr, *pscal = slicing ? pstate + (size_t)FX::kParkDoubles * NT : nullptr;
-    if constexpr (PH == 2) fx.template park_io<false>(st, pstate); else fx.template state_io<false>(st, state);
-    for (int i = fx.tid; i < fx.L.total; i += NT) smem[i] = 0.0;
-    __syncthreads();
-    fx.scale_to_lds();
-    const int lo_it = uni(oi->iters), lo_nref = uni(oi->n_refactor);
-    const double lo_rho = uni(oi->rho), rp0 = uni(oi->r_prim), rd0 = uni(oi->r_dual);
-    const int rounds = P.ref_rounds > 1 ? P.ref_rounds : 1, rounds_total = rounds + P.ref_extra;
-    const bool last = 1 >= rounds_total;
-#ifdef PO_NW_TRACE
-    const long long tk1_ = __builtin_readcyclecounter();
-#endif
-    const RefineOut ro = refine_phase_newton<F, SPL, NT, NWX, PH, NFIX>(fx, st, P, lo_rho, rp0, rd0, slicing ? P.ref_nw_slice : 1 << 30, pscal, slicing ? in.nw_keys + b : nullptr);
-    __syncthreads();
-#ifdef PO_NW_TRACE
-    const long long tk2_ = __builtin_readcyclecounter();
-    if (fx.b == 0 && fx.tid == 0) printf("  dev kernel PH %d: entry %lld cycles (load, LDS set-up, state block), phase %lld (%d steps)\n", PH, tk1_ - tk0_, tk2_ - tk1_, ro.it);
-#endif
-    if constexpr (PH == 1) if (ro.parked) { fx.template park_io<true>(st, pstate); return; }
-    const bool hand_back = !ro.stop && !last;
-    if (ro.take) { if (hand_back || P.polish) fx.template state_io<true>(st, state); }
-    else if (!hand_back) fx.template state_io<false>(st, state);
-    if (hand_back) {
-        if (fx.tid == 0) {
-            oi->status = kStatusDeferred - 1; oi->iters = lo_it + ro.it; oi->status_polish = lo_it; oi->n_refactor = lo_nref + ro.nfac;
-            if (ro.take) { oi->r_prim = ro.R.rp; oi->r_dual = ro.R.rd; oi->obj = ro.R.obj; }
-            oi->status_refine = -1;
-            in.fb_list[1 + atomicAdd(in.fb_list, 1)] = b;
-        }
-        return;
-    }
-    fx.output_pass(st);
+    bool standard = st.clsc == kStdClsCtl;
+#pragma unroll
+    for (int q = 0; q < SPL; ++q) standard = standard && st.cls[q] == kStdClsLoc;
+    const bool all = __all(standard) != 0;
     if (fx.tid == 0) {
-        oi->iters = lo_it + ro.it; oi->n_refactor = lo_nref + ro.nfac;
-        if (ro.take) { oi->r_prim = ro.R.rp; oi->r_dual = ro.R.rd; oi->obj = ro.R.obj; }
-        oi->status_refine = ro.stop ? 1 : -1;
+        const StdLists sl = std_lists(in.nw_keys, in.B);
+        (all ? sl.order : sl.left1)[blockIdx.x] = b;
+        sl.flag[b] = all ? 1 : 0;
     }
 }
 
diff --git a/path_optimizer_amd/csrc/po_handle.hpp b/path_optimizer_amd/csrc/po_handle.hpp
--- a/path_optimizer_amd/csrc/po_handle.hpp
+++ b/path_optimizer_amd/csrc/po_handle.hpp
@@ -110,6 +110,9 @@
     int wave_slots = 1024;
     PO_GUARDED_BY(mu) bool fixed_length = true;
     PO_GUARDED_BY(mu) int fixed_used = 0;
+    PO_GUARDED_BY(mu) bool fixed_classes = true;
+    PO_GUARDED_BY(mu) int std_B = 0;
+    PO_GUARDED_BY(mu) long std_flag_at = -1, std_left2_at = -1;
     PO_GUARDED_BY(mu) int dp_waves_used = 0;
     PO_GUARDED_BY(mu) int smooth_variant_used = 0;
     PO_GUARDED_BY(mu) int nw_slice = 8;
diff --git a/path_optimizer_amd/csrc/po_kernels.hip b/path_optimizer_amd/csrc/po_kernels.hip
--- a/path_optimizer_amd/csrc/po_kernels.hip
+++ b/path_optimizer_amd/csrc/po_kernels.hip
@@ -100,25 +100,43 @@
     return call(form, kind, launch, *s, in, P, st);
 }
 extern "C" hipError_t po_launch_newton(int form, const po::SolveShape *s, const po::DevBatch *in, const po::DevParams *P, hipStream_t st) { return launch_two_level(form, po::kLaunchNewton, s, in, P, st); }
+extern "C" hipError_t po_launch_newton_std(int form, const po::SolveShape *s, const po::DevBatch *in, const po::DevParams *P, hipStream_t st) {
+    using namespace po;
+    if (!s->two || !fixed(*s, in) || !in->nw_keys) return hipErrorInvalidValue;
+    const bool second = in->nw_phase == 2;
+    const StdLists sl = std_lists(in->nw_keys, in->B);
+    hipError_t e;
+    DevBatch std_ = *in, rest = *in;
+    if (second) rest.nw_list = sl.left2;
+    else {
+        if ((e = call(form, kObjFixNewtonStd1, kLaunchStdSelect, *s, in, P, st)) != hipSuccess) return e;
+        std_.order = sl.order; rest.order = sl.left1;
+    }
+    if ((e = call(form, second ? kObjFixNewtonStd2 : kObjFixNewtonStd1, kLaunchNewtonStd, *s, &std_, P, st)) != hipSuccess) return e;
+    return call(form, second ? kObjFixNewton2 : kObjFixNewton1, kLaunchNewton, *s, &rest, P, st);
+}
 extern "C" hipError_t po_launch_newton_fallback(int form, const po::SolveShape *s, const po::DevBatch *in, const po::DevParams *P, hipStream_t st) { return launch_two_level(form, po::kLaunchFallback, s, in, P, st); }
 extern "C" hipError_t po_launch_polish(int form, const po::SolveShape *s, const po::DevBatch *in, const po::DevParams *P, hipStream_t st) { return launch_two_level(form, po::kLaunchPolish, s, in, P, st); }
 namespace po {
 constexpr int kNwSortThreads = 256;
-__global__ __launch_bounds__(kNwSortThreads) void nw_sort_kernel(const int *keys, int B, int *list) {
+__global__ __launch_bounds__(kNwSortThreads) void nw_sort_kernel(const int *keys, int B, int *list, const int *flag, int *list2) {
+    const int want = blockIdx.x == 0 ? 1 : 0;
+    if (blockIdx.x != 0) list = list2;
+    auto key = [&](int b) { return (flag == nullptr || flag[b] == want) ? keys[b] : -1; };
     __shared__ int cnt[kNwKeys][kNwSortThreads + 1];
     __shared__ int rowbase[kNwKeys];
     const int t = threadIdx.x, per = (B + kNwSortThreads - 1) / kNwSortThreads, lo = t * per, hi = min(B, lo + per);
     constexpr int kCache = 16;
     int kc[kCache];
 #pragma unroll
-    for (int i = 0; i < kCache; ++i) kc[i] = (lo + i < hi) ? keys[lo + i] : -1;
+    for (int i = 0; i < kCache; ++i) kc[i] = (lo + i < hi) ? key(lo + i) : -1;
 #pragma unroll
     for (int k = 0; k < kNwKeys; ++k) cnt[k][t] = 0;
 #pragma unroll
     for (int i = 0; i < kCache; ++i)
         if (kc[i] >= 0) cnt[kc[i] < kNwKeys ? kc[i] : kNwKeys - 1][t] += 1;
     for (int b = lo + kCache; b < hi; ++b) {
-        const int k = keys[b];
+        const int k = key(b);
         if (k >= 0) cnt[k < kNwKeys ? k : kNwKeys - 1][t] += 1;
     }
     __syncthreads();
@@ -156,14 +174,14 @@
     for (int i = 0; i < kCache; ++i)
         if (kc[i] >= 0) place(lo + i, kc[i]);
     for (int b = lo + kCache; b < hi; ++b) {
-        const int k = keys[b];
+        const int k = key(b);
         if (k >= 0) place(b, k);
     }
 }
 
 }
-extern "C" hipError_t po_launch_nw_sort(const int *keys, int B, int *list, hipStream_t st) {
-    hipLaunchKernelGGL(po::nw_sort_kernel, dim3(1), dim3(po::kNwSortThreads), 0, st, keys, B, list);
+extern "C" hipError_t po_launch_nw_sort(const int *keys, int B, int *list, const int *flag, int *list2, hipStream_t st) {
+    hipLaunchKernelGGL(po::nw_sort_kernel, dim3(flag ? 2 : 1), dim3(po::kNwSortThreads), 0, st, keys, B, list, flag, list2);
     return hipGetLastError();
 }
 extern "C" int po_resolve_solve(int form, int N, int C, int keep, po::SolveShape *r) {
@@ -198,12 +216,13 @@
 extern "C" int po_has_polish_kernel(int form, int N, int C, int keep) { return resolved(form, N, C, keep).polish; }
 extern "C" int po_has_fixed_length(int form, int N, int C, int keep) { return resolved(form, N, C, keep).fixed; }
 
-extern "C" hipError_t po_launch_scale(int form, const po::DevBatch *in, const po::DevParams *P, int passes, double *sc, int *nw_keys, int *fb_count, hipStream_t st) {
+extern "C" hipError_t po_launch_scale(int form, const po::DevBatch *in, const po::DevParams *P, int passes, double *sc, int *nw_keys, int *fb_count, int *std_block,
+                                      hipStream_t st) {
     using namespace po;
     const int bs = 64, gs = (in->B + bs - 1) / bs;
-    if (form == F_KP) hipLaunchKernelGGL(scale_kernel<F_KP>, dim3(gs), dim3(bs), 0, st, *in, *P, passes, sc, nw_keys, fb_count);
-    else if (form == F_KPC) hipLaunchKernelGGL(scale_kernel<F_KPC>, dim3(gs), dim3(bs), 0, st, *in, *P, passes, sc, nw_keys, fb_count);
-    else hipLaunchKernelGGL(scale_kernel<F_K>, dim3(gs), dim3(bs), 0, st, *in, *P, passes, sc, nw_keys, fb_count);
+    if (form == F_KP) hipLaunchKernelGGL(scale_kernel<F_KP>, dim3(gs), dim3(bs), 0, st, *in, *P, passes, sc, nw_keys, fb_count, std_block);
+    else if (form == F_KPC) hipLaunchKernelGGL(scale_kernel<F_KPC>, dim3(gs), dim3(bs), 0, st, *in, *P, passes, sc, nw_keys, fb_count, std_block);
+    else hipLaunchKernelGGL(scale_kernel<F_K>, dim3(gs), dim3(bs), 0, st, *in, *P, passes, sc, nw_keys, fb_count, std_block);
     return hipGetLastError();
 }
 
diff --git a/path_optimizer_amd/csrc/po_launch.hpp b/path_optimizer_amd/csrc/po_launch.hpp
--- a/path_optimizer_amd/csrc/po_launch.hpp
+++ b/path_optimizer_amd/csrc/po_launch.hpp
@@ -6,8 +6,8 @@
 namespace po {
 struct DevBatch; struct DevParams;
 struct Shape;
-enum { kObjUni, kObjGen, kObjNewton, kObjFixUni, kObjFixNewton1, kObjFixNewton2 };
-enum { kLaunchSolve, kLaunchNewton, kLaunchFallback, kLaunchPolish };
+enum { kObjUni, kObjGen, kObjNewton, kObjFixUni, kObjFixNewton1, kObjFixNewton2, kObjFixNewtonStd1, kObjFixNewtonStd2 };
+enum { kLaunchSolve, kLaunchNewton, kLaunchFallback, kLaunchPolish, kLaunchNewtonStd, kLaunchStdSelect };
 enum { kGrpLane = 1, kGrpSplit = 2, kGrpMulti = 4, kGrpW56 = 8, kGrpW7 = 16, kGrpW8 = 32, kGrpOne = 64 };
 struct SolveShape {
     int nt, spl, two, nwx;
@@ -27,12 +27,13 @@
 int po_resolve_solve(int form, int N, int C, int keep, po::SolveShape *s);
 hipError_t po_launch_solve(int form, const po::SolveShape *s, const po::DevBatch *in, const po::DevParams *P, hipStream_t st);
 hipError_t po_launch_newton(int form, const po::SolveShape *s, const po::DevBatch *in, const po::DevParams *P, hipStream_t st);
+hipError_t po_launch_newton_std(int form, const po::SolveShape *s, const po::DevBatch *in, const po::DevParams *P, hipStream_t st);
 hipError_t po_launch_newton_fallback(int form, const po::SolveShape *s, const po::DevBatch *in, const po::DevParams *P, hipStream_t st);
 hipError_t po_launch_polish(int form, const po::SolveShape *s, const po::DevBatch *in, const po::DevParams *P, hipStream_t st);
 hipError_t po_launch_finalize_status(po_info *info, int B, hipStream_t st);
 hipError_t po_launch_mark_unavailable(po_info *info, int B, int refine, int polish, hipStream_t st);
-hipError_t po_launch_nw_sort(const int *keys, int B, int *list, hipStream_t st);
-hipError_t po_launch_scale(int form, const po::DevBatch *in, const po::DevParams *P, int passes, double *sc, int *nw_keys, int *fb_count, hipStream_t st);
+hipError_t po_launch_nw_sort(const int *keys, int B, int *list, const int *flag, int *list2, hipStream_t st);
+hipError_t po_launch_scale(int form, const po::DevBatch *in, const po::DevParams *P, int passes, double *sc, int *nw_keys, int *fb_count, int *std_block, hipStream_t st);
 hipError_t po_launch_assemble(int form, const po::DevBatch *in, const po::DevParams *P, double *l, double *u, double *dyn, hipStream_t st);
 size_t po_lds_bytes(int form, int N, int C, int keep);
 int po_shape_threads(int form, int N, int C, int keep);
@@ -63,7 +64,9 @@
     X(po_newton_k, F_K, kObjNewton, kGrpLane)                                   \
     X(po_solve_kp_fix_uni, F_KP, kObjFixUni, kGrpLane)                          \
     X(po_newton_kp_fix1, F_KP, kObjFixNewton1, kGrpLane)                        \
-    X(po_newton_kp_fix2, F_KP, kObjFixNewton2, kGrpLane)
+    X(po_newton_kp_fix2, F_KP, kObjFixNewton2, kGrpLane)                        \
+    X(po_newton_kp_fixstd1, F_KP, kObjFixNewtonStd1, kGrpLane)                  \
+    X(po_newton_kp_fixstd2, F_KP, kObjFixNewtonStd2, kGrpLane)
 #if defined(PO_DEV_HEADLINE) && !defined(PO_ENTRY)
 #define PO_OBJECT_ATTR __attribute__((weak))
 #else
diff --git a/path_optimizer_amd/csrc/po_newton_kernel.inc b/path_optimizer_amd/csrc/po_newton_kernel.inc
--- /dev/null
+++ b/path_optimizer_amd/csrc/po_newton_kernel.inc
@@ -0,0 +1,58 @@
+template <int F, int SPL, int NT, int NWX = 1, int PH = 1, int NFIX = 0> __global__ PO_KERNEL_ATTR __launch_bounds__(NT) void PO_NW_KERNEL(DevBatch in, DevParams P) {
+    constexpr bool CK = PO_NW_CK;
+    using FX = Fast<F, SPL, NT, true, NWX, NFIX>;
+    extern __shared__ double smem[];
+#ifdef PO_NW_TRACE
+    const long long tk0_ = __builtin_readcyclecounter();
+#endif
+    int b;
+    if constexpr (PH == 2) {
+        if ((int)blockIdx.x >= in.nw_list[0]) return;
+        b = in.nw_list[1 + blockIdx.x];
+    } else b = in.order ? in.order[blockIdx.x] : perm_index(blockIdx.x, in.perm_bits, in.B);
+    if ((unsigned)b >= (unsigned)in.B) return;
+    po_info *oi = in.out_info + b;
+    const bool slicing = PH == 2 || P.ref_nw_slice > 0;
+    if (oi->status != PO_STATUS_SOLVED) return;
+    FX fx(P, in, smem, b);
+    typename FX::LS st;
+    fx.load(st);
+    double *state = in.pol_state + (size_t)b * in.pol_stride;
+    double *pstate = slicing ? in.nw_state + (size_t)b * in.nw_stride : nullptr, *pscal = slicing ? pstate + (size_t)FX::kParkDoubles * NT : nullptr;
+    if constexpr (PH == 2) fx.template park_io<false>(st, pstate); else fx.template state_io<false>(st, state);
+    for (int i = fx.tid; i < fx.L.total; i += NT) smem[i] = 0.0;
+    __syncthreads();
+    fx.scale_to_lds();
+    const int lo_it = uni(oi->iters), lo_nref = uni(oi->n_refactor);
+    const double lo_rho = uni(oi->rho), rp0 = uni(oi->r_prim), rd0 = uni(oi->r_dual);
+    const int rounds = P.ref_rounds > 1 ? P.ref_rounds : 1, rounds_total = rounds + P.ref_extra;
+    const bool last = 1 >= rounds_total;
+#ifdef PO_NW_TRACE
+    const long long tk1_ = __builtin_readcyclecounter();
+#endif
+    const RefineOut ro = refine_phase_newton<F, SPL, NT, NWX, PH, NFIX, CK>(fx, st, P, lo_rho, rp0, rd0, slicing ? P.ref_nw_slice : 1 << 30, pscal, slicing ? in.nw_keys + b : nullptr);
+    __syncthreads();
+#ifdef PO_NW_TRACE
+    const long long tk2_ = __builtin_readcyclecounter();
+    if (fx.b == 0 && fx.tid == 0) printf("  dev kernel PH %d: entry %lld cycles (load, LDS set-up, state block), phase %lld (%d steps)\n", PH, tk1_ - tk0_, tk2_ - tk1_, ro.it);
+#endif
+    if constexpr (PH == 1) if (ro.parked) { fx.template park_io<true>(st, pstate); return; }
+    const bool hand_back = !ro.stop && !last;
+    if (ro.take) { if (hand_back || P.polish) fx.template state_io<true>(st, state); }
+    else if (!hand_back) fx.template state_io<false>(st, state);
+    if (hand_back) {
+        if (fx.tid == 0) {
+            oi->status = kStatusDeferred - 1; oi->iters = lo_it + ro.it; oi->status_polish = lo_it; oi->n_refactor = lo_nref + ro.nfac;
+            if (ro.take) { oi->r_prim = ro.R.rp; oi->r_dual = ro.R.rd; oi->obj = ro.R.obj; }
+            oi->status_refine = -1;
+            in.fb_list[1 + atomicAdd(in.fb_list, 1)] = b;
+        }
+        return;
+    }
+    fx.output_pass(st);
+    if (fx.tid == 0) {
+        oi->iters = lo_it + ro.it; oi->n_refactor = lo_nref + ro.nfac;
+        if (ro.take) { oi->r_prim = ro.R.rp; oi->r_dual = ro.R.rd; oi->obj = ro.R.obj; }
+        oi->status_refine = ro.stop ? 1 : -1;
+    }
+}
diff --git a/path_optimizer_amd/csrc/po_scale.hpp b/path_optimizer_amd/csrc/po_scale.hpp
--- a/path_optimizer_amd/csrc/po_scale.hpp
+++ b/path_optimizer_amd/csrc/po_scale.hpp
@@ -108,11 +108,16 @@
     out[kScC] = c;
 }
 
-template <int F> __global__ void scale_kernel(DevBatch in, DevParams P, int passes, double *sc, int *nw_keys, int *fb_count) {
+template <int F> __global__ void scale_kernel(DevBatch in, DevParams P, int passes, double *sc, int *nw_keys, int *fb_count, int *std_block) {
     const int b = blockIdx.x * blockDim.x + threadIdx.x;
     if (b >= in.B) return;
     if (nw_keys) nw_keys[b] = -1;
     if (fb_count && b == 0) *fb_count = 0;
+    if (std_block) {
+        const StdLists sl = std_lists(std_block, in.B);
+        sl.left1[b] = -1; sl.order[b] = -1; sl.flag[b] = 0;
+        if (b == 0) sl.left2[0] = 0;
+    }
     const double *s = in.ref_s + (size_t)b * in.N;
     int N = in.N, C = in.C;
     if (in.n_points) { N = in.n_points[b]; N = N < 2 ? 2 : (N > in.N ? in.N : N); C = (F == F_K) ? N - 1 : (N + in.keep - 2) / in.keep; }
diff --git a/path_optimizer_amd/csrc/po_solve.cpp b/path_optimizer_amd/csrc/po_solve.cpp
--- a/path_optimizer_amd/csrc/po_solve.cpp
+++ b/path_optimizer_amd/csrc/po_solve.cpp
@@ -93,11 +93,12 @@
     bool state;
     bool split, sliced;
     bool polish, fixed;
+    bool std_classes;
     bool no_refine, no_polish;
     bool read_back;
     int warm_decades;
 };
-SolveSchedule plan_solve(const po_params &p, const po::SolveShape &s, int B, bool ragged, int nw_slice, bool slice_forced, bool fixed_on, int wave_slots) {
+SolveSchedule plan_solve(const po_params &p, const po::SolveShape &s, int B, bool ragged, int nw_slice, bool slice_forced, bool fixed_on, int wave_slots, bool classes_on) {
     SolveSchedule q{};
     const int rounds = p.refine_rounds > 1 ? p.refine_rounds : 1;
     const int rounds_total = rounds + ((p.refine && p.refine_extra_rounds > 0) ? p.refine_extra_rounds : 0);
@@ -106,6 +107,7 @@
     q.split = p.refine == 2 && q.state && rounds_total < 32;
     q.sliced = q.split && nw_slice > 0 && (slice_forced || (B >= 2 * wave_slots && s.nt == 64));
     q.fixed = fixed_on && !ragged && s.fixed;
+    q.std_classes = q.fixed && q.split && classes_on;
     q.no_refine = p.refine == 2 && !q.split;
     q.no_polish = p.polish && !q.polish;
     q.read_back = p.refine_chain != 3;
@@ -117,15 +119,24 @@
     if (h->env_cycles) PO_TRY(h->dbg_buf.ensure(sizeof(long long) * 16 * B));
     PO_TRY(h->scale_buf.ensure(sizeof(double) * 64 * B));
     if (q->state) PO_TRY(h->pol_buf.ensure(sizeof(double) * (size_t)s.state_doubles * B));
+    h->std_B = 0; h->std_flag_at = h->std_left2_at = -1;
     if (!q->split) return PO_OK;
     PO_TRY(h->fb_buf.ensure(sizeof(int) * (B + 1)));
     PO_TRY(h->fb_host.ensure(64));
-    if (q->sliced && (h->nw_state_buf.ensure(sizeof(double) * (size_t)s.park_doubles * B) || h->nw_idx_buf.ensure(sizeof(int) * (2 * B + 1)))) {
+    const size_t idx_bytes = sizeof(int) * (q->std_classes ? po::std_lists_ints(B) : 2 * B + 1);
+    if (q->sliced && (h->nw_state_buf.ensure(sizeof(double) * (size_t)s.park_doubles * B) || h->nw_idx_buf.ensure(idx_bytes))) {
         (void)hipGetLastError();
         h->nw_state_buf.release();
         q->sliced = false;
     }
+    if (q->std_classes && h->nw_idx_buf.ensure(idx_bytes)) {
+        (void)hipGetLastError();
+        q->std_classes = false;
+    }
     h->nw_last_B = q->sliced ? (int)B : 0;
+    h->std_flag_at = q->std_classes ? (long)po::std_flag_index(B) : -1;
+    h->std_B = q->std_classes ? (int)B : 0;
+    h->std_left2_at = q->std_classes && q->sliced ? (long)po::std_left2_index(B) : -1;
     return PO_OK;
 }
 
@@ -139,8 +150,9 @@
     if (q.state) { D.pol_state = static_cast<double *>(h->pol_buf.p); D.pol_stride = s.state_doubles; }
     HIP_TRY(hipEventRecord(h->ev0, h->stream));
     h->timed_phases = false;
-    HIP_TRY(po_launch_scale(form, &D, &P, h->params.scaling, static_cast<double *>(h->scale_buf.p), q.sliced ? static_cast<int *>(h->nw_idx_buf.p) : nullptr,
-                            q.split ? static_cast<int *>(h->fb_buf.p) : nullptr, h->stream));
+    int *const nw_block = static_cast<int *>(h->nw_idx_buf.p);
+    HIP_TRY(po_launch_scale(form, &D, &P, h->params.scaling, static_cast<double *>(h->scale_buf.p), q.sliced ? nw_block : nullptr,
+                            q.split ? static_cast<int *>(h->fb_buf.p) : nullptr, q.std_classes ? nw_block : nullptr, h->stream));
     if (q.split) {
         po::DevParams P1 = P;
         for (int r = 0; r < q.warm_decades; ++r) { P1.eps_abs *= 10.0; P1.eps_rel *= 10.0; }
@@ -149,18 +161,23 @@
         D.nw_follows = 0;
         HIP_TRY(hipEventRecord(h->evp[0], h->stream));
         D.fb_list = static_cast<int *>(h->fb_buf.p);
+        const auto launch_newton = q.std_classes ? &po_launch_newton_std : &po_launch_newton;
+        if (q.std_classes) D.nw_keys = nw_block;
         if (q.sliced) {
             D.nw_state = static_cast<double *>(h->nw_state_buf.p); D.nw_stride = s.park_doubles;
-            D.nw_keys = static_cast<int *>(h->nw_idx_buf.p); D.nw_list = D.nw_keys + B;
+            D.nw_keys = nw_block; D.nw_list = D.nw_keys + B;
             P.ref_nw_slice = h->nw_slice;
             D.nw_phase = 1;
-            HIP_TRY(po_launch_newton(form, &s, &D, &P, h->stream));
-            HIP_TRY(po_launch_nw_sort(D.nw_keys, B, D.nw_list, h->stream));
+            HIP_TRY(launch_newton(form, &s, &D, &P, h->stream));
+            if (q.std_classes) {
+                const po::StdLists sl = po::std_lists(D.nw_keys, B);
+                HIP_TRY(po_launch_nw_sort(D.nw_keys, B, D.nw_list, sl.flag, sl.left2, h->stream));
+            } else HIP_TRY(po_launch_nw_sort(D.nw_keys, B, D.nw_list, nullptr, nullptr, h->stream));
             D.nw_phase = 2;
-            HIP_TRY(po_launch_newton(form, &s, &D, &P, h->stream));
+            HIP_TRY(launch_newton(form, &s, &D, &P, h->stream));
             D.nw_phase = 0;
         } else {
-            HIP_TRY(po_launch_newton(form, &s, &D, &P, h->stream));
+            HIP_TRY(launch_newton(form, &s, &D, &P, h->stream));
         }
         HIP_TRY(hipEventRecord(h->evp[1], h->stream));
         h->timed_phases = true;
@@ -226,7 +243,7 @@
     if (s.lds > po::kLdsLimit) return PO_ERR_UNSUPPORTED;
     po_params p{};
     p.refine = refine; p.refine_rounds = refine_rounds; p.refine_extra_rounds = refine_extra_rounds; p.refine_chain = refine_chain; p.polish = polish;
-    const SolveSchedule q = plan_solve(p, s, B, ragged != 0, nw_slice, slice_forced != 0, fixed_on != 0, wave_slots);
+    const SolveSchedule q = plan_solve(p, s, B, ragged != 0, nw_slice, slice_forced != 0, fixed_on != 0, wave_slots,  true);
     for (int v : {(int)q.split, (int)q.state, (int)q.polish, (int)q.sliced, (int)q.fixed, (int)q.no_refine, (int)q.no_polish, (int)q.read_back, q.warm_decades}) *out++ = v;
     return PO_OK;
 }
@@ -242,7 +259,7 @@
     po::DevParams P = make_dev_params(h->params, in->formulation, in->keep);
     po::DevBatch D = fill_dev_batch(h, in, out, d);
     const po::SolveShape &s = d.shape;
-    SolveSchedule q = plan_solve(h->params, s, in->B, in->n_points != nullptr, h->nw_slice, h->nw_slice_forced, h->fixed_length, h->wave_slots);
+    SolveSchedule q = plan_solve(h->params, s, in->B, in->n_points != nullptr, h->nw_slice, h->nw_slice_forced, h->fixed_length, h->wave_slots, h->fixed_classes);
     h->fixed_used = D.fixed_len = q.fixed;
     PO_TRY(provision(h, s, (size_t)in->B, &q));
     PO_TRY(enqueue(h, in->formulation, s, q, D, P));
@@ -401,7 +418,7 @@
         din.ref_s = rs;
         const po::DevParams P = make_dev_params(h->params, in->formulation, in->keep);
         const po::DevBatch D = fill_dev_batch(h, &din, nullptr, d);
-        HIP_TRY(po_launch_scale(in->formulation, &D, &P, h->params.scaling, sc, nullptr, nullptr, h->stream));
+        HIP_TRY(po_launch_scale(in->formulation, &D, &P, h->params.scaling, sc, nullptr, nullptr, nullptr, h->stream));
         return PO_OK;
     });
 }
diff --git a/path_optimizer_amd/csrc/po_solve_form.hip b/path_optimizer_amd/csrc/po_solve_form.hip
--- a/path_optimizer_amd/csrc/po_solve_form.hip
+++ b/path_optimizer_amd/csrc/po_solve_form.hip
@@ -17,10 +17,11 @@
     return {-1, -1, 0};
 }
 static_assert(me().form >= 0, "PO_ENTRY names no object of PO_SOLVE_OBJECTS");
+constexpr bool newton_object(int kind) { return kind == kObjNewton || kind == kObjFixNewton1 || kind == kObjFixNewton2 || kind == kObjFixNewtonStd1 || kind == kObjFixNewtonStd2; }
 #ifdef PO_REF
-static_assert(me().kind == kObjNewton || me().kind == kObjFixNewton1 || me().kind == kObjFixNewton2, "-DPO_REF=3 is for the Newton objects");
+static_assert(newton_object(me().kind), "-DPO_REF=3 is for the Newton objects");
 #else
-static_assert(me().kind != kObjNewton && me().kind != kObjFixNewton1 && me().kind != kObjFixNewton2, "the Newton objects build with -DPO_REF=3");
+static_assert(!newton_object(me().kind), "the Newton objects build with -DPO_REF=3");
 #endif
 [[maybe_unused]] constexpr bool holds(int G, bool two, int spl, int nt, int nwx, int g) {
 #ifdef PO_DEV_HEADLINE
@@ -66,10 +67,16 @@
 #undef PO_X
     return hipErrorNotSupported;
 }
-template <int F, int KIND> hipError_t launch_fixed(const DevBatch *in, const DevParams *P, size_t lds, hipStream_t st) {
+template <int F, int KIND> hipError_t launch_fixed(int launch, const DevBatch *in, const DevParams *P, size_t lds, hipStream_t st) {
 #define PO_X(N_)                                                                                                                                \
     if (in->N == N_) {                                                                                                                          \
         if constexpr (KIND == kObjFixUni) return launch1(&solve_kernel_fast<F, kFixSpl, kFixNt, true, true, 1, N_>, in, P, kFixNt, lds, st);    \
+        else if constexpr (KIND == kObjFixNewtonStd1) {                                                                                         \
+                           \
+            if (launch == kLaunchStdSelect) return launch1(&newton_std_select_kernel<F, kFixSpl, kFixNt, N_>, in, P, kFixNt, 0, st);            \
+            return launch1(&newton_kernel_std<F, kFixSpl, kFixNt, 1, 1, N_>, in, P, kFixNt, lds, st);                                           \
+        }                                                                                                                                       \
+        else if constexpr (KIND == kObjFixNewtonStd2) return launch1(&newton_kernel_std<F, kFixSpl, kFixNt, 1, 2, N_>, in, P, kFixNt, lds, st);    \
         else return launch1(&newton_kernel<F, kFixSpl, kFixNt, 1, KIND == kObjFixNewton2 ? 2 : 1, N_>, in, P, kFixNt, lds, st);                 \
     }
     PO_FIXED_LIST(PO_X)
@@ -82,7 +89,7 @@
         if (launch == kLaunchNewton) return launch_newton<F, G, false>(s, lds, in, P, st);
         if (launch == kLaunchFallback) return launch_newton<F, G, true>(s, lds, in, P, st);
         return hipErrorNotSupported;
-    } else return launch_fixed<F, KIND>(in, P, lds, st);
+    } else return launch_fixed<F, KIND>(launch, in, P, lds, st);
 }
 }
 extern "C" hipError_t PO_ENTRY(int launch, const po::Shape &s, size_t lds, const po::DevBatch *in, const po::DevParams *P, hipStream_t st) {
```

After: 1.223 million (median of 6 runs). 1.01x the previous value.
